# AdeeshKolluru/AdsorbDiff

Measured on AMD Instinct MI355X. Metric: sampled adsorbate sites/sec (50 denoise steps, ~200-atom slabs), higher is better.
Workload: dtype f32 (f16x3-split MFMA, fp32 accumulate; ADF_GEMM=f32 selects exact f32)

## Files before the change

### adsorbdiff_amd/csrc/api.hip

```cpp
#include <stdarg.h>
#include <stdlib.h>
#include <string.h>

#include <new>

#include "common.h"

static thread_local char g_err[512] = "";

void adf_set_error(const char* fmt, ...) {
    va_list ap;
    va_start(ap, fmt);
    vsnprintf(g_err, sizeof(g_err), fmt, ap);
    va_end(ap);
}

extern "C" const char* adf_last_error(void) { return g_err; }
extern "C" const char* adf_version(void) { return "adsorbdiff_hip 0.5.0 (gfx950)"; }

adf_tune adf_tune_from_env() {
    auto off_is_0 = [](const char* name) { const char* e = getenv(name); return (e && atoi(e) == 0) ? 0 : 1; };
    auto is_f32 = [](const char* name) { const char* e = getenv(name); return e && strcmp(e, "f32") == 0; };
    adf_tune t = {};
    const char* mi = getenv("ADF_GEMM16_MI");
    t.gemm16_mi = (mi && atoi(mi) == 4) ? 4 : 2;
    t.gemm_w8_plain = off_is_0("ADF_GEMM_W8_PLAIN");
    t.gemm_w8 = off_is_0("ADF_GEMM_W8");
    t.gemm_wreg = off_is_0("ADF_GEMM_WREG");
    const char* wf = getenv("ADF_GEMM_WR_FUSED");
    t.gemm_wr_fused = wf ? atoi(wf) : 2;
    if (t.gemm_wr_fused != 0 && t.gemm_wr_fused != 4) t.gemm_wr_fused = 2;
    t.head_gate_fused = off_is_0("ADF_HEAD_GATE_FUSED");
    t.lift_emit = off_is_0("ADF_LIFT_EMIT");
    t.graph_sys_csr = off_is_0("ADF_GRAPH_SYS_CSR");
    t.train_gemm16 = is_f32("ADF_TRAIN_GEMM") ? 0 : 1;
    t.wgrad_f32 = is_f32("ADF_WGRAD") ? 1 : 0;
    const char* pw = getenv("ADF_EQV2_PW_MI");
    t.eqv2_pw_mi = (pw && atoi(pw) == 3) ? 3 : 4;
    const char* gt = getenv("ADF_EQV2_GEMM_TILE");
    t.eqv2_gemm_tile256 = (gt && atoi(gt) == 128) ? 0 : 1;
    t.eqv2_rotin_generic = getenv("ADF_EQV2_ROTIN_GENERIC") != nullptr;
    t.eqv2_rotout_generic = getenv("ADF_EQV2_ROTOUT_GENERIC") != nullptr;
    const char* r4 = getenv("ADF_GEMM_ROWS4");
    t.gemm_rows4 = r4 ? (atoi(r4) & 3) : 3;
    return t;
}
const adf_tune& adf_tune_process() {
    static const adf_tune t = adf_tune_from_env();
    return t;
}
int adf_current_num_cus() {
    int dev = 0, n = 0;
    if (hipGetDevice(&dev) != hipSuccess || hipDeviceGetAttribute(&n, hipDeviceAttributeMultiprocessorCount, dev) != hipSuccess) return 0;
    return n;
}

extern "C" int32_t adf_profile_enable(adf_painn_t h, int32_t on) {
    if (!h) { adf_set_error("null handle"); return ADF_EINVAL; }
    h->prof.enable(on != 0);
    ADF_HIP_CHECK(hipMemset(h->kcount, 0, 8 * sizeof(unsigned long long)));
    return ADF_OK;
}

extern "C" int32_t adf_profile_read(adf_painn_t h, float* ms, int64_t* count, int64_t* message_ksteps, void* stream) {
    if (!h || !ms || !count) { adf_set_error("null argument"); return ADF_EINVAL; }
    ADF_HIP_CHECK(hipStreamSynchronize((hipStream_t)stream));
    if (message_ksteps) {
        unsigned long long k[8];
        ADF_HIP_CHECK(hipMemcpy(k, h->kcount, sizeof(k), hipMemcpyDeviceToHost));
        ADF_HIP_CHECK(hipMemset(h->kcount, 0, sizeof(k)));
        *message_ksteps = (int64_t)k[0];
    }
    return h->prof.read(ms, count, ADF_PROF_NCAT);
}

extern "C" int32_t adf_painn_create(const adf_painn_hparams* hp, adf_painn_t* out) {
    if (!hp || !out) { adf_set_error("null argument"); return ADF_EINVAL; }
    if (hp->hidden_channels % ADF_SLICE_CH != 0 || hp->hidden_channels < 128 || hp->hidden_channels > 1024) {
        adf_set_error("hidden_channels=%d must be a multiple of %d in [128,1024]", hp->hidden_channels, ADF_SLICE_CH);
        return ADF_EINVAL;
    }
    if (hp->num_rbf % 2 != 0 || hp->num_rbf > 128 || hp->num_rbf < 2) {
        adf_set_error("num_rbf=%d must be even and <= 128", hp->num_rbf);
        return ADF_EINVAL;
    }
    if (hp->max_neighbors < 1 || hp->max_neighbors > ADF_MAX_K) {
        adf_set_error("max_neighbors=%d must be in [1,%d]", hp->max_neighbors, ADF_MAX_K);
        return ADF_EINVAL;
    }
    if (hp->num_layers < 1 || hp->num_layers > 16 || hp->num_heads < 0 || hp->num_heads > 2) {
        adf_set_error("num_layers must be in [1,16], num_heads in [0,2]");
        return ADF_EINVAL;
    }
    adf_painn* h = new (std::nothrow) adf_painn();
    if (!h) { adf_set_error("host allocation failed"); return ADF_EOOM; }
    h->hp = *hp;
    hipDeviceProp_t prop;
    if (hipGetDevice(&h->device) != hipSuccess || hipGetDeviceProperties(&prop, h->device) != hipSuccess) {
        adf_set_error("no usable HIP device: %s", hipGetErrorString(hipGetLastError()));
        adf_painn_destroy(h);
        return ADF_EHIP;
    }
    h->num_cus = prop.multiProcessorCount;
    h->dist_floor = 1.0e-3f;
    {
        const char* e = getenv("ADF_INCREMENTAL");
        h->inc_on = !(e && e[0] == '0');
        const char* e2 = getenv("ADF_INC_SYNC");
        h->inc_sync = e2 && e2[0] == '1';
    }
    const int H = hp->hidden_channels, R = hp->num_rbf, L = hp->num_layers;
    adf_pool& m = h->m_life;
    int32_t st = m.alloc(&h->rbf_pack, (size_t)L * (H / ADF_SLICE_CH) * R * 192);
    if (st == ADF_OK) st = m.alloc(&h->rbf_bias_pack, (size_t)L * (H / ADF_SLICE_CH) * 192);
    if (st == ADF_OK) st = m.alloc(&h->rbf_pack16, (size_t)L * (H / ADF_SLICE_CH) * R * 192 * 2 * sizeof(uint16_t));
    if (st == ADF_OK) st = m.alloc(&h->rbf_bias_pack16, (size_t)L * (H / ADF_SLICE_CH) * 192);
    if (st == ADF_OK) st = m.alloc(&h->rbf_scales, 16);
    if (st == ADF_OK) st = m.alloc(&h->flags, ADF_NFLAGS);
    if (st == ADF_OK && hipMemset(h->flags, 0, sizeof(int32_t) * ADF_NFLAGS) != hipSuccess) st = ADF_EHIP;
    {
        const size_t HH = (size_t)H * H;
        const size_t per_layer = HH + 3 * HH + 2 * HH + 2 * HH + 3 * HH;
        const size_t per_head = HH + HH / 2 + 2 * HH + HH + HH / 4 + HH / 2;
        const size_t elems = (size_t)L * per_layer + (size_t)hp->num_heads * per_head;
        h->w16_bytes = elems * 2 * sizeof(uint16_t) + 4096;
        if (st == ADF_OK) st = m.alloc(&h->w16_arena, h->w16_bytes);
        if (st == ADF_OK) st = m.alloc(&h->w16_scales, 256);
        if (st == ADF_OK) st = m.alloc(&h->w16_bias_perm, (size_t)L * 2 * 3 * H);
        if (st == ADF_OK) st = m.alloc(&h->w16_scratch, 1);
        if (st == ADF_OK) st = m.alloc(&h->wfrag_arena, h->w16_bytes);
        const char* e = getenv("ADF_GEMM");
        h->gemm_f32 = e && strcmp(e, "f32") == 0;
        const char* el = getenv("ADF_LIFT");
        h->lift_on = !(el && strcmp(el, "0") == 0);
        const char* e2 = getenv("ADF_MSG");
        h->msg_f32 = e2 ? strcmp(e2, "f32") == 0 : h->gemm_f32;
        const char* er = getenv("ADF_ROW_MAXIMA");
        h->rmx = (er && atoi(er) == 0) ? 0 : 1;
        h->tune = adf_tune_from_env();
    }
    if (st == ADF_OK) st = m.alloc(&h->kcount, 8);
    if (st == ADF_OK && hipMemset(h->kcount, 0, 8 * sizeof(unsigned long long)) != hipSuccess) st = ADF_EHIP;
    if (st != ADF_OK) { adf_painn_destroy(h); return st; }
    *out = h;
    return ADF_OK;
}

static void inc_free(adf_painn* h) {
    h->m_inc.release();
    h->inc_tmp_bytes = 0;
    h->inc_capN = 0; h->inc_valid = false;
}

static void free_workspaces(adf_painn* h) {
    h->m_ws.release();
    h->inc_valid = false;
    h->scan_tmp_bytes = 0;
    h->lift.cap = 0; h->mag_v3_valid = false;
    h->xpart = h->catpart = h->vpart = nullptr; h->part_stride = 0;
    h->part_x = h->part_vec = nullptr; h->dbg_msg_rows = h->dbg_cat_rows = h->dbg_comb_rows = 0; h->dbg_mag = nullptr;
    h->cache_valid = false;
    h->capN = h->capB = h->capE = 0;
}

extern "C" int32_t adf_painn_destroy(adf_painn_t h) {
    if (!h) return ADF_OK;
    if (h->inc_cnt_host) (void)hipHostFree(h->inc_cnt_host);
    for (int i = 0; i < 2; ++i)
        if (h->inc_ev[i]) (void)hipEventDestroy((hipEvent_t)h->inc_ev[i]);
    adf_grad_free(h);
    delete h;
    return ADF_OK;
}

extern "C" int32_t adf_painn_set_weights(adf_painn_t h, int32_t n_weights, const void* const* w,
                                         const float* scale_factors, void* stream) {
    if (!h || !w || !scale_factors) { adf_set_error("null argument"); return ADF_EINVAL; }
    const int L = h->hp.num_layers;
    const int expect = 2 + ADF_WEIGHTS_PER_LAYER * L + ADF_WEIGHTS_PER_HEAD * h->hp.num_heads;
    if (n_weights != expect) {
        adf_set_error("expected %d weight tensors, got %d", expect, n_weights);
        return ADF_EINVAL;
    }
    for (int i = 0; i < n_weights; ++i)
        if (!w[i]) { adf_set_error("weight %d is null", i); return ADF_EINVAL; }
    auto f = [&](int i) { return reinterpret_cast<const float*>(w[i]); };
    h->emb = f(0);
    h->rbf_offset = f(1);
    int k = 2;
    for (int l = 0; l < L; ++l) {
        adf_layer_weights& lw = h->layer[l];
        lw.ln_w = f(k++); lw.ln_b = f(k++); lw.xp0_w = f(k++); lw.xp0_b = f(k++); lw.xp2_w = f(k++); lw.xp2_b = f(k++);
        lw.rbf_w = f(k++); lw.rbf_b = f(k++); lw.vp_w = f(k++); lw.xv0_w = f(k++); lw.xv0_b = f(k++);
        lw.xv2_w = f(k++); lw.xv2_b = f(k++);
        h->scale[l] = scale_factors[l];
    }
    for (int hd = 0; hd < h->hp.num_heads; ++hd)
        for (int b = 0; b < 2; ++b) {
            adf_block_weights& bw = h->head[hd][b];
            bw.vec1_w = f(k++); bw.vec2_w = f(k++); bw.un0_w = f(k++); bw.un0_b = f(k++); bw.un2_w = f(k++);
            bw.un2_b = f(k++);
        }
    ADF_TRY(adf_pack_rbf(h, (hipStream_t)stream));
    {
        hipStream_t s = (hipStream_t)stream;
        const long long H = h->hp.hidden_channels, HH = H * H;
        unsigned char* cur = h->w16_arena;
        unsigned char* fcur = h->wfrag_arena;
        int nscale = 0;
        float* bperm = h->w16_bias_perm;
        auto split = [&](const float* w, long long rows, long long K, adf_w16* out, const float* fused_bias = nullptr,
                         bool pair_perm = false) -> int32_t {
            const long long n = rows * K;
            out->hi = cur; cur += n * 2;
            out->lo = cur; cur += n * 2;
            out->inv_scale = h->w16_scales + nscale++;
            out->bias_perm = nullptr;
            out->frag = nullptr;
            if (fused_bias) {
                out->bias_perm = bperm; bperm += 3 * H;
                ADF_TRY(adf_split_weight(w, n, out, h->w16_scratch, s, (int)H, (int)H, fused_bias));
            } else if (pair_perm) {
                ADF_TRY(adf_split_weight(w, n, out, h->w16_scratch, s, (int)H, (int)H, nullptr, 2));
            } else {
                ADF_TRY(adf_split_weight(w, n, out, h->w16_scratch, s));
            }
            if (rows % 32 == 0 && K % 16 == 0) {
                out->frag = fcur; fcur += n * 4;
                ADF_TRY(adf_pack_frag(out, (int)rows, (int)K, out->frag, s));
            }
            return ADF_OK;
        };
        for (int l = 0; l < L; ++l) {
            adf_layer_weights& lw = h->layer[l];
            ADF_TRY(split(lw.xp0_w, H, H, &lw.xp0_16));
            ADF_TRY(split(lw.xp2_w, 3 * H, H, &lw.xp2_16, lw.xp2_b));
            ADF_TRY(split(lw.vp_w, 2 * H, H, &lw.vp_16, nullptr, true));
            ADF_TRY(split(lw.xv0_w, H, 2 * H, &lw.xv0_16));
            ADF_TRY(split(lw.xv2_w, 3 * H, H, &lw.xv2_16, lw.xv2_b));
        }
        for (int hd = 0; hd < h->hp.num_heads; ++hd) {
            adf_block_weights& b0 = h->head[hd][0];
            adf_block_weights& b1 = h->head[hd][1];
            ADF_TRY(split(b0.vec1_w, H, H, &b0.vec1_16));
            ADF_TRY(split(b0.vec2_w, H / 2, H, &b0.vec2_16));
            ADF_TRY(split(b0.un0_w, H, 2 * H, &b0.un0_16));
            ADF_TRY(split(b0.un2_w, H, H, &b0.un2_16));
            ADF_TRY(split(b1.vec1_w, H / 2, H / 2, &b1.vec1_16));
            ADF_TRY(split(b1.un0_w, H / 2, H, &b1.un0_16));
        }
        if ((size_t)(cur - h->w16_arena) > h->w16_bytes || (size_t)(fcur - h->wfrag_arena) > h->w16_bytes || nscale > 256) {
            adf_set_error("internal: fp16 weight arena overflow");
            return ADF_EINVAL;
        }
    }
    h->weights_set = true;
    h->rec0_valid = false;
    h->inc_valid = false;
    adf_grad_invalidate(h);
    return ADF_OK;
}

static int32_t ensure_capacity(adf_painn* h, int64_t N, int64_t B) {
    if (N <= h->capN && B <= h->capB) return ADF_OK;
    const int64_t capN = N > h->capN ? N : h->capN;
    const int64_t capB = B > h->capB ? B : h->capB;
    ADF_HIP_CHECK(hipDeviceSynchronize());
    free_workspaces(h);
    const int64_t H = h->hp.hidden_channels, K = h->hp.max_neighbors;
    const int64_t capE = 2 * capN * K;
    int32_t st = ADF_OK;
#define ALLOC(field, count) if (st == ADF_OK) st = h->m_ws.alloc(&h->field, (size_t)(count))
    ALLOC(nbr_cnt, capN);
    ALLOC(nbr_src, capN * K);
    ALLOC(nbr_shift, capN * K);
    ALLOC(cache_d2, capN * K);
    ALLOC(cache_cid, capN * K);
    ALLOC(cache_cnt, capN);
    ALLOC(deg, capN + 1);
    ALLOC(nptr, capN + 1);
    ALLOC(cursor, capN);
    ALLOC(img_cnt, capB);
    ALLOC(sys_slow, capB);
    ALLOC(e_src, capE);
    ALLOC(e_geom, capE);
    if (h->inc_on) {
        ALLOC(prev_nptr, capN + 1);
        ALLOC(prev_src, capE);
        ALLOC(prev_geom, capE);
    }
    if (st == ADF_OK) {
        h->scan_tmp_bytes = adf_scan_temp_bytes(capN + 1);
        st = h->m_ws.alloc(&h->scan_tmp, h->scan_tmp_bytes + 16);
    }
    ALLOC(x, capN * H);
    ALLOC(vecA, capN * 3 * H);
    ALLOC(vecB, capN * 3 * H);
    ALLOC(rec, (capN + 1) * 5 * H);
    ALLOC(y, capN * H);
    ALLOC(xh, capN * 3 * H);
    ALLOC(vv, capN * 6 * H);
    ALLOC(cat, capN * 2 * H);
    ALLOC(dot, capN * H);
    ALLOC(sys, capB * 16);
    ALLOC(lift.buf, capN * 3);
    ALLOC(mag_a, capN);
    ALLOC(mag_b, capN);
    ALLOC(mag_v3, capN * 3);
    const int64_t ps = (capN + 31) / 32 * 32, ns = H / ADF_SLICE_CH;
    if (h->rmx) ALLOC(rmx_part, (4 * ns + H / 32 + 4) * ps);
#undef ALLOC
    h->lift.cap = st == ADF_OK ? capN * 3 : 0;
    if (st != ADF_OK) { free_workspaces(h); return st; }
    if (h->rmx) {
        h->part_stride = ps;
        h->xpart = h->rmx_part; h->catpart = h->xpart + ns * ps; h->vpart = h->catpart + (H / 32) * ps;
        h->dbg_mag = h->vpart + 3 * ns * ps;
    }
    h->capN = capN; h->capB = capB; h->capE = capE;
    return ADF_OK;
}

static int32_t check_batch(const adf_painn* h, const adf_batch* b) {
    if (!h || !b) { adf_set_error("null argument"); return ADF_EINVAL; }
    if (b->num_atoms <= 0 || b->num_systems <= 0) { adf_set_error("empty batch"); return ADF_EINVAL; }
    if (!b->pos || !b->cell || !b->batch || !b->atom_offset) { adf_set_error("null batch array"); return ADF_EINVAL; }
    for (int k = 0; k < 3; ++k)
        if (b->reps[k] < 0 || b->reps[k] > 16) { adf_set_error("reps[%d]=%d out of range", k, b->reps[k]); return ADF_EINVAL; }
    return ADF_OK;
}

static int32_t read_flags(adf_painn* h, hipStream_t s) {
    int32_t f[ADF_NFLAGS];
    ADF_HIP_CHECK(hipMemcpyAsync(f, h->flags, sizeof(f), hipMemcpyDeviceToHost, s));
    ADF_HIP_CHECK(hipMemsetAsync(h->flags, 0, sizeof(f), s));
    ADF_HIP_CHECK(hipStreamSynchronize(s));
    if (f[4]) { adf_set_error("atomic number outside [1, %d] (rows of the embedding table)", h->hp.num_elements); return ADF_EINVAL; }
    if (f[0]) { adf_set_error("a centre atom has more than %d in-cutoff candidates", ADF_MAX_CAND); return ADF_EOVERFLOW; }
    if (f[2]) { adf_set_error("edge buffer overflow"); return ADF_EOVERFLOW; }
    if (f[3]) { adf_set_error("an atom has more than %d incoming edges", ADF_MAX_INDEG); return ADF_EOVERFLOW; }
    if (f[1]) { adf_set_error("An image has no neighbors"); return ADF_ENONEIGHBOR; }
    if (f[6]) { adf_set_error("energy gradient: an edge row has no reverse row in its partner's segment (asymmetric graph)"); return ADF_EINVAL; }
    if (f[5]) {
        adf_set_error("non-finite model output%s", h->gemm_f32 ? " (exact-f32 arithmetic: the inputs or weights are not finite)"
                      : " in f16x3 arithmetic: an activation left the fp16 range or the inputs are not finite; "
                        "adf_painn_set_arithmetic(h, 1) selects exact f32");
        return ADF_ENUMERIC;
    }
    return ADF_OK;
}

extern "C" int32_t adf_graph_set_moving(adf_painn_t h, const int32_t* moving, const int32_t* mov_idx,
                                        const int32_t* mov_off) {
    if (!h) { adf_set_error("null handle"); return ADF_EINVAL; }
    if (moving && (!mov_idx || !mov_off)) { adf_set_error("moving mask needs mov_idx and mov_off"); return ADF_EINVAL; }
    h->moving = moving; h->mov_idx = mov_idx; h->mov_off = mov_off;
    ADF_HIP_CHECK(hipMemset(h->flags, 0, sizeof(int32_t) * ADF_NFLAGS));
    h->cache_valid = false;
    h->rec0_valid = false;
    h->inc_valid = false;
    return ADF_OK;
}

extern "C" int32_t adf_graph_build(adf_painn_t h, const adf_batch* b, void* stream, int64_t* num_edges) {
    ADF_TRY(check_batch(h, b));
    ADF_TRY(ensure_capacity(h, b->num_atoms, b->num_systems));
    hipStream_t s = (hipStream_t)stream;
    ADF_TRY(adf_graph_build_impl(h, b, s));
    if (num_edges) {
        int32_t e = 0;
        ADF_HIP_CHECK(hipMemcpyAsync(&e, h->nptr + b->num_atoms, sizeof(int32_t), hipMemcpyDeviceToHost, s));
        ADF_TRY(read_flags(h, s));
        *num_edges = e;
    }
    return ADF_OK;
}

__global__ void adf_export_edges_kernel(const int32_t* nptr, const int32_t* e_src, const float4* eg, int N,
                                        int32_t* src, int32_t* dst, float* dist, float* vec, long long cap) {
    const int n = blockIdx.x * 4 + (threadIdx.x >> 6);
    if (n >= N) return;
    for (int e = nptr[n] + (threadIdx.x & 63); e < nptr[n + 1]; e += 64) {
        if (e >= cap) continue;
        if (src) src[e] = e_src[e];
        if (dst) dst[e] = n;
        const float4 q = eg[e];
        if (dist) dist[e] = q.w;
        if (vec) { vec[3 * (size_t)e] = q.x; vec[3 * (size_t)e + 1] = q.y; vec[3 * (size_t)e + 2] = q.z; }
    }
}

__global__ void adf_export_shift_kernel(const int32_t* nbr_shift, int32_t* out, long long n, int r0, int r1, int r2) {
    const long long i = (long long)blockIdx.x * blockDim.x + threadIdx.x;
    if (i >= n) return;
    const int c = nbr_shift[i];
    const int n2 = 2 * r2 + 1, n1 = 2 * r1 + 1;
    const int ia = c / (n1 * n2), rem = c - ia * (n1 * n2);
    out[3 * i] = ia - r0;
    out[3 * i + 1] = rem / n2 - r1;
    out[3 * i + 2] = rem % n2 - r2;
}

extern "C" int32_t adf_graph_export(adf_painn_t h, int32_t* nbr_count, int32_t* nbr_src, int32_t* nbr_shift,
                                    int64_t edge_capacity, int32_t* edge_src, int32_t* edge_dst, float* edge_dist,
                                    float* edge_vec, int64_t* num_edges, void* stream) {
    if (!h || h->lastN <= 0) { adf_set_error("no graph built"); return ADF_EINVAL; }
    hipStream_t s = (hipStream_t)stream;
    const int64_t N = h->lastN, K = h->hp.max_neighbors;
    if (nbr_count) ADF_HIP_CHECK(hipMemcpyAsync(nbr_count, h->nbr_cnt, sizeof(int32_t) * N, hipMemcpyDeviceToDevice, s));
    if (nbr_src) ADF_HIP_CHECK(hipMemcpyAsync(nbr_src, h->nbr_src, sizeof(int32_t) * N * K, hipMemcpyDeviceToDevice, s));
    if (nbr_shift)
        hipLaunchKernelGGL(adf_export_shift_kernel, dim3((unsigned)((N * K + 255) / 256)), dim3(256), 0, s, h->nbr_shift,
                           nbr_shift, (long long)(N * K), h->last_reps[0], h->last_reps[1], h->last_reps[2]);
    if (edge_src || edge_dst || edge_dist || edge_vec)
        hipLaunchKernelGGL(adf_export_edges_kernel, dim3((unsigned)((N + 3) / 4)), dim3(256), 0, s, h->nptr, h->e_src,
                           h->e_geom, (int)N, edge_src, edge_dst, edge_dist, edge_vec, (long long)edge_capacity);
    ADF_HIP_CHECK(hipGetLastError());
    int32_t e = 0;
    ADF_HIP_CHECK(hipMemcpyAsync(&e, h->nptr + N, sizeof(int32_t), hipMemcpyDeviceToHost, s));
    ADF_HIP_CHECK(hipStreamSynchronize(s));
    if (num_edges) *num_edges = e;
    return ADF_OK;
}

static int32_t zero_pad_rows(adf_painn* h, int N, hipStream_t s) {
    const size_t row = (size_t)5 * h->hp.hidden_channels;
    ADF_HIP_CHECK(hipMemsetAsync(h->rec + (size_t)N * row, 0, sizeof(float) * row, s));
    return ADF_OK;
}

static int32_t make_records(adf_painn* h, int l, int n, const float* x, const float* vec, bool vec_is_zero, float* rec,
                            const int32_t* row_map, hipStream_t s) {
    const int H = h->hp.hidden_channels;
    const adf_layer_weights& w = h->layer[l];
    if (n <= 0) return ADF_OK;
    adf_prof_begin(h, ADF_PROF_NODE, s);
    const bool lift = h->lift_on && !h->gemm_f32;
    const bool em = lift && h->tune.lift_emit;
    ADF_TRY(adf_nodewise_layernorm(x, w.ln_w, w.ln_b, h->y, n, H, s, em ? h->mag_a : nullptr, h->rows_dev));
    ADF_TRY(adf_linear(h, h->y, H, w.xp0_w, &w.xp0_16, w.xp0_b, h->cat, H, n, H, H, 1, s, em ? h->mag_a : nullptr,
                       em ? h->mag_b : nullptr));
    if (h->gemm_f32) {
        if (row_map) { adf_set_error("internal: mapped records need the f16x3 path"); return ADF_EINVAL; }
        ADF_TRY(adf_launch_gemm(h->cat, H, w.xp2_w, H, w.xp2_b, h->xh, 3 * H, n, 3 * H, H, 0, s));
        ADF_TRY(adf_pack_records(h, n, h->xh, vec, vec_is_zero, s, rec));
    } else {
        adf_epi ep = {};
        ep.vec_in = vec; ep.rec = rec ? rec : h->rec; ep.H = H; ep.vec_is_zero = vec_is_zero ? 1 : 0;
        ep.row_map = row_map;
        ep.rmag = em ? h->mag_b : nullptr;
        ep.m_dev = h->rows_dev;
        ADF_TRY(adf_launch_gemm16_fused(h->cat, H, &w.xp2_16, n, H, H, 1, &ep, s, h->tune, lift ? &h->lift : nullptr));
    }
    adf_prof_end(h, s);
    return ADF_OK;
}

static int32_t message_layer(adf_painn* h, int l, int N, const float* x, const float* vec, float* x_out,
                             float* vec_out, bool vec_is_zero, hipStream_t s, const int32_t* tlist = nullptr,
                             int n_targets = 0, float* rec = nullptr, bool records_ready = false) {
    if (!records_ready) ADF_TRY(make_records(h, l, N, x, vec, vec_is_zero, rec, nullptr, s));
    adf_prof_begin(h, ADF_PROF_MESSAGE, s);
    const int items = tlist ? n_targets : N;
    const bool emit = h->rmx && h->lift_on && !h->gemm_f32 && !h->msg_f32 && items > 0 && items <= h->part_stride;
    h->part_x = h->part_vec = nullptr;
    const int32_t st = adf_message_impl(h, l, N, x, h->xh, vec, x_out, vec_out, vec_is_zero, s, tlist, n_targets, rec,
                                        tlist ? h->rows_dev : nullptr, emit ? h->xpart : nullptr, h->vpart, h->part_stride);
    if (st == ADF_OK && emit) {
        h->part_x = x_out; h->part_vec = vec_out; h->part_n = items; h->part_dev = tlist ? h->rows_dev : nullptr;
        h->dbg_msg_rows = items;
    }
    adf_prof_end(h, s);
    return st;
}

static int32_t update_layer(adf_painn* h, int l, int N, float* x, float* vec, hipStream_t s, bool from_message = true) {
    const int H = h->hp.hidden_channels;
    const adf_layer_weights& w = h->layer[l];
    adf_prof_begin(h, ADF_PROF_NODE, s);
    const bool parts = from_message && h->rmx && h->lift_on && !h->gemm_f32 && N > 0 && h->part_x == x && h->part_vec == vec &&
                       h->part_n == N && h->part_dev == h->rows_dev;
    h->part_x = h->part_vec = nullptr;
    if (h->gemm_f32) {
        ADF_TRY(adf_launch_gemm(vec, H, w.vp_w, H, nullptr, h->vv, 2 * H, 3 * N, 2 * H, H, 0, s));
        ADF_TRY(adf_nodewise_update_prep(h->vv, x, h->cat, h->dot, N, H, s));
        ADF_TRY(adf_linear(h, h->cat, 2 * H, w.xv0_w, &w.xv0_16, w.xv0_b, h->y, H, N, H, 2 * H, 1, s));
    } else {
        adf_epi ep = {};
        ep.v1 = h->vv; ep.dotw = h->dot; ep.cat = h->cat; ep.H = H; ep.m_dev = h->rows_dev;
        const adf_lift* lf = h->lift_on ? &h->lift : nullptr;
        if (parts) {
            ADF_TRY(adf_launch_rowmax_combine(h->vpart, 3 * h->part_stride, H / ADF_SLICE_CH, 3ll * N, h->lift.buf, s, h->rows_dev, 3));
            ep.rmag = h->lift.buf;
            if (h->dbg_capture) ADF_HIP_CHECK(hipMemcpyAsync(h->dbg_mag, h->lift.buf, sizeof(float) * 3 * (size_t)N, hipMemcpyDeviceToDevice, s));
        }
        if (parts || (h->dbg_capture && h->rmx && lf && N <= h->part_stride)) {
            ep.catpart = h->catpart; ep.part_stride = h->part_stride; h->dbg_cat_rows = N;
        }
        ADF_TRY(adf_launch_gemm16_fused(vec, H, &w.vp_16, N, H, H, 3, &ep, s, h->tune, lf));
        if (parts) {
            ADF_TRY(adf_launch_rowmax_combine(h->xpart, h->part_stride, H / ADF_SLICE_CH + H / 32, N, h->lift.buf, s, h->rows_dev, 1));
            if (h->dbg_capture) {
                ADF_HIP_CHECK(hipMemcpyAsync(h->dbg_mag + 3 * h->part_stride, h->lift.buf, sizeof(float) * (size_t)N, hipMemcpyDeviceToDevice, s));
                h->dbg_comb_rows = N;
            }
        }
        adf_epi e0 = {};
        e0.A2 = h->cat; e0.K1 = H; e0.m_dev = h->rows_dev;
        e0.rmag = parts ? h->lift.buf : nullptr;
        e0.out_mag = h->lift_on ? reinterpret_cast<unsigned int*>(h->mag_b) : nullptr;
        ADF_TRY(adf_launch_gemm16(x, H, &w.xv0_16, w.xv0_b, h->y, H, N, H, 2 * H, 1, &e0, s, lf, h->tune, h->num_cus));
    }
    int32_t st;
    if (h->gemm_f32) {
        ADF_TRY(adf_launch_gemm(h->y, H, w.xv2_w, H, w.xv2_b, h->xh, 3 * H, N, 3 * H, H, 0, s));
        st = adf_nodewise_update_apply(h->xh, h->dot, h->vv, x, vec, h->scale[l], N, H, s);
    } else {
        adf_epi ep = {};
        ep.x = x; ep.vec = vec; ep.dot = h->dot; ep.vv = h->vv; ep.scale = h->scale[l]; ep.H = H;
        ep.rmag = h->lift_on ? h->mag_b : nullptr;
        ep.m_dev = h->rows_dev;
        st = adf_launch_gemm16_fused(h->y, H, &w.xv2_16, N, H, H, 2, &ep, s, h->tune);
    }
    adf_prof_end(h, s);
    return st;
}

extern "C" int32_t adf_painn_message_layer(adf_painn_t h, int32_t layer, int32_t N, const float* x, const float* vec,
                                           float* x_out, float* vec_out, void* stream) {
    if (!h || !h->weights_set || layer < 0 || layer >= h->hp.num_layers || N != h->lastN) {
        adf_set_error("message_layer: bad handle/layer, or N differs from the built graph");
        return ADF_EINVAL;
    }
    hipStream_t s = (hipStream_t)stream;
    ADF_TRY(zero_pad_rows(h, N, s));
    ADF_TRY(message_layer(h, layer, N, x, vec, x_out, vec_out, false, s));
    return ADF_OK;
}

extern "C" int32_t adf_painn_update_layer(adf_painn_t h, int32_t layer, int32_t N, float* x, float* vec, void* stream) {
    if (!h || !h->weights_set || layer < 0 || layer >= h->hp.num_layers) {
        adf_set_error("update_layer: bad handle/layer");
        return ADF_EINVAL;
    }
    ADF_TRY(ensure_capacity(h, N, 1));
    return update_layer(h, layer, N, x, vec, (hipStream_t)stream, false);
}

extern "C" int32_t adf_painn_get_tune(adf_painn_t h, adf_tune* out) {
    if (!h || !out) { adf_set_error("get_tune: null handle or output"); return ADF_EINVAL; }
    *out = h->tune;
    return ADF_OK;
}

extern "C" int32_t adf_painn_debug_row_maxima(adf_painn_t h, int32_t which, float* out, int64_t capacity, int32_t* rows,
                                              void* stream) {
    if (!h || which < 0 || which > 6) { adf_set_error("debug_row_maxima: null handle or which outside 0..6"); return ADF_EINVAL; }
    if (which == 4) { h->dbg_capture = capacity != 0; h->dbg_comb_rows = 0; return ADF_OK; }
    const int H = h->hp.hidden_channels, ns = H / ADF_SLICE_CH;
    const int n = which <= 1 ? h->dbg_msg_rows : which <= 3 ? h->dbg_cat_rows : h->dbg_comb_rows;
    if (!h->rmx_part || n <= 0) { adf_set_error("debug_row_maxima: no launch has emitted row maxima (ADF_ROW_MAXIMA=0?)"); return ADF_EINVAL; }
    if (rows) *rows = n;
    if (!out) return ADF_OK;
    const int64_t need = (which == 1 || which == 5) ? 3ll * n : which == 3 ? (int64_t)n * H : n;
    if (capacity < need) { adf_set_error("debug_row_maxima: out holds %lld floats, need %lld", (long long)capacity, (long long)need); return ADF_EINVAL; }
    hipStream_t s = (hipStream_t)stream;
    if (which == 0) return adf_launch_rowmax_combine(h->xpart, h->part_stride, ns, n, out, s);
    if (which == 1) return adf_launch_rowmax_combine(h->vpart, 3 * h->part_stride, ns, 3ll * n, out, s);
    if (which == 2) return adf_launch_rowmax_combine(h->catpart, h->part_stride, H / 32, n, out, s);
    if (which >= 5) {
        ADF_HIP_CHECK(hipMemcpyAsync(out, h->dbg_mag + (which == 5 ? 0 : 3 * h->part_stride), sizeof(float) * (size_t)need, hipMemcpyDeviceToDevice, s));
        return ADF_OK;
    }
    ADF_HIP_CHECK(hipMemcpyAsync(out, h->cat, sizeof(float) * (size_t)n * H, hipMemcpyDeviceToDevice, s));
    return ADF_OK;
}

__global__ void adf_scatter_rows3_kernel(const float* __restrict__ src, const int32_t* __restrict__ idx, int n,
                                         float* __restrict__ dst) {
    const int i = blockIdx.x * blockDim.x + threadIdx.x;
    if (i < 3 * n) dst[(size_t)idx[i / 3] * 3 + i % 3] = src[i];
}

static int32_t ensure_subset(adf_painn* h, int32_t n_out) {
    if (n_out <= h->capS) return ADF_OK;
    const int64_t cap = (int64_t)n_out + n_out / 4 + 64;
    const size_t H = h->hp.hidden_channels;
    h->m_sub.release();
    h->capS = 0;
    ADF_TRY(h->m_sub.alloc(&h->sub_x, (size_t)cap * H));
    ADF_TRY(h->m_sub.alloc(&h->sub_vec, (size_t)cap * 3 * H));
    ADF_TRY(h->m_sub.alloc(&h->sub_f, (size_t)cap * 3));
    h->capS = cap;
    return ADF_OK;
}

static int inc_prepare(adf_painn* h, int N) {
    const int L = h->hp.num_layers, H = h->hp.hidden_channels;
    if (!h->inc_on || !h->moving || h->gemm_f32 || h->msg_f32 || L > ADF_MAX_LAYERS || !h->prev_nptr)
        return 0;
    if (N > h->inc_capN) {
        (void)hipDeviceSynchronize();
        inc_free(h);
        const size_t cap = (size_t)N;
        int32_t st = ADF_OK;
        for (int l = 0; l <= L && st == ADF_OK; ++l) {
            st = h->m_inc.alloc(&h->incX[l], cap * H);
            if (st == ADF_OK && l >= 1) st = h->m_inc.alloc(&h->incV[l], cap * 3 * H);
            if (st == ADF_OK && l < L) st = h->m_inc.alloc(&h->incR[l], (cap + 1) * 5 * H);
        }
        if (st == ADF_OK) st = h->m_inc.alloc(&h->inc_c0, cap);
        if (st == ADF_OK) st = h->m_inc.alloc(&h->inc_chg, 2 * cap);
        if (st == ADF_OK) st = h->m_inc.alloc(&h->inc_pend, cap * L);
        if (st == ADF_OK) st = h->m_inc.alloc(&h->inc_need, cap * L);
        if (st == ADF_OK) st = h->m_inc.alloc(&h->inc_tf, cap * L);
        if (st == ADF_OK) st = h->m_inc.alloc(&h->inc_list, cap * L);
        if (st == ADF_OK) st = h->m_inc.alloc(&h->inc_cnt, (size_t)2 * ADF_MAX_LAYERS + 1);
        if (st == ADF_OK) {
            h->inc_tmp_bytes = adf_inc_temp_bytes((int64_t)cap);
            st = h->m_inc.alloc(&h->inc_tmp, h->inc_tmp_bytes + 16);
        }
        if (st == ADF_OK && !h->inc_cnt_host &&
            hipHostMalloc(reinterpret_cast<void**>(&h->inc_cnt_host), sizeof(int32_t) * 2 * (2 * ADF_MAX_LAYERS + 1)) != hipSuccess)
            st = ADF_EOOM;
        for (int i = 0; i < 2 && st == ADF_OK; ++i)
            if (!h->inc_ev[i] && hipEventCreateWithFlags(reinterpret_cast<hipEvent_t*>(&h->inc_ev[i]), hipEventDisableTiming) != hipSuccess)
                st = ADF_EHIP;
        if (st != ADF_OK) {
            (void)hipGetLastError();
            inc_free(h);
            h->inc_on = false;
            fprintf(stderr, "adsorbdiff_hip: no memory for incremental layers (%d atoms), continuing without\n", N);
            return 0;
        }
        h->inc_capN = (int64_t)cap;
    }
    if (h->inc_N != N || h->inc_layers != L || h->build_serial != h->inc_serial) h->inc_valid = false;
    h->inc_N = N; h->inc_layers = L;
    int32_t* tn = h->nptr; h->nptr = h->prev_nptr; h->prev_nptr = tn;
    int32_t* ts = h->e_src; h->e_src = h->prev_src; h->prev_src = ts;
    float4* tg = h->e_geom; h->e_geom = h->prev_geom; h->prev_geom = tg;
    const int state = h->inc_valid ? 1 : 2;
    h->inc_valid = false;
    return state;
}

static int32_t inc_harvest(adf_painn* h, int slot, bool wait, bool peek = false) {
    if (!h->inc_ev_live[slot]) return ADF_OK;
    hipEvent_t ev = (hipEvent_t)h->inc_ev[slot];
    if (wait) {
        ADF_HIP_CHECK(hipEventSynchronize(ev));
    } else {
        const hipError_t q = hipEventQuery(ev);
        if (q == hipErrorNotReady) { (void)hipGetLastError(); return ADF_OK; }
        ADF_HIP_CHECK(q);
    }
    const int L = h->inc_layers, N = h->inc_pend_N[slot];
    const int32_t* c = h->inc_cnt_host + (size_t)slot * (2 * ADF_MAX_LAYERS + 1);
    for (int i = 0; i < 2 * L + 1; ++i) h->inc_seen[i] = c[i];
    h->inc_seen_valid = true;
    h->inc_pend_Nseen = N;
    if (peek) return ADF_OK;
    h->inc_ev_live[slot] = false;
    for (int l = 0; l < L; ++l) {
        const bool whole = h->inc_pend_whole[slot][l] != 0;
        h->inc_rows += (unsigned long long)(whole ? N : c[l]);
        h->inc_rows_full += (unsigned long long)N;
        h->inc_edges += (unsigned long long)(whole ? c[2 * L] : c[L + l]);
        if (whole || c[l] > 0) ++h->inc_launches;
    }
    return ADF_OK;
}

static int32_t forward_incremental(adf_painn* h, int N, const int32_t* Z, const int32_t* out_idx, int32_t n_out,
                                   float* f1, float* f2, bool first, int heads, hipStream_t s) {
    const int L = h->hp.num_layers, H = h->hp.hidden_channels;
    const size_t cap = (size_t)h->inc_capN, row = (size_t)5 * H;
    if (out_idx && n_out == 0) return ADF_OK;
    adf_prof_begin(h, ADF_PROF_GRAPH, s);
    if (first) {
        ADF_TRY(adf_nodewise_embed(h, Z, N, h->incX[0], s));
        for (int l = 0; l < L; ++l) ADF_HIP_CHECK(hipMemsetAsync(h->incR[l] + (size_t)N * row, 0, sizeof(float) * row, s));
        ADF_HIP_CHECK(hipMemsetAsync(h->inc_pend, 0, cap * L, s));
    } else {
        ADF_TRY(adf_inc_compare(h, N, s));
    }
    ADF_HIP_CHECK(hipMemsetAsync(h->inc_cnt, 0, sizeof(int32_t) * (2 * ADF_MAX_LAYERS + 1), s));
    if (out_idx) ADF_TRY(adf_inc_need_from_list(h, N, L, out_idx, n_out, s));
    for (int l = 0; l < L; ++l) ADF_TRY(adf_inc_plan_layer(h, l, N, first, out_idx != nullptr, s));
    ADF_HIP_CHECK(hipMemcpyAsync(h->inc_cnt + 2 * L, h->nptr + N, sizeof(int32_t), hipMemcpyDeviceToDevice, s));
    const int slot = h->inc_slot;
    h->inc_slot ^= 1;
    if (h->inc_ev_live[slot]) ADF_TRY(inc_harvest(h, slot, true));
    int32_t* host = h->inc_cnt_host + (size_t)slot * (2 * ADF_MAX_LAYERS + 1);
    ADF_HIP_CHECK(hipMemcpyAsync(host, h->inc_cnt, sizeof(int32_t) * (2 * L + 1), hipMemcpyDeviceToHost, s));
    ADF_HIP_CHECK(hipEventRecord((hipEvent_t)h->inc_ev[slot], s));
    h->inc_ev_live[slot] = true;
    h->inc_pend_N[slot] = N;
    ADF_TRY(inc_harvest(h, slot ^ 1, false));
    if (h->inc_sync) ADF_TRY(inc_harvest(h, slot, true, true));
    adf_prof_end(h, s);
    if (first) ADF_TRY(make_records(h, 0, N, h->incX[0], nullptr, true, h->incR[0], nullptr, s));
    for (int l = 0; l < L; ++l) {
        const int n_seen = h->inc_seen_valid ? h->inc_seen[l] : N;
        const bool whole = first || !h->inc_seen_valid || h->inc_pend_Nseen != N || (long long)n_seen * 10 >= (long long)N * 9;
        h->inc_pend_whole[slot][l] = whole ? 1 : 0;
        if (h->inc_sync && !whole && n_seen == 0) continue;
        const float* vin = l == 0 ? h->vecA : h->incV[l];
        if (whole) {
            ADF_TRY(message_layer(h, l, N, h->incX[l], vin, h->incX[l + 1], h->incV[l + 1], l == 0, s, nullptr, 0,
                                  h->incR[l], true));
            ADF_TRY(update_layer(h, l, N, h->incX[l + 1], h->incV[l + 1], s));
            if (l + 1 < L)
                ADF_TRY(make_records(h, l + 1, N, h->incX[l + 1], h->incV[l + 1], false, h->incR[l + 1], nullptr, s));
            continue;
        }
        const int32_t* list = h->inc_list + cap * l;
        const int ncap = h->inc_sync ? n_seen : N;
        h->rows_dev = h->inc_cnt + l;
        int32_t st = message_layer(h, l, N, h->incX[l], vin, h->x, h->vecB, l == 0, s, list, ncap, h->incR[l], true);
        if (st == ADF_OK) st = update_layer(h, l, ncap, h->x, h->vecB, s);
        if (st == ADF_OK) {
            adf_prof_begin(h, ADF_PROF_NODE, s);
            st = adf_inc_scatter_rows(h->x, list, ncap, H, h->incX[l + 1], s, h->rows_dev);
            if (st == ADF_OK) st = adf_inc_scatter_rows(h->vecB, list, ncap, 3 * H, h->incV[l + 1], s, h->rows_dev);
            adf_prof_end(h, s);
        }
        if (st == ADF_OK && l + 1 < L) st = make_records(h, l + 1, ncap, h->x, h->vecB, false, h->incR[l + 1], list, s);
        h->rows_dev = nullptr;
        ADF_TRY(st);
    }
    adf_prof_begin(h, ADF_PROF_HEADS, s);
    if (!out_idx) {
        if (heads >= 1) ADF_TRY(adf_head_forward(h, 0, N, h->incX[L], h->incV[L], f1, s));
        if (heads == 2) ADF_TRY(adf_head_forward(h, 1, N, h->incX[L], h->incV[L], f2, s));
        h->x_last = h->incX[L];
    } else {
        ADF_TRY(ensure_subset(h, n_out));
        ADF_TRY(adf_inc_gather_rows(h->incX[L], out_idx, n_out, H, h->sub_x, s));
        ADF_TRY(adf_inc_gather_rows(h->incV[L], out_idx, n_out, 3 * H, h->sub_vec, s));
        for (int hd = 0; hd < heads; ++hd) {
            ADF_TRY(adf_head_forward(h, hd, n_out, h->sub_x, h->sub_vec, h->sub_f, s));
            hipLaunchKernelGGL(adf_scatter_rows3_kernel, dim3((3 * n_out + 255) / 256), dim3(256), 0, s, h->sub_f, out_idx,
                               n_out, hd == 0 ? f1 : f2);
        }
        ADF_HIP_CHECK(hipGetLastError());
    }
    adf_prof_end(h, s);
    h->inc_valid = true;
    return ADF_OK;
}

static int32_t forward_impl(adf_painn_t h, const adf_batch* b, const int32_t* out_idx, int32_t n_out, float* f1,
                            float* f2, void* stream, bool head1_only = false) {
    ADF_TRY(check_batch(h, b));
    if (!h->weights_set) { adf_set_error("weights not set"); return ADF_EINVAL; }
    const int heads = head1_only ? 1 : h->hp.num_heads;
    if (heads > h->hp.num_heads) { adf_set_error("the model has no force head"); return ADF_EINVAL; }
    if (!b->atomic_numbers || (heads >= 1 && !f1) || (heads == 2 && !f2)) { adf_set_error("null argument"); return ADF_EINVAL; }
    h->x_last = nullptr;
    hipStream_t s = (hipStream_t)stream;
    const int N = b->num_atoms;
    ADF_TRY(ensure_capacity(h, N, b->num_systems));
    const int inc = inc_prepare(h, N);
    adf_prof_begin(h, ADF_PROF_GRAPH, s);
    ADF_TRY(adf_graph_build_impl(h, b, s));
    adf_prof_end(h, s);
    if (inc) {
        h->inc_serial = h->build_serial;
        return forward_incremental(h, N, b->atomic_numbers, out_idx, n_out, f1, f2, inc == 2, heads, s);
    }
    ADF_TRY(zero_pad_rows(h, N, s));
    ADF_TRY(adf_nodewise_embed(h, b->atomic_numbers, N, h->x, s));
    float* vin = h->vecA;
    float* vout = h->vecB;
    const int L = h->hp.num_layers, H = h->hp.hidden_channels;
    float* rec0 = nullptr;
    bool rec0_ready = false;
    if (h->moving) {
        const size_t row = (size_t)5 * H;
        if ((int64_t)N + 1 > h->rec0_cap) {
            h->rec0_cap = 0; h->rec0_valid = false;
            ADF_TRY(h->m_rec0.alloc(&h->rec0, ((size_t)N + 1) * row));
            h->rec0_cap = (int64_t)N + 1;
        }
        rec0 = h->rec0;
        rec0_ready = h->rec0_valid && h->rec0_N == N;
        if (!rec0_ready) ADF_HIP_CHECK(hipMemsetAsync(rec0 + (size_t)N * row, 0, sizeof(float) * row, s));
        h->rec0_valid = true; h->rec0_N = N;
    }
    if (!out_idx) {
        for (int l = 0; l < L; ++l) {
            if (l == 0) ADF_TRY(message_layer(h, 0, N, h->x, vin, h->x, vout, true, s, nullptr, 0, rec0, rec0_ready));
            else
            ADF_TRY(message_layer(h, l, N, h->x, vin, h->x, vout, l == 0, s));
            ADF_TRY(update_layer(h, l, N, h->x, vout, s));
            float* t = vin; vin = vout; vout = t;
        }
        adf_prof_begin(h, ADF_PROF_HEADS, s);
        if (heads >= 1) ADF_TRY(adf_head_forward(h, 0, N, h->x, vin, f1, s));
        if (heads == 2) ADF_TRY(adf_head_forward(h, 1, N, h->x, vin, f2, s));
        adf_prof_end(h, s);
        h->x_last = h->x;
        return ADF_OK;
    }
    if (n_out == 0) return ADF_OK;
    ADF_TRY(ensure_subset(h, n_out));
    for (int l = 0; l + 1 < L; ++l) {
        if (l == 0) ADF_TRY(message_layer(h, 0, N, h->x, vin, h->x, vout, true, s, nullptr, 0, rec0, rec0_ready));
        else
        ADF_TRY(message_layer(h, l, N, h->x, vin, h->x, vout, l == 0, s));
        ADF_TRY(update_layer(h, l, N, h->x, vout, s));
        float* t = vin; vin = vout; vout = t;
    }
    ADF_TRY(message_layer(h, L - 1, N, h->x, vin, h->sub_x, h->sub_vec, L == 1, s, out_idx, n_out,
                          L == 1 ? rec0 : nullptr, L == 1 && rec0_ready));
    ADF_TRY(update_layer(h, L - 1, n_out, h->sub_x, h->sub_vec, s));
    adf_prof_begin(h, ADF_PROF_HEADS, s);
    for (int hd = 0; hd < heads; ++hd) {
        ADF_TRY(adf_head_forward(h, hd, n_out, h->sub_x, h->sub_vec, h->sub_f, s));
        hipLaunchKernelGGL(adf_scatter_rows3_kernel, dim3((3 * n_out + 255) / 256), dim3(256), 0, s, h->sub_f, out_idx,
                           n_out, hd == 0 ? f1 : f2);
    }
    ADF_HIP_CHECK(hipGetLastError());
    adf_prof_end(h, s);
    return ADF_OK;
}

extern "C" int32_t adf_painn_forward(adf_painn_t h, const adf_batch* b, float* f1, float* f2, void* stream) {
    return forward_impl(h, b, nullptr, 0, f1, f2, stream);
}

extern "C" int32_t adf_painn_forward_subset(adf_painn_t h, const adf_batch* b, const int32_t* out_idx, int32_t n_out,
                                            float* f1, float* f2, void* stream) {
    if (!out_idx || n_out < 0) { adf_set_error("forward_subset: null index list"); return ADF_EINVAL; }
    return forward_impl(h, b, out_idx, n_out, f1, f2, stream);
}

extern "C" int32_t adf_painn_set_energy_head(adf_painn_t h, int32_t n_weights, const void* const* w, void* stream) {
    if (!h || !w) { adf_set_error("null argument"); return ADF_EINVAL; }
    if (n_weights != 4) { adf_set_error("set_energy_head: expected 4 tensors (out_energy.0.weight/bias, out_energy.2.weight/bias), got %d", n_weights); return ADF_EINVAL; }
    for (int i = 0; i < 4; ++i)
        if (!w[i]) { adf_set_error("energy-head tensor %d is null", i); return ADF_EINVAL; }
    const int H = h->hp.hidden_channels, H2 = H / 2;
    const size_t n = (size_t)H2 * H;
    if (!h->oe0_buf) ADF_TRY(h->m_life.alloc(&h->oe0_buf, n * 4 + 64));
    h->oe0_w = reinterpret_cast<const float*>(w[0]);
    h->oe0_b = reinterpret_cast<const float*>(w[1]);
    h->oe2_w = reinterpret_cast<const float*>(w[2]);
    h->oe2_b = reinterpret_cast<const float*>(w[3]);
    adf_w16& e = h->oe0_16;
    e = adf_w16{};
    e.hi = h->oe0_buf; e.lo = h->oe0_buf + n * 2; e.inv_scale = reinterpret_cast<float*>(h->oe0_buf + n * 4);
    ADF_TRY(adf_split_weight(h->oe0_w, (long long)n, &e, reinterpret_cast<unsigned int*>(h->oe0_buf + n * 4 + 16),
                             (hipStream_t)stream));
    h->energy_set = true;
    adf_grad_invalidate(h);
    return ADF_OK;
}

extern "C" int32_t adf_painn_set_distance_floor(adf_painn_t h, float floor) {
    if (!h || !(floor > 0.f)) { adf_set_error("set_distance_floor: null handle or non-positive floor"); return ADF_EINVAL; }
    if (floor != h->dist_floor) {
        h->dist_floor = floor;
        h->cache_valid = false;
        h->rec0_valid = false;
        h->inc_valid = false;
    }
    return ADF_OK;
}

__global__ __launch_bounds__(256) void adf_energy_sum_kernel(const float* __restrict__ y, int H2, const float* __restrict__ w,
                                                             const float* __restrict__ bias, const int32_t* __restrict__ atom_offset,
                                                             float* __restrict__ energy) {
    __shared__ float part[4];
    const int b = blockIdx.x, lane = threadIdx.x & 63, wave = threadIdx.x >> 6;
    const int a0 = atom_offset[b], a1 = atom_offset[b + 1];
    const float b0 = bias[0];
    float acc = 0.f;
    for (int a = a0 + wave; a < a1; a += 4) {
        const float* row = y + (size_t)a * H2;
        float d = 0.f;
        for (int c = lane; c < H2; c += 64) d = fmaf(row[c], w[c], d);
        for (int o = 32; o > 0; o >>= 1) d = __fadd_rn(d, __shfl_xor(d, o, 64));
        acc = __fadd_rn(acc, __fadd_rn(d, b0));
    }
    if (lane == 0) part[wave] = acc;
    __syncthreads();
    if (threadIdx.x == 0) energy[b] = __fadd_rn(__fadd_rn(part[0], part[1]), __fadd_rn(part[2], part[3]));
}

int32_t adf_energy_sum(const float* y, int H2, const float* w, const float* bias, const int32_t* atom_offset, float* energy,
                       int num_systems, hipStream_t s) {
    hipLaunchKernelGGL(adf_energy_sum_kernel, dim3(num_systems), dim3(256), 0, s, y, H2, w, bias, atom_offset, energy);
    ADF_HIP_CHECK(hipGetLastError());
    return ADF_OK;
}

extern "C" int32_t adf_painn_forward_energy(adf_painn_t h, const adf_batch* b, float* energy, float* forces, void* stream) {
    ADF_TRY(check_batch(h, b));
    if (!h->energy_set) { adf_set_error("forward_energy: energy head not set (adf_painn_set_energy_head)"); return ADF_EINVAL; }
    if (!energy || (h->hp.num_heads >= 1 && !forces)) { adf_set_error("forward_energy: null output"); return ADF_EINVAL; }
    if (h->hp.num_heads > 1) { adf_set_error("forward_energy: the S2EF model has one force head"); return ADF_EINVAL; }
    hipStream_t s = (hipStream_t)stream;
    ADF_TRY(forward_impl(h, b, nullptr, 0, forces, nullptr, stream));
    if (!h->x_last) { adf_set_error("internal: no node features after the forward"); return ADF_EINVAL; }
    const int N = b->num_atoms, H = h->hp.hidden_channels, H2 = H / 2;
    adf_prof_begin(h, ADF_PROF_HEADS, s);
    ADF_TRY(adf_linear(h, h->x_last, H, h->oe0_w, &h->oe0_16, h->oe0_b, h->y, H2, N, H2, H, 1, s));
    ADF_TRY(adf_energy_sum(h->y, H2, h->oe2_w, h->oe2_b, b->atom_offset, energy, b->num_systems, s));
    adf_prof_end(h, s);
    return ADF_OK;
}

extern "C" int32_t adf_linear_forward(const float* A, const float* W, const float* bias, float* C, int32_t M,
                                      int32_t N, int32_t K, int32_t act_ssilu, int32_t mode, void* stream) {
    hipStream_t s = (hipStream_t)stream;
    if (!A || !W || !C || M <= 0 || N <= 0 || K <= 0) { adf_set_error("bad argument"); return ADF_EINVAL; }
    if (mode == 0) return adf_launch_gemm(A, K, W, K, bias, C, N, M, N, K, act_ssilu, s);
    adf_pool tmp;
    unsigned char* buf = nullptr;
    const size_t n = (size_t)N * K;
    ADF_TRY(tmp.alloc(&buf, n * 4 + 64));
    adf_w16 w16 = {};
    w16.hi = buf; w16.lo = buf + n * 2; w16.inv_scale = reinterpret_cast<float*>(buf + n * 4);
    unsigned int* scratch = reinterpret_cast<unsigned int*>(buf + n * 4 + 16);
    int32_t st = adf_split_weight(W, (long long)n, &w16, scratch, s);
    float* mags = nullptr;
    const char* el = getenv("ADF_LIFT");
    const bool lift = !(el && strcmp(el, "0") == 0);
    if (st == ADF_OK && lift) st = tmp.alloc(&mags, (size_t)M);
    adf_lift lf = {mags, M};
    if (st == ADF_OK) st = adf_launch_gemm16(A, K, &w16, bias, C, N, M, N, K, act_ssilu, nullptr, s, lift ? &lf : nullptr,
                                             adf_tune_process(), adf_current_num_cus());
    (void)hipStreamSynchronize(s);
    return st;
}

extern "C" int32_t adf_painn_set_arithmetic(adf_painn_t h, int32_t exact_f32) {
    if (!h) { adf_set_error("null handle"); return ADF_EINVAL; }
    h->gemm_f32 = exact_f32 != 0;
    h->msg_f32 = exact_f32 != 0;
    h->rec0_valid = false;
    h->inc_valid = false;
    return ADF_OK;
}

extern "C" int32_t adf_painn_set_incremental(adf_painn_t h, int32_t on) {
    if (!h) { adf_set_error("null handle"); return ADF_EINVAL; }
// ... 126 lines not shown
```

### adsorbdiff_amd/csrc/common.h

```cpp
#pragma once
#include <hip/hip_runtime.h>
#include <stdint.h>
#include <stdio.h>
#include <string>
#include <vector>

#include "../../include/adsorbdiff_hip.h"

#define ADF_GROUP_NODES 32
#define ADF_SLICE_CH 64
#define ADF_MAX_CAND 1024
#define ADF_MAX_K 128
#define ADF_NFLAGS 8
#define ADF_MAX_INDEG 1024
#define ADF_MAX_LAYERS 16

void adf_set_error(const char* fmt, ...);

#define ADF_HIP_CHECK(expr)                                                             \
    do {                                                                                \
        hipError_t _e = (expr);                                                         \
        if (_e != hipSuccess) {                                                         \
            adf_set_error("%s failed: %s (%s:%d)", #expr, hipGetErrorString(_e),        \
                          __FILE__, __LINE__);                                          \
            return (_e == hipErrorOutOfMemory) ? ADF_EOOM : ADF_EHIP;                   \
        }                                                                               \
    } while (0)

#define ADF_TRY(expr)                     \
    do {                                  \
        int32_t _s = (expr);              \
        if (_s != ADF_OK) return _s;      \
    } while (0)

struct adf_pool {
    std::vector<void**> slots;
    adf_pool() = default;
    adf_pool(const adf_pool&) = delete;
    adf_pool& operator=(const adf_pool&) = delete;
    ~adf_pool() { release(); }
    int32_t alloc(void** field, size_t bytes) {
        bool known = false;
        for (void** s : slots) known = known || s == field;
        if (known) { if (*field) (void)hipFree(*field); } else slots.push_back(field);
        *field = nullptr;
        if (bytes == 0) bytes = 16;
        const hipError_t e = hipMalloc(field, bytes);
        if (e == hipSuccess) return ADF_OK;
        *field = nullptr;
        (void)hipGetLastError();
        adf_set_error("device allocation of %zu bytes failed: %s", bytes, hipGetErrorString(e));
        return ADF_EOOM;
    }
    template <typename T>
    int32_t alloc(T** field, size_t count) { return alloc(reinterpret_cast<void**>(field), count * sizeof(T)); }
    void release() {
        for (void** s : slots) {
            if (*s) (void)hipFree(*s);
            *s = nullptr;
        }
        slots.clear();
    }
};

struct adf_prof {
    bool on = false;
    bool open = false;
    std::vector<hipEvent_t> ev;
    std::vector<int> cat;
    size_t used = 0;
    adf_prof() = default;
    adf_prof(const adf_prof&) = delete;
    adf_prof& operator=(const adf_prof&) = delete;
    ~adf_prof() { for (hipEvent_t e : ev) (void)hipEventDestroy(e); }
    void begin(int c, hipStream_t s) {
        open = false;
        if (!on) return;
        if (used + 2 > ev.size())
            for (int i = 0; i < 512; ++i) {
                hipEvent_t e;
                if (hipEventCreate(&e) != hipSuccess) { (void)hipGetLastError(); break; }
                ev.push_back(e);
            }
        if (used + 2 > ev.size()) return;
        cat.resize(used / 2);
        cat.push_back(c);
        (void)hipEventRecord(ev[used], s);
        open = true;
    }
    void end(hipStream_t s) {
        if (!on || !open) return;
        (void)hipEventRecord(ev[used + 1], s);
        used += 2;
        open = false;
    }
    void enable(bool o) { on = o; open = false; used = 0; cat.clear(); }
    int32_t read(float* ms, int64_t* count, int ncat) {
        for (int c = 0; c < ncat; ++c) { ms[c] = 0.f; count[c] = 0; }
        for (size_t i = 0; i < used; i += 2) {
            float t = 0.f;
            ADF_HIP_CHECK(hipEventElapsedTime(&t, ev[i], ev[i + 1]));
            ms[cat[i / 2]] += t;
            count[cat[i / 2]] += 1;
        }
        enable(on);
        return ADF_OK;
    }
    struct scope {
        adf_prof& p; hipStream_t s;
        scope(adf_prof& p_, int c, hipStream_t s_) : p(p_), s(s_) { p.begin(c, s); }
        ~scope() { p.end(s); }
    };
};

struct adf_w16 {
    void* hi;
    void* lo;
    float* inv_scale;
    float* bias_perm;
    void* frag;
};
struct adf_epi {
    const float* vec_in;
    float* rec;
    float* x;
    float* vec;
    const float* dot;
    const float* vv;
    float* v1;
    float* dotw;
    float* cat;
    float scale;
    int H;
    int vec_is_zero;
    const float* A2;
    int K1;
    const int32_t* row_map;
    const float* rmag;
    unsigned int* out_mag;
    const int32_t* m_dev;
    int accumulate;
    const float* gate;
    int gate_ld;
    float* catpart;
    long long part_stride;
};
struct adf_lift {
    float* buf;
    long long cap;
};
struct adf_layer_weights {
    const float *ln_w, *ln_b, *xp0_w, *xp0_b, *xp2_w, *xp2_b, *rbf_w, *rbf_b;
    const float *vp_w, *xv0_w, *xv0_b, *xv2_w, *xv2_b;
    adf_w16 xp0_16, xp2_16, vp_16, xv0_16, xv2_16;
};
struct adf_block_weights {
    const float *vec1_w, *vec2_w, *un0_w, *un0_b, *un2_w, *un2_b;
    adf_w16 vec1_16, vec2_16, un0_16, un2_16;
};

struct adf_painn {
    adf_painn_hparams hp;
    int device;
    bool weights_set;
    const float* emb;
    const float* rbf_offset;
    adf_layer_weights layer[16];
    adf_block_weights head[2][2];
    float scale[16];
    float* rbf_pack;
    float* rbf_bias_pack;
    void* rbf_pack16;
    float* rbf_bias_pack16;
    float* rbf_scales;
    unsigned char* w16_arena;
    size_t w16_bytes;
    float* w16_scales;
    float* w16_bias_perm;
    unsigned int* w16_scratch;
    unsigned char* wfrag_arena;
    bool gemm_f32;
    bool msg_f32;
    adf_tune tune;
    bool lift_on;
    adf_lift lift;
    float *mag_a, *mag_b;
    float* mag_v3;
    bool mag_v3_valid;
    int rmx;
    float* rmx_part;
    float *xpart, *catpart, *vpart;
    int64_t part_stride;
    const float *part_x, *part_vec;
    int part_n;
    const int32_t* part_dev;
    int dbg_msg_rows, dbg_cat_rows;
    bool dbg_capture;
    float* dbg_mag;
    int dbg_comb_rows;

    int64_t capN, capB, capE;
    int32_t* nbr_cnt;
    int32_t* nbr_src;
    int32_t* nbr_shift;
    int32_t* deg;
    int32_t* nptr;
    int32_t* cursor;
    int32_t* img_cnt;
    int32_t* sys_slow;
    void* scan_tmp;
    size_t scan_tmp_bytes;
    const int32_t* moving;
    const int32_t* mov_idx;
    const int32_t* mov_off;
    float* cache_d2;
    int32_t* cache_cid;
    int32_t* cache_cnt;
    bool cache_valid;
    int32_t* e_src;
    float4* e_geom;
    int32_t* flags;
    float *x, *vecA, *vecB, *y, *xh, *vv, *cat, *dot;
    float* rec;
    bool rbf_uniform;
    float* rec0;
    int64_t rec0_cap, rec0_N;
    bool rec0_valid;
    bool inc_on;
    bool inc_valid;
    int64_t inc_capN, inc_N;
    int inc_layers;
    float* incX[ADF_MAX_LAYERS + 1];
    float* incV[ADF_MAX_LAYERS + 1];
    float* incR[ADF_MAX_LAYERS];
    int32_t *prev_nptr, *prev_src;
    float4* prev_geom;
    unsigned char *inc_c0, *inc_chg;
    unsigned char *inc_pend, *inc_need, *inc_tf;
    int32_t* inc_list;
    int32_t* inc_cnt;
    int32_t* inc_cnt_host;
    void* inc_ev[2];
    bool inc_ev_live[2];
    int inc_slot;
    bool inc_sync;
    int32_t inc_seen[2 * ADF_MAX_LAYERS + 1];
    bool inc_seen_valid;
    unsigned char inc_pend_whole[2][ADF_MAX_LAYERS];
    int32_t inc_pend_N[2];
    int32_t inc_pend_Nseen;
    const int32_t* rows_dev;
    void* inc_tmp; size_t inc_tmp_bytes;
    unsigned long long inc_rows, inc_rows_full, inc_edges, inc_launches;
    unsigned long long build_serial, inc_serial;
    float *sub_x, *sub_vec, *sub_f;
    int64_t capS;
    float* sys;
    const float *oe0_w, *oe0_b, *oe2_w, *oe2_b;
    adf_w16 oe0_16;
    unsigned char* oe0_buf;
    bool energy_set;
    const float* x_last;
    float dist_floor;
    void* grad;
    int64_t lastN, lastB;
    int32_t last_reps[3];
    int num_cus;
    adf_prof prof;
    unsigned long long* kcount;
    adf_pool m_life;
    adf_pool m_ws;
    adf_pool m_inc;
    adf_pool m_sub;
    adf_pool m_rec0;
};

enum { ADF_PROF_GRAPH = 0, ADF_PROF_MESSAGE = 1, ADF_PROF_NODE = 2, ADF_PROF_HEADS = 3, ADF_PROF_STEPPER = 4 };
static inline void adf_prof_begin(adf_painn* h, int cat, hipStream_t s) { h->prof.begin(cat, s); }
static inline void adf_prof_end(adf_painn* h, hipStream_t s) { h->prof.end(s); }

int32_t adf_launch_gemm(const float* A, int lda, const float* W, int ldw, const float* bias, float* C, int ldc,
                        int M, int N, int K, int act_ssilu, hipStream_t s);
adf_tune adf_tune_from_env();
const adf_tune& adf_tune_process();
int adf_current_num_cus();
int32_t adf_launch_gemm16(const float* A, int lda, const adf_w16* W, const float* bias, float* C, int ldc, int M,
                          int N, int K, int act_ssilu, const adf_epi* ep, hipStream_t s, const adf_lift* lf,
                          const adf_tune& tune, int num_cus);
int32_t adf_launch_rowmag(const float* A, int lda, int K1, const float* A2, int K2, long long M, float* mag, hipStream_t s,
                          const int32_t* m_dev = nullptr, int m_mul = 1);
int32_t adf_launch_rowmax_combine(const float* part, long long stride, int nparts, long long M, float* mag, hipStream_t s,
                                  const int32_t* m_dev = nullptr, int m_mul = 1);
int32_t adf_split_weight(const float* w, long long n, adf_w16* out, unsigned int* scratch_bits, hipStream_t s,
                         int perm_H = 0, int K = 0, const float* bias = nullptr, int parts = 3);
int32_t adf_launch_gemm16_vecnorm(const float* A, int lda, const adf_w16* W, float* nrm, int M, int N, int K,
                                  hipStream_t s, const adf_tune& tune, const adf_lift* lf = nullptr,
                                  const float* premag = nullptr);
int32_t adf_launch_gemm16_fused(const float* A, int lda, const adf_w16* W, int M, int H, int K, int epi,
                                const adf_epi* ep, hipStream_t s, const adf_tune& tune, const adf_lift* lf = nullptr);
static inline int32_t adf_linear(const adf_painn* h, const float* A, int lda, const float* W, const adf_w16* W16,
                                 const float* bias, float* C, int ldc, int M, int N, int K, int act, hipStream_t s,
                                 const float* premag = nullptr, float* out_mag = nullptr) {
    if (h->gemm_f32) return adf_launch_gemm(A, lda, W, K, bias, C, ldc, M, N, K, act, s);
    adf_epi ep = {};
    ep.m_dev = h->rows_dev;
    if (h->lift_on) { ep.rmag = premag; ep.out_mag = reinterpret_cast<unsigned int*>(out_mag); }
    return adf_launch_gemm16(A, lda, W16, bias, C, ldc, M, N, K, act, &ep, s, h->lift_on ? &h->lift : nullptr, h->tune,
                             h->num_cus);
}
int32_t adf_pack_frag(const adf_w16* w, int N, int K, void* out, hipStream_t s);
int32_t adf_graph_build_impl(adf_painn* h, const adf_batch* b, hipStream_t s);
int32_t adf_energy_sum(const float* y, int H2, const float* w, const float* bias, const int32_t* atom_offset, float* energy,
                       int num_systems, hipStream_t s);
__device__ __forceinline__ float adf_row16_max(float v) {
#define ADF_ROR(n_) __int_as_float(__builtin_amdgcn_update_dpp(0, __float_as_int(v), 0x120 + (n_), 0xf, 0xf, false))
    v = fmaxf(v, ADF_ROR(8));
    v = fmaxf(v, ADF_ROR(4));
    v = fmaxf(v, ADF_ROR(2));
    v = fmaxf(v, ADF_ROR(1));
#undef ADF_ROR
    return v;
}
__device__ __forceinline__ float adf_half32_max_hi(float v) {
    v = adf_row16_max(v);
    return fmaxf(v, __int_as_float(__builtin_amdgcn_update_dpp(0, __float_as_int(v), 0x142, 0xa, 0xf, false)));
}
__device__ __forceinline__ float adf_lane8_max(float v) {
#define ADF_DPP(c_) __int_as_float(__builtin_amdgcn_update_dpp(0, __float_as_int(v), (c_), 0xf, 0xf, false))
    v = fmaxf(v, ADF_DPP(0xb1));
    v = fmaxf(v, ADF_DPP(0x4e));
    v = fmaxf(v, ADF_DPP(0x141));
#undef ADF_DPP
    return v;
}
__device__ __forceinline__ float adf_ssilu(float x) { return x / (1.0f + expf(-x)) * 1.6666666666666667f; }
__device__ __forceinline__ float adf_dssilu_times(float x, float w) {
    const float sg = 1.0f / (1.0f + expf(-x));
    return sg * (1.0f + x * (1.0f - sg)) * 1.6666666666666667f * w;
}
void adf_grad_invalidate(adf_painn* h);
void adf_grad_free(adf_painn* h);
bool adf_message_geo_supported(const adf_painn* h);
int32_t adf_message_geo(adf_painn* h, int layer, const float* xh, const float* vec, bool vec_is_zero, float4* part,
                        long long ecap, bool accumulate, hipStream_t s);
size_t adf_inc_temp_bytes(int64_t n);
int32_t adf_inc_compare(adf_painn* h, int N, hipStream_t s);
int32_t adf_inc_need_from_list(adf_painn* h, int N, int L, const int32_t* out_idx, int n_out, hipStream_t s);
int32_t adf_inc_plan_layer(adf_painn* h, int l, int N, bool first, bool have_need, hipStream_t s);
int32_t adf_inc_scatter_rows(const float* src, const int32_t* idx, int n, int width, float* dst, hipStream_t s,
                             const int32_t* n_dev = nullptr);
int32_t adf_inc_gather_rows(const float* src, const int32_t* idx, int n, int width, float* dst, hipStream_t s);
size_t adf_scan_temp_bytes(int64_t n);
int32_t adf_message_impl(adf_painn* h, int layer, int N, const float* x, const float* xh, const float* vec,
                         float* x_out, float* vec_out, bool vec_is_zero, hipStream_t s,
                         const int32_t* tlist = nullptr, int n_targets = 0, const float* rec = nullptr,
                         const int32_t* n_targets_dev = nullptr,
                         float* xpart = nullptr, float* vpart = nullptr, long long part_stride = 0);
int32_t adf_pack_rbf(adf_painn* h, hipStream_t s);
int32_t adf_pack_rbf_layer(adf_painn* h, int l, hipStream_t s);
int32_t adf_pack_records(adf_painn* h, int N, const float* xh, const float* vec, bool vec_is_zero, hipStream_t s,
                         float* rec = nullptr);
int32_t adf_nodewise_embed(adf_painn* h, const int32_t* Z, int N, float* x, hipStream_t s);
int32_t adf_nodewise_layernorm(const float* x, const float* w, const float* b, float* y, int N, int H, hipStream_t s,
                               float* out_mag = nullptr, const int32_t* n_dev = nullptr);
int32_t adf_nodewise_update_prep(const float* vv, const float* x, float* cat, float* dot, int N, int H, hipStream_t s);
int32_t adf_nodewise_update_apply(const float* h3, const float* dot, const float* vv, float* x, float* vec,
                                  float scale, int N, int H, hipStream_t s);
int32_t adf_head_forward(adf_painn* h, int head, int N, const float* x, const float* vec, float* out, hipStream_t s);
int32_t adf_stepper_init(const adf_batch* b, float* pos, const int32_t* tags, const float* noise,
                         hipStream_t s);
int32_t adf_stepper_step(float* sys, const adf_batch* b, float* pos, const int32_t* tags, const int32_t* fixed,
                         const float* f1, const float* f2, const adf_step_coef* coef, const adf_step_coef* coefs_dev,
                         int num_steps, const float* z_tr, const float* z_rot, int32_t early_stop_count,
                         int32_t* state, float* dcom, float* drot, hipStream_t s);
int32_t adf_stepper_tr_step(float* sys, const adf_batch* b, float* pos, const int32_t* tags, const float* f1,
                            const adf_tr_coef* coef, const adf_tr_coef* coefs_dev, int num_steps, const float* z,
                            int32_t early_stop_count, int32_t* state, float* dcom, hipStream_t s);

struct adf_model {
    void* h;
    int32_t (*check)(void* h, const adf_batch* b);
    int32_t (*grow)(void* h, const adf_batch* b, float** sys);
    int32_t (*forward)(void* h, const adf_batch* b, const int32_t* out_idx, int32_t n_out, float* f1, float* f2,
                       hipStream_t s);
    void (*prof)(void* h, bool begin, hipStream_t s);
};
int32_t adf_frames_push_impl(adf_frames* f, const float* src, hipStream_t s);
int32_t adf_model_init_placement(const adf_model& m, const adf_batch* b, float* pos, const int32_t* tags,
                                 const float* noise, hipStream_t s);
int32_t adf_model_sde_step(const adf_model& m, const adf_batch* b, float* pos, const int32_t* tags, const int32_t* fixed,
                           const float* f1, const float* f2, const adf_step_coef* coef, const adf_step_coef* coefs_dev,
                           int32_t num_steps, const float* z_tr, const float* z_rot, int32_t early_stop_count,
                           int32_t* state, float* dcom, float* drot, hipStream_t s);
int32_t adf_model_tr_step(const adf_model& m, const adf_batch* b, float* pos, const int32_t* tags, const float* f1,
                          const adf_tr_coef* coef, const adf_tr_coef* coefs_dev, int32_t num_steps, const float* z,
                          int32_t early_stop_count, int32_t* state, float* dcom, hipStream_t s);
int32_t adf_model_sample(const adf_model& m, const adf_batch* b, float* pos, const int32_t* tags, const int32_t* fixed,
                         const adf_step_coef* coefs_dev, int32_t num_steps, const float* z_tr_all, const float* z_rot_all,
                         int32_t early_stop_count, int32_t poll_every, int32_t* state, const int32_t* out_idx,
                         int32_t n_out, float* f1, float* f2, adf_frames* sink, int32_t frame_every, hipStream_t s);
int32_t adf_model_tr_sample(const adf_model& m, const adf_batch* b, float* pos, const int32_t* tags,
                            const adf_tr_coef* coefs_dev, int32_t num_steps, const float* z_all, int32_t early_stop_count,
                            int32_t poll_every, int32_t* state, const int32_t* out_idx, int32_t n_out, float* f1,
                            adf_frames* sink, int32_t frame_every, hipStream_t s);
```

### adsorbdiff_amd/csrc/gemm16.hip

```cpp
#include <stdlib.h>

#include "common.h"

typedef float f32x16 __attribute__((ext_vector_type(16)));
typedef _Float16 half8 __attribute__((ext_vector_type(8)));
typedef _Float16 half4 __attribute__((ext_vector_type(4)));

#ifndef EPI_ABL
#define EPI_ABL 0
#endif
#ifndef EPI2_POLICY
#define EPI2_POLICY 0
#endif
#ifndef G16_ABL
#define G16_ABL 0
#endif
#ifndef G16_WDEEP
#define G16_WDEEP 1
#endif
#ifndef G16_START_DELAY
#define G16_START_DELAY 0
#endif
#define HK 32
#define TLD3 96
#define TLD2 64
#define HLD 40

__device__ __forceinline__ float adf_pow2_lift(float mx) {
    if (!(mx > 0.f) || !(mx < 3.0e38f)) return 1.0f;
    int e;
    (void)frexpf(mx, &e);
    e = 15 - e;
    e = e > 120 ? 120 : (e < -120 ? -120 : e);
    return ldexpf(1.0f, e);
}

__device__ __forceinline__ float ssilu16(float x) {
    float s = x / (1.0f + expf(-x));
    return s * 1.6666666666666667f;
}

template <int ACT, int MI, int NJ, int EPI, bool WR = false, int NWN = 2, int NWM = 2>
__global__ __launch_bounds__(64 * NWM * NWN, (MI == 4 || NWM * NWN == 8 ? 1 : 2)) void adf_gemm_f16x3_kernel(
    const float* __restrict__ A, int lda, const _Float16* __restrict__ Whi, const _Float16* __restrict__ Wlo,
    const float* __restrict__ inv_scale, const float* __restrict__ bias, float* __restrict__ C, int ldc, int Mh, int N,
    int K, int tiles_n, adf_epi ep) {
    const int M = ep.m_dev ? min(Mh, (int)*ep.m_dev) : Mh;
    static_assert(NWN == 2 || WR, "eight waves only with the register-streamed weights");
    static_assert(NWM == 2 || (NWM == 1 && WR), "one wave along M only with the register-streamed weights");
    constexpr int NT = 64 * NWM * NWN;
    constexpr int TM = 32 * MI * NWM;
    constexpr int TN = 32 * NJ * NWN;
    constexpr int NA = TM * 8 / NT;
    static_assert(TM * 8 % NT == 0, "A staging: whole float4s per thread");
    constexpr int LDS_WR = 4 * TM * HLD > NT / 64 * 6400 ? 4 * TM * HLD : NT / 64 * 6400;
    constexpr int LDS_MAIN = WR ? LDS_WR : (2 * TM + 2 * TN) * HLD;
    constexpr int LDS_REC = EPI == 1 ? NT / 64 * 2048 : 0;
    __shared__ __attribute__((aligned(16))) _Float16 lds[LDS_MAIN + LDS_REC];
    __shared__ float rinv[TM];
    _Float16* Ahi = lds;
    _Float16* Alo = Ahi + TM * HLD;
    _Float16* Bhi = Alo + TM * HLD;
    _Float16* Blo = Bhi + TN * HLD;
    const int tid = threadIdx.x;
    const int lane = tid & 63;
    const int wave = tid >> 6;
    const int wm = (wave / NWN) * (32 * MI);
    const int wn = (wave % NWN) * (32 * NJ);

    const int id = blockIdx.x;
    const int xcd = id & 7;
    const int qd = id >> 3;
    const int tile_m = (qd / tiles_n) * 8 + xcd;
    const int tile_n = qd % tiles_n;
    const int m0 = tile_m * (EPI >= 3 ? TM / 3 : TM);
    const int n0 = tile_n * TN;
    if (m0 >= M) return;
#if G16_START_DELAY
    if constexpr (NWM == 1) {
        if (qd >= 32 && qd < 64)
            for (int i = 0; i < G16_START_DELAY; ++i) __builtin_amdgcn_s_sleep(127);
    }
#endif

    unsigned int a_goff[NA];
    int a_off[NA];
    float a_rs[NA];
    auto global_row = [&](int row) -> unsigned int {
        if constexpr (EPI >= 3) {
            const int atom = m0 + (row / 96) * 32 + (row & 31), ax = (row % 96) >> 5;
            return (unsigned int)min(atom, M - 1) * 3u + ax;
        } else {
            return (unsigned int)min(m0 + row, M - 1);
        }
    };
#pragma unroll
    for (int i = 0; i < NA; ++i) {
        const int f = tid + NT * i;
        const int row = f >> 3, kq = f & 7;
        const unsigned int grow = global_row(row);
        a_goff[i] = (grow * (unsigned int)lda + kq * 4) * 4u;
        a_off[i] = row * HLD + kq * 4;
        a_rs[i] = ep.rmag ? adf_pow2_lift(ep.rmag[grow]) : 1.0f;
    }
    if (tid < TM) rinv[tid] = ep.rmag ? 1.0f / adf_pow2_lift(ep.rmag[global_row(tid)]) : 1.0f;
    const char* const A1b = reinterpret_cast<const char*>(A);
    const char* const A2b = reinterpret_cast<const char*>(ep.A2) - (size_t)ep.K1 * 4;
    int w_src[NJ];
    int w_off[NJ];
#pragma unroll
    for (int i = 0; i < NJ; ++i) {
        const int f = tid + 256 * i;
        const int row = f >> 2, part = f & 3;
        w_src[i] = min(n0 + row, N - 1) * K + part * 8;
        w_off[i] = row * HLD + part * 8;
    }

    float4 ra[NA];
    half8 rwh[NJ], rwl[NJ];
#pragma unroll
    for (int i = 0; i < NA; ++i) ra[i] = *reinterpret_cast<const float4*>(A1b + a_goff[i]);
    if constexpr (!WR) {
#pragma unroll
        for (int i = 0; i < NJ; ++i) {
            rwh[i] = *reinterpret_cast<const half8*>(Whi + w_src[i]);
            rwl[i] = *reinterpret_cast<const half8*>(Wlo + w_src[i]);
        }
    }
    half8 wfa[NJ][2], wfb[NJ][2];
    const half8* const wfr = reinterpret_cast<const half8*>(Whi) + (size_t)((n0 + wn) / 32) * (K / 16) * 128 + lane;
    auto load_wf = [&](int s_, half8 (&wf)[NJ][2]) {
#pragma unroll
        for (int j = 0; j < NJ; ++j) {
            const size_t base = ((size_t)j * (K / 16) + s_) * 128;
            wf[j][0] = wfr[base];
            wf[j][1] = wfr[base + 64];
        }
    };
    if constexpr (WR) load_wf(0, wfa);

    f32x16 acc[MI][NJ];
#pragma unroll
    for (int i = 0; i < MI; ++i)
#pragma unroll
        for (int j = 0; j < NJ; ++j)
#pragma unroll
            for (int r = 0; r < 16; ++r) acc[i][j][r] = 0.f;

    const int nk = K / HK;
    const int fa = (wm + (lane & 31)) * HLD + (lane >> 5) * 8;
    const int fb = (wn + (lane & 31)) * HLD + (lane >> 5) * 8;
    auto stage_a = [&](int boff = 0) {
#pragma unroll
        for (int i = 0; i < NA; ++i) {
            if (G16_ABL & 2) {
                *reinterpret_cast<float2*>(Ahi + boff + a_off[i]) = make_float2(ra[i].x, ra[i].y);
                *reinterpret_cast<float2*>(Alo + boff + a_off[i]) = make_float2(ra[i].z, ra[i].w);
                continue;
            }
            const float sx = ra[i].x * a_rs[i], sy = ra[i].y * a_rs[i], sz = ra[i].z * a_rs[i], sw = ra[i].w * a_rs[i];
            half4 h, l;
            h[0] = (_Float16)sx; h[1] = (_Float16)sy; h[2] = (_Float16)sz; h[3] = (_Float16)sw;
            l[0] = (_Float16)(sx - (float)h[0]); l[1] = (_Float16)(sy - (float)h[1]);
            l[2] = (_Float16)(sz - (float)h[2]); l[3] = (_Float16)(sw - (float)h[3]);
            *reinterpret_cast<half4*>(Ahi + boff + a_off[i]) = h;
            *reinterpret_cast<half4*>(Alo + boff + a_off[i]) = l;
        }
    };
    auto request_a = [&](int kt1) {
        const int k1 = kt1 * HK;
        const char* ab = ((ep.K1 > 0 && k1 >= ep.K1) ? A2b : A1b) + (size_t)k1 * 4;
#pragma unroll
        for (int i = 0; i < NA; ++i) ra[i] = *reinterpret_cast<const float4*>(ab + ((G16_ABL & 4) ? (a_goff[i] & 127u) : a_goff[i]));
    };
    if constexpr (WR) {
        auto kstep = [&](int boff, int ks, const half8 (&cur)[NJ][2]) {
            if (G16_ABL & 8) { asm volatile("" :: "v"(cur[0][0]), "v"(cur[0][1]), "v"(cur[NJ - 1][0]), "v"(cur[NJ - 1][1])); return; }
#pragma unroll
            for (int i = 0; i < MI; ++i) {
                const half8 ah = *reinterpret_cast<const half8*>(Ahi + boff + fa + i * 32 * HLD + ks * 16);
                const half8 al = *reinterpret_cast<const half8*>(Alo + boff + fa + i * 32 * HLD + ks * 16);
#pragma unroll
                for (int j = 0; j < NJ; ++j) {
                    acc[i][j] = __builtin_amdgcn_mfma_f32_32x32x16_f16(al, cur[j][0], acc[i][j], 0, 0, 0);
                    acc[i][j] = __builtin_amdgcn_mfma_f32_32x32x16_f16(ah, cur[j][1], acc[i][j], 0, 0, 0);
                    acc[i][j] = __builtin_amdgcn_mfma_f32_32x32x16_f16(ah, cur[j][0], acc[i][j], 0, 0, 0);
                }
            }
        };
        {
            constexpr int BUF = 2 * TM * HLD;
            float4 rb[NA];
            auto request_b = [&](int kt1) {
                const int k1 = kt1 * HK;
                const char* ab = ((ep.K1 > 0 && k1 >= ep.K1) ? A2b : A1b) + (size_t)k1 * 4;
#pragma unroll
                for (int i = 0; i < NA; ++i) rb[i] = *reinterpret_cast<const float4*>(ab + ((G16_ABL & 4) ? (a_goff[i] & 127u) : a_goff[i]));
            };
            auto stage_from = [&](const float4 (&src)[NA], int boff) {
#pragma unroll
                for (int i = 0; i < NA; ++i) {
                    if (G16_ABL & 2) {
                        *reinterpret_cast<float2*>(Ahi + boff + a_off[i]) = make_float2(src[i].x, src[i].y);
                        *reinterpret_cast<float2*>(Alo + boff + a_off[i]) = make_float2(src[i].z, src[i].w);
                        continue;
                    }
                    const float sx = src[i].x * a_rs[i], sy = src[i].y * a_rs[i], sz = src[i].z * a_rs[i], sw = src[i].w * a_rs[i];
                    half4 h, l;
                    h[0] = (_Float16)sx; h[1] = (_Float16)sy; h[2] = (_Float16)sz; h[3] = (_Float16)sw;
                    l[0] = (_Float16)(sx - (float)h[0]); l[1] = (_Float16)(sy - (float)h[1]);
                    l[2] = (_Float16)(sz - (float)h[2]); l[3] = (_Float16)(sw - (float)h[3]);
                    *reinterpret_cast<half4*>(Ahi + boff + a_off[i]) = h;
                    *reinterpret_cast<half4*>(Alo + boff + a_off[i]) = l;
                }
            };
#if G16_WDEEP
            half8 wfc[NJ][2], wfd[NJ][2];
            load_wf(1, wfb);
            auto tile = [&](int kt, int cur, const float4 (&nxt_regs)[NA], const half8 (&w0)[NJ][2], const half8 (&w1)[NJ][2],
                            half8 (&w2)[NJ][2], half8 (&w3)[NJ][2]) {
                load_wf(min(2 * kt + 2, 2 * nk - 1), w2);
                __builtin_amdgcn_sched_barrier(0);
                kstep(cur, 0, w0);
                __builtin_amdgcn_sched_barrier(0);
                load_wf(min(2 * kt + 3, 2 * nk - 1), w3);
                __builtin_amdgcn_sched_barrier(0);
                kstep(cur, 1, w1);
                stage_from(nxt_regs, BUF - cur);
#else
            auto tile = [&](int kt, int cur, const float4 (&nxt_regs)[NA]) {
                load_wf(2 * kt + 1, wfb);
                __builtin_amdgcn_sched_barrier(0);
                kstep(cur, 0, wfa);
                __builtin_amdgcn_sched_barrier(0);
                load_wf(min(2 * kt + 2, 2 * nk - 1), wfa);
                __builtin_amdgcn_sched_barrier(0);
                kstep(cur, 1, wfb);
                stage_from(nxt_regs, BUF - cur);
#endif
                __builtin_amdgcn_sched_group_barrier(0x100, 2 * MI, 0);
#pragma unroll
                for (int u = 0; u < 3 * MI * NJ; ++u) {
                    __builtin_amdgcn_sched_group_barrier(0x8, 1, 0);
                    __builtin_amdgcn_sched_group_barrier(0x2, 4, 0);
                    if (u % 3 == 2) __builtin_amdgcn_sched_group_barrier(0x200, 1, 0);
                }
                __builtin_amdgcn_sched_barrier(0);
            };
            __syncthreads();
            stage_a(0);
            request_a(min(1, nk - 1));
            request_b(min(2, nk - 1));
            __syncthreads();
            for (int kt = 0; kt < nk; kt += 2) {
#if G16_WDEEP
                tile(kt, 0, ra, wfa, wfb, wfc, wfd);
                request_a(min(kt + 3, nk - 1));
                __syncthreads();
                tile(kt + 1, BUF, rb, wfc, wfd, wfa, wfb);
#else
                tile(kt, 0, ra);
                request_a(min(kt + 3, nk - 1));
                __syncthreads();
                tile(kt + 1, BUF, rb);
#endif
                request_b(min(kt + 4, nk - 1));
                __syncthreads();
            }
        }
    } else {
    for (int kt = 0; kt < nk; ++kt) {
        __syncthreads();
        stage_a();
#pragma unroll
        for (int i = 0; i < NJ; ++i) {
            *reinterpret_cast<half8*>(Bhi + w_off[i]) = rwh[i];
            *reinterpret_cast<half8*>(Blo + w_off[i]) = rwl[i];
        }
        __syncthreads();
        if (kt + 1 < nk) {
            const int k1 = (kt + 1) * HK;
            request_a(kt + 1);
#pragma unroll
            for (int i = 0; i < NJ; ++i) {
                rwh[i] = *reinterpret_cast<const half8*>(Whi + w_src[i] + k1);
                rwl[i] = *reinterpret_cast<const half8*>(Wlo + w_src[i] + k1);
            }
        }
#pragma unroll
        for (int ks = 0; ks < 2; ++ks) {
            half8 bh[NJ], bl[NJ];
#pragma unroll
            for (int j = 0; j < NJ; ++j) {
                bh[j] = *reinterpret_cast<const half8*>(Bhi + fb + j * 32 * HLD + ks * 16);
                bl[j] = *reinterpret_cast<const half8*>(Blo + fb + j * 32 * HLD + ks * 16);
            }
#pragma unroll
            for (int i = 0; i < MI; ++i) {
                const half8 ah = *reinterpret_cast<const half8*>(Ahi + fa + i * 32 * HLD + ks * 16);
                const half8 al = *reinterpret_cast<const half8*>(Alo + fa + i * 32 * HLD + ks * 16);
#pragma unroll
                for (int j = 0; j < NJ; ++j) {
                    acc[i][j] = __builtin_amdgcn_mfma_f32_32x32x16_f16(al, bh[j], acc[i][j], 0, 0, 0);
                    acc[i][j] = __builtin_amdgcn_mfma_f32_32x32x16_f16(ah, bl[j], acc[i][j], 0, 0, 0);
                    acc[i][j] = __builtin_amdgcn_mfma_f32_32x32x16_f16(ah, bh[j], acc[i][j], 0, 0, 0);
                }
            }
        }
    }
    }

    const float isc = *inv_scale;
    if constexpr (EPI == 0) {
        if (((N | ldc) & 3) == 0 && (reinterpret_cast<uintptr_t>(C) & 15) == 0 && NJ % 2 == 0) {
            const int q = lane & 31;
            __syncthreads();
            float* T = reinterpret_cast<float*>(lds) + wave * (32 * TLD2);
#pragma unroll
            for (int jj = 0; jj < NJ / 2; ++jj) {
                const int cb = n0 + wn + 64 * jj;
                const float bv0 = (bias && cb + q < N) ? bias[cb + q] : 0.f;
                const float bv1 = (bias && cb + 32 + q < N) ? bias[cb + 32 + q] : 0.f;
#pragma unroll
                for (int i = 0; i < MI; ++i) {
#pragma unroll
                    for (int r = 0; r < 16; ++r) {
                        const int lr = (r & 3) + 8 * (r >> 2) + 4 * (lane >> 5);
                        const float sc = isc * rinv[wm + 32 * i + lr];
                        float v0 = acc[i][2 * jj][r] * sc + bv0, v1 = acc[i][2 * jj + 1][r] * sc + bv1;
                        if (ACT) { v0 = ssilu16(v0); v1 = ssilu16(v1); }
                        T[lr * TLD2 + q] = v0;
                        T[lr * TLD2 + 32 + q] = v1;
                    }
                    __builtin_amdgcn_fence(__ATOMIC_RELEASE, "wavefront");
                    __builtin_amdgcn_wave_barrier();
#pragma unroll
                    for (int it = 0; it < 8; ++it) {
                        const int item = lane + 64 * it;
                        const int lr = item >> 4, c4 = item & 15;
                        const int row = m0 + wm + 32 * i + lr, col = cb + 4 * c4;
                        float4 v = *reinterpret_cast<const float4*>(T + lr * TLD2 + 4 * c4);
                        if (row < M && col < N) {
                            if (ep.gate) {
                                const float4 g4 = *reinterpret_cast<const float4*>(ep.gate + (size_t)(row / 3) * ep.gate_ld + col);
                                v.x = g4.x * v.x; v.y = g4.y * v.y; v.z = g4.z * v.z; v.w = g4.w * v.w;
                            }
                            if (ep.accumulate) {
                                const float4 o = *reinterpret_cast<const float4*>(C + (size_t)row * ldc + col);
                                v.x += o.x; v.y += o.y; v.z += o.z; v.w += o.w;
                            }
                            *reinterpret_cast<float4*>(C + (size_t)row * ldc + col) = v;
                        }
                        if (ep.out_mag) {
                            float mg = col < N ? fmaxf(fmaxf(fabsf(v.x), fabsf(v.y)), fmaxf(fabsf(v.z), fabsf(v.w))) : 0.f;
                            mg = adf_row16_max(mg);
                            if (c4 == 0 && row < M) atomicMax(ep.out_mag + row, __float_as_uint(mg));
                        }
                    }
                    __builtin_amdgcn_wave_barrier();
                }
            }
            return;
        }
#pragma unroll
        for (int j = 0; j < NJ; ++j) {
            const int col = n0 + wn + 32 * j + (lane & 31);
            if (col >= N) continue;
            const float bv = bias ? bias[col] : 0.f;
#pragma unroll
            for (int i = 0; i < MI; ++i) {
#pragma unroll
                for (int r = 0; r < 16; ++r) {
                    const int row = m0 + wm + 32 * i + (r & 3) + 8 * (r >> 2) + 4 * (lane >> 5);
                    if (row < M) {
                        float v = acc[i][j][r] * (isc * rinv[row - m0]) + bv;
                        if (ACT) v = ssilu16(v);
                        if (ep.accumulate) v += C[(size_t)row * ldc + col];
                        C[(size_t)row * ldc + col] = v;
                        if (ep.out_mag) atomicMax(ep.out_mag + row, __float_as_uint(fabsf(v)));
                    }
                }
            }
        }
    } else if constexpr (EPI == 3) {
        static_assert(EPI != 3 || (NJ == 2 && MI == 3), "vec_proj epilogue: 3 components x (v1, v2)");
        const int q = lane & 31;
        const int g = (n0 + wn) / 64;
        const int H = ep.H;
        const float inv_sqrt_h = 1.0f / sqrtf((float)H);
        __syncthreads();
        float* T = reinterpret_cast<float*>(lds) + wave * 3200;
        const int a0 = m0 + (wave / NWN) * 32;
        float dv[16], nv[16];
#pragma unroll
        for (int r = 0; r < 16; ++r) {
            const int lr = (r & 3) + 8 * (r >> 2) + 4 * (lane >> 5);
            float d = 0.f, qq = 0.f;
#pragma unroll
            for (int i = 0; i < 3; ++i) {
                const float sc = isc * rinv[wm + 32 * i + lr];
                const float v1 = acc[i][0][r] * sc, v2 = acc[i][1][r] * sc;
                d += v1 * v2;
                qq += v2 * v2;
                T[lr * TLD3 + i * 32 + q] = v1;
            }
            dv[r] = d * inv_sqrt_h;
            nv[r] = sqrtf(qq + 1e-8f);
        }
        __builtin_amdgcn_fence(__ATOMIC_RELEASE, "wavefront");
        __builtin_amdgcn_wave_barrier();
#pragma unroll
        for (int it = 0; it < 4; ++it) {
            const int item = lane + 64 * it;
            const int lr = item >> 3, c4 = item & 7;
            const int n = a0 + lr;
            if (n < M) {
                float* vo = ep.v1 + (size_t)n * 3 * H + 32 * g + 4 * c4;
#pragma unroll
                for (int ax = 0; ax < 3; ++ax) {
                    const float4 tv_ = *reinterpret_cast<const float4*>(T + lr * TLD3 + ax * 32 + 4 * c4);
                    if (G16_ABL & 1) asm volatile("" :: "v"(tv_.x), "v"(tv_.w)); else
                    *reinterpret_cast<float4*>(vo + ax * H) = tv_;
                }
            }
        }
        __builtin_amdgcn_wave_barrier();
#pragma unroll
        for (int r = 0; r < 16; ++r) {
            const int lr = (r & 3) + 8 * (r >> 2) + 4 * (lane >> 5);
            T[lr * TLD3 + q] = dv[r];
            T[lr * TLD3 + 32 + q] = nv[r];
        }
        __builtin_amdgcn_fence(__ATOMIC_RELEASE, "wavefront");
        __builtin_amdgcn_wave_barrier();
#pragma unroll
        for (int it = 0; it < 4; ++it) {
            const int lr = it * 8 + (lane >> 3), c4 = lane & 7;
            const int n = a0 + lr, c = 32 * g + 4 * c4;
            const float4 dv_ = *reinterpret_cast<const float4*>(T + lr * TLD3 + 4 * c4);
            const float4 nv_ = *reinterpret_cast<const float4*>(T + lr * TLD3 + 32 + 4 * c4);
            if (n < M) {
                if (G16_ABL & 1) { asm volatile("" :: "v"(dv_.x), "v"(nv_.w)); } else {
                *reinterpret_cast<float4*>(ep.dotw + (size_t)n * H + c) = dv_;
                *reinterpret_cast<float4*>(ep.cat + (size_t)n * H + c) = nv_;
                }
            }
            if (ep.catpart) {
                const float mg = adf_lane8_max(fmaxf(fmaxf(fmaxf(0.f, fabsf(nv_.x)), fabsf(nv_.y)), fmaxf(fabsf(nv_.z), fabsf(nv_.w))));
                if (c4 == 0 && n < M) ep.catpart[(size_t)g * ep.part_stride + n] = mg;
            }
        }
    } else if constexpr (EPI == 4) {
        static_assert(EPI != 4 || (NJ == 2 && MI == 3), "norm epilogue: 3 components x 64 columns per wave");
        const int q = lane & 31;
        const int cb = n0 + wn;
        __syncthreads();
        float* T = reinterpret_cast<float*>(lds) + wave * 3200;
        const int a0 = m0 + (wave / NWN) * 32;
#pragma unroll
        for (int r = 0; r < 16; ++r) {
            const int lr = (r & 3) + 8 * (r >> 2) + 4 * (lane >> 5);
#pragma unroll
            for (int j = 0; j < 2; ++j) {
                const float a = acc[0][j][r] * (isc * rinv[wm + lr]), b = acc[1][j][r] * (isc * rinv[wm + 32 + lr]),
                            d = acc[2][j][r] * (isc * rinv[wm + 64 + lr]);
                T[lr * TLD2 + j * 32 + q] = sqrtf(a * a + b * b + d * d);
            }
        }
        __builtin_amdgcn_fence(__ATOMIC_RELEASE, "wavefront");
        __builtin_amdgcn_wave_barrier();
#pragma unroll
        for (int it = 0; it < 8; ++it) {
            const int lr = it * 4 + (lane >> 4), c4 = lane & 15;
            const int n = a0 + lr, c = cb + 4 * c4;
            if (n < M && c < N)
                *reinterpret_cast<float4*>(ep.cat + (size_t)n * N + c) = *reinterpret_cast<const float4*>(T + lr * TLD2 + 4 * c4);
        }
    } else {
        static_assert(EPI >= 3 || (NJ == 3 && MI == 2), "fused epilogues are written for the 64 x 96 wave tile");
        if (((EPI_ABL & 1) && EPI == 1) || ((EPI_ABL & 2) && EPI == 2)) {
            float sacc = 0.f;
            for (int i = 0; i < MI; ++i) for (int j = 0; j < NJ; ++j) for (int r = 0; r < 16; ++r) sacc += acc[i][j][r];
            if (ep.H < 0) ep.x[0] = sacc;
            return;
        }
        const int q = lane & 31;
        const int g = (n0 + wn) / 96;
        const int H = ep.H;
        const float b0 = bias[n0 + wn + q], b1 = bias[n0 + wn + 32 + q], b2 = bias[n0 + wn + 64 + q];
        __syncthreads();
        float* T = reinterpret_cast<float*>(lds) + wave * 3200;
#pragma unroll
        for (int i = 0; i < MI; ++i) {
#pragma unroll
            for (int r = 0; r < 16; ++r) {
                const int lr = (r & 3) + 8 * (r >> 2) + 4 * (lane >> 5);
                const float sc = isc * rinv[wm + 32 * i + lr];
                T[lr * TLD3 + q] = acc[i][0][r] * sc + b0;
                T[lr * TLD3 + 32 + q] = acc[i][1][r] * sc + b1;
                T[lr * TLD3 + 64 + q] = acc[i][2][r] * sc + b2;
            }
            __builtin_amdgcn_fence(__ATOMIC_RELEASE, "wavefront");
            __builtin_amdgcn_wave_barrier();
            const int c4 = lane & 7;
            const int c = 32 * g + 4 * c4;
            if constexpr (EPI == 1) {
                float4 v0[4], v1[4], v2[4];
                if (EPI_ABL & 4) { for (int it = 0; it < 4; ++it) { v0[it] = make_float4(1.f, 2.f, 3.f, 4.f); v1[it] = v0[it]; v2[it] = v0[it]; } }
                else if (!ep.vec_is_zero) {
#pragma unroll
                    for (int it = 0; it < 4; ++it) {
                        const int n = min(m0 + wm + 32 * i + it * 8 + (lane >> 3), M - 1);
                        const float* vr = ep.vec_in + (size_t)n * 3 * H + c;
                        v0[it] = *reinterpret_cast<const float4*>(vr);
                        v1[it] = *reinterpret_cast<const float4*>(vr + H);
                        v2[it] = *reinterpret_cast<const float4*>(vr + 2 * H);
                    }
                }
#pragma unroll
                for (int it = 0; it < 4; ++it) {
                    const int lr = it * 8 + (lane >> 3);
                    const int n = m0 + wm + 32 * i + lr;
                    const float4 p0 = *reinterpret_cast<const float4*>(T + lr * TLD3 + 4 * c4);
                    const float4 p1 = *reinterpret_cast<const float4*>(T + lr * TLD3 + 32 + 4 * c4);
                    const float4 p2 = *reinterpret_cast<const float4*>(T + lr * TLD3 + 64 + 4 * c4);
                    float4 o[4];
                    if (!ep.vec_is_zero) {
                        o[0] = make_float4(v0[it].x * p1.x, v1[it].x * p1.x, v2[it].x * p1.x, p0.x);
                        o[1] = make_float4(v0[it].y * p1.y, v1[it].y * p1.y, v2[it].y * p1.y, p0.y);
                        o[2] = make_float4(v0[it].z * p1.z, v1[it].z * p1.z, v2[it].z * p1.z, p0.z);
                        o[3] = make_float4(v0[it].w * p1.w, v1[it].w * p1.w, v2[it].w * p1.w, p0.w);
                    } else {
                        o[0] = make_float4(0.f, 0.f, 0.f, p0.x);
                        o[1] = make_float4(0.f, 0.f, 0.f, p0.y);
                        o[2] = make_float4(0.f, 0.f, 0.f, p0.z);
                        o[3] = make_float4(0.f, 0.f, 0.f, p0.w);
                    }
                    float4* X = reinterpret_cast<float4*>(lds + LDS_MAIN) + wave * 256;
#pragma unroll
                    for (int k = 0; k < 4; ++k) X[lane * 4 + k] = o[k];
                    __builtin_amdgcn_fence(__ATOMIC_RELEASE, "wavefront");
                    __builtin_amdgcn_wave_barrier();
#pragma unroll
                    for (int k = 0; k < 4; ++k) o[k] = X[(lane >> 3) * 32 + 8 * k + c4];
                    __builtin_amdgcn_wave_barrier();
                    if ((EPI_ABL & 8) && n >= 0) { if (ep.H < 0) ep.rec[0] = p2.x + o[0].x + o[1].y + o[2].z + o[3].w; }
                    else if (n < M) {
                        float* rec = ep.rec + ((size_t)(ep.row_map ? ep.row_map[n] : n) * (H / 32) + g) * 160;
#pragma unroll
                        for (int k = 0; k < 4; ++k) *reinterpret_cast<float4*>(rec + 32 * k + 4 * c4) = o[k];
                        *reinterpret_cast<float4*>(rec + 128 + 4 * c4) = p2;
                    }
                }
            } else {
                float4 d[4], xv[4], w1[4][3], tv[4][3];
#pragma unroll
                for (int it = 0; it < 4; ++it) {
                    const int n = min(m0 + wm + 32 * i + it * 8 + (lane >> 3), M - 1);
                    const size_t xo = (size_t)n * H + c;
#if EPI2_POLICY & 2
                    typedef float f32x4_t __attribute__((ext_vector_type(4)));
                    auto ntld = [](const float* p_) { const f32x4_t v = __builtin_nontemporal_load(reinterpret_cast<const f32x4_t*>(p_));
                                                      return make_float4(v.x, v.y, v.z, v.w); };
#define EPI2_LD(p_) ntld(p_)
#else
#define EPI2_LD(p_) (*reinterpret_cast<const float4*>(p_))
#endif
                    d[it] = EPI2_LD(ep.dot + xo);
                    xv[it] = EPI2_LD(ep.x + xo);
                    const float* vr = ep.vec + (size_t)n * 3 * H + c;
                    const float* v1p = ep.vv + (size_t)n * 3 * H + c;
#pragma unroll
                    for (int ax = 0; ax < 3; ++ax) {
                        w1[it][ax] = EPI2_LD(v1p + ax * H);
                        tv[it][ax] = EPI2_LD(vr + ax * H);
                    }
                }
#pragma unroll
                for (int it = 0; it < 4; ++it) {
                    const int lr = it * 8 + (lane >> 3);
                    const int n = m0 + wm + 32 * i + lr;
                    const float4 p0 = *reinterpret_cast<const float4*>(T + lr * TLD3 + 4 * c4);
                    const float4 p1 = *reinterpret_cast<const float4*>(T + lr * TLD3 + 32 + 4 * c4);
                    const float4 p2 = *reinterpret_cast<const float4*>(T + lr * TLD3 + 64 + 4 * c4);
                    const float k2 = 0.70710678118654752f, sc = ep.scale;
                    float4 xo4 = xv[it];
                    xo4.x = (xo4.x + (p0.x + p1.x * d[it].x) * k2) * sc;
                    xo4.y = (xo4.y + (p0.y + p1.y * d[it].y) * k2) * sc;
                    xo4.z = (xo4.z + (p0.z + p1.z * d[it].z) * k2) * sc;
                    xo4.w = (xo4.w + (p0.w + p1.w * d[it].w) * k2) * sc;
#undef EPI2_LD
#if EPI2_POLICY & 1
                    typedef unsigned int u32x4 __attribute__((ext_vector_type(4)));
                    const auto rx = __builtin_amdgcn_make_buffer_rsrc(ep.x, 0, (int)((unsigned int)M * (unsigned int)H * 4u), 0x00020000);
                    const auto rv = __builtin_amdgcn_make_buffer_rsrc(ep.vec, 0, (int)((unsigned int)M * 3u * (unsigned int)H * 4u), 0x00020000);
#define EPI2_ST(r_, p_, base_, v_) __builtin_amdgcn_raw_buffer_store_b128(__builtin_bit_cast(u32x4, v_), r_, (int)(((p_) - (base_)) * 4), 0, 16)
#else
#define EPI2_ST(r_, p_, base_, v_) (*reinterpret_cast<float4*>(p_) = (v_))
#endif
                    if (n < M) {
                        EPI2_ST(rx, ep.x + (size_t)n * H + c, ep.x, xo4);
                        float* vr = ep.vec + (size_t)n * 3 * H + c;
#pragma unroll
                        for (int ax = 0; ax < 3; ++ax) {
                            float4 t = tv[it][ax];
                            const float4 v1 = w1[it][ax];
                            t.x += p2.x * v1.x; t.y += p2.y * v1.y; t.z += p2.z * v1.z; t.w += p2.w * v1.w;
                            EPI2_ST(rv, vr + ax * H, ep.vec, t);
                        }
                    }
#undef EPI2_ST
                }
            }
            __builtin_amdgcn_wave_barrier();
        }
    }
}

__global__ __launch_bounds__(256) void adf_rowmag_kernel(const float* __restrict__ A, int lda, int K1,
                                                         const float* __restrict__ A2, int K2, long long M,
                                                         float* __restrict__ mag, const int32_t* __restrict__ m_dev,
                                                         int m_mul) {
    const long long r = (long long)blockIdx.x * 4 + (threadIdx.x >> 6);
    const int lane = threadIdx.x & 63;
    if (r >= M || (m_dev && r >= (long long)*m_dev * m_mul)) return;
    float mx = 0.f;
    const float* a = A + (size_t)r * lda;
    for (int k = lane * 4; k < K1; k += 256) {
        const float4 v = *reinterpret_cast<const float4*>(a + k);
        mx = fmaxf(fmaxf(fmaxf(mx, fabsf(v.x)), fabsf(v.y)), fmaxf(fabsf(v.z), fabsf(v.w)));
    }
    if (A2) {
        const float* b = A2 + (size_t)r * lda;
        for (int k = lane * 4; k < K2; k += 256) {
            const float4 v = *reinterpret_cast<const float4*>(b + k);
            mx = fmaxf(fmaxf(fmaxf(mx, fabsf(v.x)), fabsf(v.y)), fmaxf(fabsf(v.z), fabsf(v.w)));
        }
    }
#pragma unroll
    for (int o = 32; o > 0; o >>= 1) mx = fmaxf(mx, __shfl_xor(mx, o));
    if (lane == 0) mag[r] = mx;
}

__global__ __launch_bounds__(256) void adf_rowmax_combine_kernel(const float* __restrict__ part, long long stride, int nparts,
                                                                 long long M, float* __restrict__ mag,
                                                                 const int32_t* __restrict__ m_dev, int m_mul) {
    const long long r = (long long)blockIdx.x * 256 + threadIdx.x;
    if (r >= M || (m_dev && r >= (long long)*m_dev * m_mul)) return;
    float mx = 0.f;
    for (int p = 0; p < nparts; ++p) mx = fmaxf(mx, part[(size_t)p * stride + r]);
    mag[r] = mx;
}

int32_t adf_launch_rowmax_combine(const float* part, long long stride, int nparts, long long M, float* mag, hipStream_t s,
                                  const int32_t* m_dev, int m_mul) {
    if (M <= 0) return ADF_OK;
    hipLaunchKernelGGL(adf_rowmax_combine_kernel, dim3((unsigned)((M + 255) / 256)), dim3(256), 0, s, part, stride, nparts, M,
                       mag, m_dev, m_mul);
    ADF_HIP_CHECK(hipGetLastError());
    return ADF_OK;
}

int32_t adf_launch_rowmag(const float* A, int lda, int K1, const float* A2, int K2, long long M, float* mag, hipStream_t s,
                          const int32_t* m_dev, int m_mul) {
    if (M <= 0) return ADF_OK;
    hipLaunchKernelGGL(adf_rowmag_kernel, dim3((unsigned)((M + 3) / 4)), dim3(256), 0, s, A, lda, K1, A2, K2, M, mag, m_dev,
                       m_mul);
    ADF_HIP_CHECK(hipGetLastError());
    return ADF_OK;
}

static int32_t lift_mags(const float* A, int lda, int K1, const float* A2, int K2, long long rows, const adf_lift* lf,
                         const float* premag, const float** out, hipStream_t s, const int32_t* m_dev = nullptr, int m_mul = 1) {
    *out = premag;
    if (!premag && lf && lf->buf) {
        if (rows > lf->cap) { adf_set_error("gemm16: lift scratch holds %lld rows, need %lld", lf->cap, rows); return ADF_EINVAL; }
        ADF_TRY(adf_launch_rowmag(A, lda, K1, A2, K2, rows, lf->buf, s, m_dev, m_mul));
        *out = lf->buf;
    }
    return ADF_OK;
}

__global__ void adf_absmax_kernel(const float* __restrict__ w, long long n, unsigned int* out_bits) {
    float m = 0.f;
    for (long long i = (long long)blockIdx.x * blockDim.x + threadIdx.x; i < n; i += (long long)gridDim.x * blockDim.x)
        m = fmaxf(m, fabsf(w[i]));
#pragma unroll
    for (int o = 32; o > 0; o >>= 1) m = fmaxf(m, __shfl_xor(m, o));
    if ((threadIdx.x & 63) == 0) atomicMax(out_bits, __float_as_uint(m));
}

__global__ void adf_split_kernel(const float* __restrict__ w, long long n, const unsigned int* absmax_bits,
                                 _Float16* __restrict__ hi, _Float16* __restrict__ lo, float* inv_scale, int perm_H,
                                 int K, const float* __restrict__ bias, float* __restrict__ bias_perm, int parts) {
    const float amax = __uint_as_float(*absmax_bits);
    int e = 0;
    if (amax > 0.f) (void)frexpf(amax, &e);
    const float scale = ldexpf(1.0f, 10 - e);
    if (blockIdx.x == 0 && threadIdx.x == 0) *inv_scale = 1.0f / scale;
    for (long long i = (long long)blockIdx.x * blockDim.x + threadIdx.x; i < n; i += (long long)gridDim.x * blockDim.x) {
        long long src = i;
        if (perm_H > 0) {
            const long long prow = i / K;
            const int k = (int)(i - prow * K);
            const int gw = 32 * parts;
            const int g = (int)(prow / gw), part = (int)((prow % gw) / 32), qq = (int)(prow % 32);
            const long long orow = (long long)part * perm_H + 32 * g + qq;
            src = orow * K + k;
            if (k == 0 && bias_perm) bias_perm[prow] = bias ? bias[orow] : 0.f;
        }
        const float v = w[src] * scale;
        const _Float16 h = (_Float16)v;
        hi[i] = h;
        lo[i] = (_Float16)(v - (float)h);
    }
}

int32_t adf_split_weight(const float* w, long long n, adf_w16* out, unsigned int* scratch_bits, hipStream_t s,
                         int perm_H, int K, const float* bias, int parts) {
    ADF_HIP_CHECK(hipMemsetAsync(scratch_bits, 0, sizeof(unsigned int), s));
    hipLaunchKernelGGL(adf_absmax_kernel, dim3(64), dim3(256), 0, s, w, n, scratch_bits);
    hipLaunchKernelGGL(adf_split_kernel, dim3(64), dim3(256), 0, s, w, n, scratch_bits, (_Float16*)out->hi,
                       (_Float16*)out->lo, out->inv_scale, perm_H, K, bias, out->bias_perm, parts);
    ADF_HIP_CHECK(hipGetLastError());
    return ADF_OK;
}

__global__ void adf_pack_frag_kernel(const _Float16* __restrict__ hi, const _Float16* __restrict__ lo, half8* __restrict__ out,
                                     int N, int K) {
    const int nks = K / 16;
    const long long total = (long long)(N / 32) * nks * 2 * 64;
    for (long long i = (long long)blockIdx.x * blockDim.x + threadIdx.x; i < total; i += (long long)gridDim.x * blockDim.x) {
        const int lane = (int)(i & 63), plane = (int)((i >> 6) & 1);
        const long long cs = i >> 7;
        const int s = (int)(cs % nks), cb = (int)(cs / nks);
        const _Float16* src = (plane ? lo : hi) + (size_t)(32 * cb + (lane & 31)) * K + 16 * s + 8 * (lane >> 5);
        out[i] = *reinterpret_cast<const half8*>(src);
    }
}

int32_t adf_pack_frag(const adf_w16* w, int N, int K, void* out, hipStream_t s) {
    if (N % 32 || K % 16) { adf_set_error("pack_frag: N %% 32 or K %% 16"); return ADF_EINVAL; }
    hipLaunchKernelGGL(adf_pack_frag_kernel, dim3(256), dim3(256), 0, s, (const _Float16*)w->hi, (const _Float16*)w->lo,
                       (half8*)out, N, K);
    ADF_HIP_CHECK(hipGetLastError());
    return ADF_OK;
}

static int32_t check_a_span(long long rows, int lda) {
    if (rows * (long long)lda * 4 >= (1ll << 32)) {
        adf_set_error("gemm16: A operand of %lld rows x %d exceeds the 32-bit offset range, split the batch", rows, lda);
        return ADF_EOOM;
    }
    return ADF_OK;
}

int32_t adf_launch_gemm16(const float* A, int lda, const adf_w16* W, const float* bias, float* C, int ldc, int M,
                          int N, int K, int act_ssilu, const adf_epi* ep_in, hipStream_t s, const adf_lift* lf,
                          const adf_tune& tune, int num_cus) {
    if (M <= 0) return ADF_OK;
    adf_epi ep = {};
    if (ep_in) ep = *ep_in;
    if (!ep.A2) ep.K1 = 0;
    if (K % HK != 0 || (lda & 3) || (ep.A2 && (ep.K1 <= 0 || ep.K1 % HK != 0 || ep.K1 >= K))) {
        adf_set_error("gemm16: K=%d (K1=%d) must be multiples of %d and lda a multiple of 4", K, ep.K1, HK);
        return ADF_EINVAL;
    }
    ADF_TRY(check_a_span(M, lda));
    const int mi = tune.gemm16_mi;
    const int TM = 64 * mi, TN = 256;
    const int tiles_n = (N + TN - 1) / TN;
    const int tiles_m = (M + TM - 1) / TM;
    const int tiles_m8 = (tiles_m + 7) / 8 * 8;
    dim3 grid((unsigned)(tiles_m8 * tiles_n));
    if (ep.gate && (((N | ldc | ep.gate_ld) & 3) || (((uintptr_t)C | (uintptr_t)ep.gate) & 15))) {
        adf_set_error("gemm16: the gate epilogue needs N, ldc and gate_ld multiples of 4 and 16-byte aligned C and gate");
        return ADF_EINVAL;
    }
    ADF_TRY(lift_mags(A, lda, ep.A2 ? ep.K1 : K, ep.A2, ep.A2 ? K - ep.K1 : 0, M, lf, ep.rmag, &ep.rmag, s, ep.m_dev, 1));
    if (ep.out_mag) ADF_HIP_CHECK(hipMemsetAsync(ep.out_mag, 0, sizeof(float) * (size_t)M, s));
    const int ncu = num_cus > 0 ? num_cus : 256;
    const long long wg8 = (long long)((M + 191) / 192) * (N / 256 > 0 ? N / 256 : 1);
    const bool ragged = wg8 < 4ll * ncu && wg8 % ncu != 0 && wg8 % ncu < (3 * ncu) / 10 && wg8 > ncu;
    const long long wg4 = (long long)((M + 95) / 96) * (N / 256 > 0 ? N / 256 : 1), slots4 = 2ll * ncu;
    const bool ragged4 = wg4 < 4 * slots4 && wg4 % slots4 != 0 && wg4 % slots4 < (3 * slots4) / 10 && wg4 > slots4;
    if ((tune.gemm_rows4 & 1) && tune.gemm_w8_plain && W->frag && N % 256 == 0 && (K / HK) % 2 == 0 && mi == 2 && !ragged4) {
        const int tn4 = N / 256, tmw4 = ((M + 95) / 96 + 7) / 8 * 8;
        dim3 g4((unsigned)(tmw4 * tn4));
        if (act_ssilu)
            hipLaunchKernelGGL((adf_gemm_f16x3_kernel<1, 3, 2, 0, true, 4, 1>), g4, dim3(256), 0, s, A, lda, (const _Float16*)W->frag,
                               (const _Float16*)nullptr, W->inv_scale, bias, C, ldc, M, N, K, tn4, ep);
        else
            hipLaunchKernelGGL((adf_gemm_f16x3_kernel<0, 3, 2, 0, true, 4, 1>), g4, dim3(256), 0, s, A, lda, (const _Float16*)W->frag,
                               (const _Float16*)nullptr, W->inv_scale, bias, C, ldc, M, N, K, tn4, ep);
        ADF_HIP_CHECK(hipGetLastError());
        return ADF_OK;
    }
    if (!(tune.gemm_rows4 & 1) && tune.gemm_w8_plain && W->frag && N % 256 == 0 && (K / HK) % 2 == 0 && mi == 2 && !ragged) {
        const int tn8 = N / 256, tmw8 = ((M + 191) / 192 + 7) / 8 * 8;
        dim3 g8((unsigned)(tmw8 * tn8));
        if (act_ssilu)
            hipLaunchKernelGGL((adf_gemm_f16x3_kernel<1, 3, 2, 0, true, 4>), g8, dim3(512), 0, s, A, lda, (const _Float16*)W->frag,
                               (const _Float16*)nullptr, W->inv_scale, bias, C, ldc, M, N, K, tn8, ep);
        else
            hipLaunchKernelGGL((adf_gemm_f16x3_kernel<0, 3, 2, 0, true, 4>), g8, dim3(512), 0, s, A, lda, (const _Float16*)W->frag,
                               (const _Float16*)nullptr, W->inv_scale, bias, C, ldc, M, N, K, tn8, ep);
        ADF_HIP_CHECK(hipGetLastError());
        return ADF_OK;
    }
#define LAUNCH16(ACT_, MI_)                                                                                  \
    hipLaunchKernelGGL((adf_gemm_f16x3_kernel<ACT_, MI_, 4, 0>), grid, dim3(256), 0, s, A, lda,              \
                       (const _Float16*)W->hi, (const _Float16*)W->lo, W->inv_scale, bias, C, ldc, M, N, K, \
                       tiles_n, ep)
    if (mi == 4) { if (act_ssilu) LAUNCH16(1, 4); else LAUNCH16(0, 4); }
    else { if (act_ssilu) LAUNCH16(1, 2); else LAUNCH16(0, 2); }
#undef LAUNCH16
    ADF_HIP_CHECK(hipGetLastError());
    return ADF_OK;
}

int32_t adf_launch_gemm16_vecnorm(const float* A, int lda, const adf_w16* W, float* nrm, int M, int N, int K,
                                  hipStream_t s, const adf_tune& tune, const adf_lift* lf, const float* premag) {
    if (M <= 0) return ADF_OK;
    if (K % HK != 0 || (lda & 3) || (N & 3)) { adf_set_error("gemm16_vecnorm: bad shape"); return ADF_EINVAL; }
    ADF_TRY(check_a_span(3ll * M, lda));
    adf_epi ep = {};
    ep.cat = nrm;
    ADF_TRY(lift_mags(A, lda, K, nullptr, 0, 3ll * M, lf, premag, &ep.rmag, s));
    const int tn = (N + 127) / 128, tm8 = ((M + 63) / 64 + 7) / 8 * 8;
    if ((tune.gemm_rows4 & 1) && tune.gemm_w8 && W->frag && N % 256 == 0 && (K / HK) % 2 == 0) {
        const int tm4 = ((M + 31) / 32 + 7) / 8 * 8;
        hipLaunchKernelGGL((adf_gemm_f16x3_kernel<0, 3, 2, 4, true, 4, 1>), dim3((unsigned)(tm4 * (N / 256))), dim3(256), 0, s, A, lda,
                           (const _Float16*)W->frag, (const _Float16*)nullptr, W->inv_scale, (const float*)nullptr,
                           (float*)nullptr, 0, M, N, K, N / 256, ep);
        ADF_HIP_CHECK(hipGetLastError());
        return ADF_OK;
    }
    if (tune.gemm_w8 && W->frag && N % 256 == 0 && (K / HK) % 2 == 0) {
        hipLaunchKernelGGL((adf_gemm_f16x3_kernel<0, 3, 2, 4, true, 4>), dim3((unsigned)(tm8 * (N / 256))), dim3(512), 0, s, A, lda,
                           (const _Float16*)W->frag, (const _Float16*)nullptr, W->inv_scale, (const float*)nullptr,
                           (float*)nullptr, 0, M, N, K, N / 256, ep);
        ADF_HIP_CHECK(hipGetLastError());
        return ADF_OK;
    }
    hipLaunchKernelGGL((adf_gemm_f16x3_kernel<0, 3, 2, 4>), dim3((unsigned)(tm8 * tn)), dim3(256), 0, s, A, lda,
                       (const _Float16*)W->hi, (const _Float16*)W->lo, W->inv_scale, (const float*)nullptr,
                       (float*)nullptr, 0, M, N, K, tn, ep);
    ADF_HIP_CHECK(hipGetLastError());
    return ADF_OK;
}

int32_t adf_launch_gemm16_fused(const float* A, int lda, const adf_w16* W, int M, int H, int K, int epi,
                                const adf_epi* ep_in, hipStream_t s, const adf_tune& tune, const adf_lift* lf) {
    adf_epi epv = *ep_in;
    const adf_epi* ep = &epv;
    if (M <= 0) return ADF_OK;
    if (K % HK != 0 || (lda & 3) || H % 64 != 0 || (epi != 3 && !W->bias_perm)) {
        adf_set_error("gemm16_fused: bad shape");
        return ADF_EINVAL;
    }
    ADF_TRY(check_a_span(epi == 3 ? 3ll * M : (long long)M, lda));
    ADF_TRY(lift_mags(A, lda, K, nullptr, 0, epi == 3 ? 3ll * M : (long long)M, lf, ep_in->rmag, &epv.rmag, s, ep_in->m_dev,
                      epi == 3 ? 3 : 1));
    const int N = 3 * H, TM = 128, TN = 192;
    const int tiles_n = N / TN;
    const int tiles_m = (M + TM - 1) / TM;
    const int tiles_m8 = (tiles_m + 7) / 8 * 8;
    dim3 grid((unsigned)(tiles_m8 * tiles_n));
    if (epi == 3) {
        const int tn = 2 * H / 128, tm8 = ((M + 63) / 64 + 7) / 8 * 8;
        if ((tune.gemm_rows4 & 1) && tune.gemm_wreg && W->frag && tune.gemm_w8 && (2 * H) % 256 == 0 && (K / HK) % 2 == 0)
            hipLaunchKernelGGL((adf_gemm_f16x3_kernel<0, 3, 2, 3, true, 4, 1>), dim3((unsigned)(((M + 31) / 32 + 7) / 8 * 8 * (2 * H / 256))),
                               dim3(256), 0, s, A, lda, (const _Float16*)W->frag, (const _Float16*)nullptr, W->inv_scale,
                               (const float*)nullptr, (float*)nullptr, 0, M, 2 * H, K, 2 * H / 256, *ep);
        else if (tune.gemm_wreg && W->frag && tune.gemm_w8 && (2 * H) % 256 == 0 && (K / HK) % 2 == 0)
            hipLaunchKernelGGL((adf_gemm_f16x3_kernel<0, 3, 2, 3, true, 4>), dim3((unsigned)(tm8 * (2 * H / 256))), dim3(512), 0, s,
                               A, lda, (const _Float16*)W->frag, (const _Float16*)nullptr, W->inv_scale, (const float*)nullptr,
                               (float*)nullptr, 0, M, 2 * H, K, 2 * H / 256, *ep);
        else
        hipLaunchKernelGGL((adf_gemm_f16x3_kernel<0, 3, 2, 3>), dim3((unsigned)(tm8 * tn)), dim3(256), 0, s, A, lda,
                           (const _Float16*)W->hi, (const _Float16*)W->lo, W->inv_scale, (const float*)nullptr,
                           (float*)nullptr, 0, M, 2 * H, K, tn, *ep);
        ADF_HIP_CHECK(hipGetLastError());
        return ADF_OK;
    }
    const int wf = tune.gemm_wr_fused;
    if ((tune.gemm_rows4 & 2) && wf == 2 && W->frag && (K / HK) % 2 == 0 && N % 384 == 0) {
        dim3 g4((unsigned)(((M + 63) / 64 + 7) / 8 * 8 * (N / 384)));
        if (epi == 1)
            hipLaunchKernelGGL((adf_gemm_f16x3_kernel<0, 2, 3, 1, true, 4, 1>), g4, dim3(256), 0, s, A, lda, (const _Float16*)W->frag,
                               (const _Float16*)nullptr, W->inv_scale, W->bias_perm, (float*)nullptr, 0, M, N, K, N / 384, *ep);
        else
            hipLaunchKernelGGL((adf_gemm_f16x3_kernel<0, 2, 3, 2, true, 4, 1>), g4, dim3(256), 0, s, A, lda, (const _Float16*)W->frag,
                               (const _Float16*)nullptr, W->inv_scale, W->bias_perm, (float*)nullptr, 0, M, N, K, N / 384, *ep);
        ADF_HIP_CHECK(hipGetLastError());
        return ADF_OK;
    }
    if (wf && W->frag && (K / HK) % 2 == 0 && (wf == 2 || N % 384 == 0)) {
        const int tnw = wf == 4 ? N / 384 : tiles_n;
        dim3 gw((unsigned)(tiles_m8 * tnw));
#define LAUNCHWF(EPI_, NWN_)                                                                                                  \
        hipLaunchKernelGGL((adf_gemm_f16x3_kernel<0, 2, 3, EPI_, true, NWN_>), gw, dim3(128 * NWN_), 0, s, A, lda,            \
                           (const _Float16*)W->frag, (const _Float16*)nullptr, W->inv_scale, W->bias_perm, (float*)nullptr, 0, \
                           M, N, K, tnw, *ep)
        if (epi == 1) { if (wf == 4) LAUNCHWF(1, 4); else LAUNCHWF(1, 2); }
        else { if (wf == 4) LAUNCHWF(2, 4); else LAUNCHWF(2, 2); }
#undef LAUNCHWF
        ADF_HIP_CHECK(hipGetLastError());
        return ADF_OK;
    }
    if (epi == 1)
        hipLaunchKernelGGL((adf_gemm_f16x3_kernel<0, 2, 3, 1>), grid, dim3(256), 0, s, A, lda, (const _Float16*)W->hi,
                           (const _Float16*)W->lo, W->inv_scale, W->bias_perm, (float*)nullptr, 0, M, N, K, tiles_n, *ep);
    else
        hipLaunchKernelGGL((adf_gemm_f16x3_kernel<0, 2, 3, 2>), grid, dim3(256), 0, s, A, lda, (const _Float16*)W->hi,
                           (const _Float16*)W->lo, W->inv_scale, W->bias_perm, (float*)nullptr, 0, M, N, K, tiles_n, *ep);
    ADF_HIP_CHECK(hipGetLastError());
    return ADF_OK;
}
```

### adsorbdiff_amd/csrc/nodewise.hip

```cpp
#include "common.h"

__device__ __forceinline__ float ssilu_d(float x) {
    float s = x / (1.0f + expf(-x));
    return s * 1.6666666666666667f;
}

__global__ void adf_embed_kernel(const float* __restrict__ emb, const int32_t* __restrict__ Z, float* __restrict__ x,
                                 int N, int H, int num_elements, int32_t* flags) {
    const int h4 = H / 4;
    const long long total = (long long)N * h4;
    for (long long i = (long long)blockIdx.x * blockDim.x + threadIdx.x; i < total;
         i += (long long)gridDim.x * blockDim.x) {
        const int n = (int)(i / h4), c = (int)(i - (long long)n * h4);
        int z = Z[n] - 1;
        if (z < 0 || z >= num_elements) { if (c == 0) atomicExch(&flags[4], 1); z = min(max(z, 0), num_elements - 1); }
        const float4 v = reinterpret_cast<const float4*>(emb + (size_t)z * H)[c];
        reinterpret_cast<float4*>(x + (size_t)n * H)[c] = v;
    }
}

__global__ __launch_bounds__(256) void adf_layernorm_kernel(const float* __restrict__ x, const float* __restrict__ w,
                                                             const float* __restrict__ b, float* __restrict__ y,
                                                             int N, int H, float* __restrict__ out_mag,
                                                             const int32_t* __restrict__ n_dev) {
// ... 80 lines not shown
         i += (long long)gridDim.x * blockDim.x) {
        const int n = (int)(i / h4), c = (int)(i - (long long)n * h4);
        const float4* hr = reinterpret_cast<const float4*>(h3 + (size_t)n * 3 * H);
        const float4 a = hr[c], b = hr[h4 + c], g = hr[2 * h4 + c];
        const float4 d = reinterpret_cast<const float4*>(dot + (size_t)n * H)[c];
        float4* xr = reinterpret_cast<float4*>(x + (size_t)n * H) + c;
        float4 xv = *xr;
        xv.x = (xv.x + (a.x + b.x * d.x) * inv_sqrt2) * scale;
        xv.y = (xv.y + (a.y + b.y * d.y) * inv_sqrt2) * scale;
        xv.z = (xv.z + (a.z + b.z * d.z) * inv_sqrt2) * scale;
        xv.w = (xv.w + (a.w + b.w * d.w) * inv_sqrt2) * scale;
        *xr = xv;
        const float4* vb = reinterpret_cast<const float4*>(vv + (size_t)n * 6 * H);
        float4* vr = reinterpret_cast<float4*>(vec + (size_t)n * 3 * H);
#pragma unroll
        for (int ax = 0; ax < 3; ++ax) {
            const float4 v1 = vb[ax * 2 * h4 + c];
            float4 t = vr[ax * h4 + c];
            t.x += g.x * v1.x; t.y += g.y * v1.y; t.z += g.z * v1.z; t.w += g.w * v1.w;
            vr[ax * h4 + c] = t;
        }
    }
}

__global__ void adf_head_norm_cat_kernel(const float* __restrict__ xin, const float* __restrict__ t1,
                                         float* __restrict__ cat, int N, int C) {
    const int c4 = C / 4;
    const long long total = (long long)N * c4;
    for (long long i = (long long)blockIdx.x * blockDim.x + threadIdx.x; i < total;
         i += (long long)gridDim.x * blockDim.x) {
        const int n = (int)(i / c4), c = (int)(i - (long long)n * c4);
        const float4* tb = reinterpret_cast<const float4*>(t1 + (size_t)n * 3 * C);
        const float4 a = tb[c], b = tb[c4 + c], d = tb[2 * c4 + c];
        float4* cr = reinterpret_cast<float4*>(cat + (size_t)n * 2 * C);
        cr[c] = reinterpret_cast<const float4*>(xin + (size_t)n * C)[c];
        cr[c4 + c] = make_float4(sqrtf(a.x * a.x + b.x * b.x + d.x * d.x), sqrtf(a.y * a.y + b.y * b.y + d.y * d.y),
                                 sqrtf(a.z * a.z + b.z * b.z + d.z * d.z), sqrtf(a.w * a.w + b.w * b.w + d.w * d.w));
    }
}

__global__ void adf_head_gate_kernel(const float* __restrict__ o, const float* __restrict__ t2,
                                     float* __restrict__ xout, float* __restrict__ vout, int N, int Cout) {
    const int c4 = Cout / 4;
    const long long total = (long long)N * c4;
    for (long long i = (long long)blockIdx.x * blockDim.x + threadIdx.x; i < total;
         i += (long long)gridDim.x * blockDim.x) {
        const int n = (int)(i / c4), c = (int)(i - (long long)n * c4);
        const float4* orow = reinterpret_cast<const float4*>(o + (size_t)n * 2 * Cout);
        const float4 xs = orow[c], g = orow[c4 + c];
        reinterpret_cast<float4*>(xout + (size_t)n * Cout)[c] =
            make_float4(ssilu_d(xs.x), ssilu_d(xs.y), ssilu_d(xs.z), ssilu_d(xs.w));
        const float4* tb = reinterpret_cast<const float4*>(t2 + (size_t)n * 3 * Cout);
        float4* vb = reinterpret_cast<float4*>(vout + (size_t)n * 3 * Cout);
#pragma unroll
        for (int ax = 0; ax < 3; ++ax) {
            const float4 t = tb[ax * c4 + c];
            vb[ax * c4 + c] = make_float4(g.x * t.x, g.y * t.y, g.z * t.z, g.w * t.w);
        }
    }
}

__global__ void adf_head_xact_kernel(const float* __restrict__ o, float* __restrict__ xout, int N, int Cout) {
    const int c4 = Cout / 4;
    const long long total = (long long)N * c4;
    for (long long i = (long long)blockIdx.x * blockDim.x + threadIdx.x; i < total;
         i += (long long)gridDim.x * blockDim.x) {
        const int n = (int)(i / c4), c = (int)(i - (long long)n * c4);
        const float4 xs = reinterpret_cast<const float4*>(o + (size_t)n * 2 * Cout)[c];
        reinterpret_cast<float4*>(xout + (size_t)n * Cout)[c] =
            make_float4(ssilu_d(xs.x), ssilu_d(xs.y), ssilu_d(xs.z), ssilu_d(xs.w));
    }
}

__global__ __launch_bounds__(256) void adf_head_final_kernel(const float* __restrict__ u, const float* __restrict__ v,
                                                              const float* __restrict__ w_vec2,
                                                              const float* __restrict__ un2_w,
                                                              const float* __restrict__ un2_b, float* __restrict__ out,
                                                              int N, int C, int32_t* flags) {
    const int lane = threadIdx.x & 63;
    const int n = blockIdx.x * 4 + (threadIdx.x >> 6);
    if (n >= N) return;
    float g = 0.f, t0 = 0.f, t1 = 0.f, t2 = 0.f;
    for (int c = lane; c < C; c += 64) {
        const float w2 = w_vec2[c];
        g += u[(size_t)n * C + c] * un2_w[C + c];
        t0 += v[((size_t)n * 3 + 0) * C + c] * w2;
        t1 += v[((size_t)n * 3 + 1) * C + c] * w2;
        t2 += v[((size_t)n * 3 + 2) * C + c] * w2;
    }
#pragma unroll
    for (int o = 32; o > 0; o >>= 1) {
        g += __shfl_xor(g, o); t0 += __shfl_xor(t0, o); t1 += __shfl_xor(t1, o); t2 += __shfl_xor(t2, o);
    }
    if (lane == 0) {
        g += un2_b[1];
        out[(size_t)n * 3 + 0] = g * t0;
        out[(size_t)n * 3 + 1] = g * t1;
        out[(size_t)n * 3 + 2] = g * t2;
        const float s3 = g * t0 + g * t1 + g * t2;
        if (!(fabsf(s3) <= 3.0e38f)) atomicExch(&flags[5], 1);
    }
}

static inline unsigned ew_grid(long long total) {
    long long b = (total + 255) / 256;
    if (b > 256 * 8) b = 256 * 8;
    if (b < 1) b = 1;
    return (unsigned)b;
}

int32_t adf_nodewise_embed(adf_painn* h, const int32_t* Z, int N, float* x, hipStream_t s) {
    const int H = h->hp.hidden_channels;
    hipLaunchKernelGGL(adf_embed_kernel, dim3(ew_grid((long long)N * H / 4)), dim3(256), 0, s, h->emb, Z, x, N, H,
                       h->hp.num_elements, h->flags);
    ADF_HIP_CHECK(hipGetLastError());
    return ADF_OK;
}

int32_t adf_nodewise_layernorm(const float* x, const float* w, const float* b, float* y, int N, int H, hipStream_t s,
                               float* out_mag, const int32_t* n_dev) {
    hipLaunchKernelGGL(adf_layernorm_kernel, dim3((N + 3) / 4), dim3(256), 0, s, x, w, b, y, N, H, out_mag, n_dev);
    ADF_HIP_CHECK(hipGetLastError());
    return ADF_OK;
}

int32_t adf_nodewise_update_prep(const float* vv, const float* x, float* cat, float* dot, int N, int H, hipStream_t s) {
    hipLaunchKernelGGL(adf_update_prep_kernel, dim3(ew_grid((long long)N * H / 4)), dim3(256), 0, s, vv, x, cat, dot, N, H);
    ADF_HIP_CHECK(hipGetLastError());
    return ADF_OK;
}

int32_t adf_nodewise_update_apply(const float* h3, const float* dot, const float* vv, float* x, float* vec,
                                  float scale, int N, int H, hipStream_t s) {
    hipLaunchKernelGGL(adf_update_apply_kernel, dim3(ew_grid((long long)N * H / 4)), dim3(256), 0, s, h3, dot, vv, x,
                       vec, scale, N, H);
    ADF_HIP_CHECK(hipGetLastError());
    return ADF_OK;
}

int32_t adf_head_forward(adf_painn* h, int head, int N, const float* x, const float* vec, float* out, hipStream_t s) {
    const int H = h->hp.hidden_channels, H2 = H / 2;
    const adf_block_weights& b0 = h->head[head][0];
    const adf_block_weights& b1 = h->head[head][1];
    float* t1 = h->vv;
    float* t2 = h->vv + (size_t)3 * N * H;
    float* v1 = t2 + (size_t)3 * N * H2;
    float* o = h->xh;
    float* x1 = h->xh + (size_t)N * H;
    float* t1b = x1 + (size_t)N * H2;
    float* cat1 = h->dot;
    const bool lift = h->lift_on && !h->gemm_f32;
    const adf_lift* lf = lift ? &h->lift : nullptr;
    const float* vmag = nullptr;
    if (lift) {
        if (head == 0 || !h->mag_v3_valid) ADF_TRY(adf_launch_rowmag(vec, H, H, nullptr, 0, 3ll * N, h->mag_v3, s));
        h->mag_v3_valid = head == 0;
        vmag = h->mag_v3;
    }
    if (h->gemm_f32) {
        ADF_TRY(adf_linear(h, vec, H, b0.vec1_w, &b0.vec1_16, nullptr, t1, H, 3 * N, H, H, 0, s));
        hipLaunchKernelGGL(adf_head_norm_cat_kernel, dim3(ew_grid((long long)N * H / 4)), dim3(256), 0, s, x, t1, h->cat, N, H);
    } else {
        ADF_TRY(adf_launch_gemm16_vecnorm(vec, H, &b0.vec1_16, h->cat, N, H, H, s, h->tune, lf, vmag));
    }
    const bool fg = h->tune.head_gate_fused && !h->gemm_f32 && (H2 & 3) == 0;
    if (!fg) ADF_TRY(adf_linear(h, vec, H, b0.vec2_w, &b0.vec2_16, nullptr, t2, H2, 3 * N, H2, H, 0, s, vmag));
    if (h->gemm_f32) ADF_TRY(adf_linear(h, h->cat, 2 * H, b0.un0_w, &b0.un0_16, b0.un0_b, h->y, H, N, H, 2 * H, 1, s));
    else {
        adf_epi e0 = {};
        e0.A2 = h->cat; e0.K1 = H;
        e0.out_mag = h->lift_on ? reinterpret_cast<unsigned int*>(h->mag_b) : nullptr;
        ADF_TRY(adf_launch_gemm16(x, H, &b0.un0_16, b0.un0_b, h->y, H, N, H, 2 * H, 1, &e0, s, h->lift_on ? &h->lift : nullptr,
                                  h->tune, h->num_cus));
    }
    ADF_TRY(adf_linear(h, h->y, H, b0.un2_w, &b0.un2_16, b0.un2_b, o, H, N, H, H, 0, s, (h->lift_on && !h->gemm_f32) ? h->mag_b : nullptr));
    if (fg) {
        adf_epi eg = {};
        eg.rmag = vmag;
        eg.out_mag = lift ? reinterpret_cast<unsigned int*>(h->lift.buf) : nullptr;
        eg.gate = o + H2; eg.gate_ld = H;
        ADF_TRY(adf_launch_gemm16(vec, H, &b0.vec2_16, nullptr, v1, H2, 3 * N, H2, H, 0, &eg, s, lf, h->tune, h->num_cus));
        hipLaunchKernelGGL(adf_head_xact_kernel, dim3(ew_grid((long long)N * H2 / 4)), dim3(256), 0, s, o, x1, N, H2);
    } else
    hipLaunchKernelGGL(adf_head_gate_kernel, dim3(ew_grid((long long)N * H2 / 4)), dim3(256), 0, s, o, t2, x1, v1, N, H2);
    if (h->gemm_f32) {
        ADF_TRY(adf_linear(h, v1, H2, b1.vec1_w, &b1.vec1_16, nullptr, t1b, H2, 3 * N, H2, H2, 0, s));
        hipLaunchKernelGGL(adf_head_norm_cat_kernel, dim3(ew_grid((long long)N * H2 / 4)), dim3(256), 0, s, x1, t1b, cat1, N, H2);
        ADF_TRY(adf_linear(h, cat1, H, b1.un0_w, &b1.un0_16, b1.un0_b, h->y, H2, N, H2, H, 1, s));
    } else {
        ADF_TRY(adf_launch_gemm16_vecnorm(v1, H2, &b1.vec1_16, cat1, N, H2, H2, s, h->tune, h->lift_on ? &h->lift : nullptr,
                                          (fg && lift) ? h->lift.buf : nullptr));
        adf_epi e1 = {};
        e1.A2 = cat1; e1.K1 = H2;
        ADF_TRY(adf_launch_gemm16(x1, H2, &b1.un0_16, b1.un0_b, h->y, H2, N, H2, H, 1, &e1, s, h->lift_on ? &h->lift : nullptr,
                                  h->tune, h->num_cus));
    }
    hipLaunchKernelGGL(adf_head_final_kernel, dim3((N + 3) / 4), dim3(256), 0, s, h->y, v1, b1.vec2_w, b1.un2_w,
                       b1.un2_b, out, N, H2, h->flags);
    ADF_HIP_CHECK(hipGetLastError());
    return ADF_OK;
}
```

### adsorbdiff_amd/lib.py

```python
from __future__ import annotations

import ctypes as C
from pathlib import Path

ADF_OK, ADF_EINVAL, ADF_EOOM, ADF_ENONEIGHBOR, ADF_EHIP, ADF_EOVERFLOW, ADF_ENUMERIC = 0, 1, 2, 3, 4, 5, 6


class NumericRangeError(ArithmeticError):
    """Non-finite model output (ADF_ENUMERIC).  Not a RuntimeError on purpose: ``ml_diffuse`` must not answer it by
    splitting the batch; the engine answers it by re-running in exact f32."""

EXPORTS = (
    "adf_painn_create", "adf_painn_destroy", "adf_painn_set_weights", "adf_graph_build", "adf_graph_set_moving",
    "adf_check_flags", "adf_painn_set_arithmetic", "adf_painn_set_incremental", "adf_painn_get_tune",
    "adf_graph_export", "adf_painn_forward", "adf_painn_forward_subset", "adf_linear_forward", "adf_painn_message_layer", "adf_painn_update_layer",
    "adf_painn_debug_row_maxima",
    "adf_sde_init_placement", "adf_sde_step", "adf_sde_step_scheduled", "adf_sample", "adf_sample_traj",
    "adf_tr_step", "adf_tr_sample", "adf_tr_sample_traj",
    "adf_painn_set_energy_head", "adf_painn_set_distance_floor", "adf_painn_forward_energy",
    "adf_painn_forward_energy_gradient", "adf_painn_energy_gradient_workspace",
    "adf_lbfgs_create", "adf_lbfgs_destroy", "adf_lbfgs_reset", "adf_lbfgs_converge", "adf_lbfgs_step",
    "adf_lbfgs_get_mask", "adf_lbfgs_last_step_max", "adf_lbfgs_set_per_system", "adf_lbfgs_get_step_state",
    "adf_lbfgs_active_build", "adf_active_gather", "adf_active_scatter",
    "adf_frames_create", "adf_frames_destroy", "adf_frames_push", "adf_frames_wait", "adf_frames_release", "adf_frames_pushed", "adf_frames_abort",
    "adf_get_counters", "adf_profile_enable", "adf_profile_read", "adf_measure_peaks",
    "adf_lift_adsorbates", "adf_flag_anomalies", "adf_select_best_sites", "adf_comm_unique_id", "adf_comm_create", "adf_comm_destroy", "adf_allgather_sites",
    "adf_op_linear_fwd", "adf_op_linear_bwd_scratch", "adf_op_linear_bwd", "adf_op_ssilu_fwd", "adf_op_ssilu_bwd", "adf_op_layernorm_fwd", "adf_op_layernorm_bwd", "adf_op_embed_fwd", "adf_op_embed_bwd", "adf_op_rbf", "adf_op_message_fwd", "adf_op_message_fwd_fused", "adf_op_message_bwd", "adf_op_message_bwd_fused", "adf_op_message_bwd_fused_supported", "adf_op_message_bwd_perm", "adf_op_edge_owner", "adf_op_rbf_image_bytes", "adf_op_rbf_image", "adf_op_rbf_wgrad_fused_scratch", "adf_op_rbf_wgrad_fused", "adf_op_vdot_fwd", "adf_op_vdot_bwd", "adf_op_update_out_fwd", "adf_op_update_out_bwd", "adf_op_vnorm_fwd", "adf_op_vnorm_bwd", "adf_op_gate_fwd", "adf_op_gate_bwd", "adf_op_copy_rows", "adf_op_score_loss", "adf_op_score_loss_tr", "adf_op_s2ef_loss", "adf_op_s2ef_loss_scratch", "adf_op_energy_sum", "adf_op_energy_head_bwd", "adf_op_energy_head_bwd_scratch", "adf_op_sqnorm_accumulate", "adf_op_adamw_step",
    "adf_noise_draws", "adf_noise_tr_so3", "adf_noise_com", "adf_igso3_score_norm",
    "adf_eval_scratch", "adf_eval_s2ef", "adf_eval_is2rs", "adf_eval_is2re", "adf_eval_add",
    "adf_eqv2_create", "adf_eqv2_destroy", "adf_eqv2_set_constants", "adf_eqv2_set_weights", "adf_eqv2_set_arithmetic",
    "adf_eqv2_set_energy_embedding", "adf_eqv2_set_system_energy",
    "adf_eqv2_set_weights_s2ef", "adf_eqv2_set_energy_head", "adf_eqv2_forward_energy", "adf_eqv2_radial_first_layer",
    "adf_eqv2_set_edges", "adf_eqv2_set_moving", "adf_eqv2_set_incremental", "adf_eqv2_forward", "adf_eqv2_forward_subset", "adf_eqv2_check_flags", "adf_eqv2_init_placement",
    "adf_eqv2_sde_step", "adf_eqv2_sample", "adf_eqv2_sample_traj", "adf_eqv2_tr_step", "adf_eqv2_tr_sample", "adf_eqv2_tr_sample_traj", "adf_eqv2_linear_forward", "adf_eqv2_get_counters", "adf_eqv2_profile_enable", "adf_eqv2_profile_read",
    "adf_last_error", "adf_version",
)


class Hparams(C.Structure):
    _fields_ = [
        ("hidden_channels", C.c_int32), ("num_layers", C.c_int32), ("num_rbf", C.c_int32),
        ("num_elements", C.c_int32), ("max_neighbors", C.c_int32), ("envelope_exponent", C.c_int32),
        ("num_heads", C.c_int32), ("cutoff", C.c_float),
    ]


class EqV2Hparams(C.Structure):
    _fields_ = [
        ("lmax", C.c_int32), ("mmax", C.c_int32), ("num_layers", C.c_int32), ("sphere_channels", C.c_int32),
        ("attn_hidden_channels", C.c_int32), ("num_heads", C.c_int32), ("attn_alpha_channels", C.c_int32),
        ("attn_value_channels", C.c_int32), ("ffn_hidden_channels", C.c_int32), ("grid_resolution", C.c_int32),
        ("edge_channels", C.c_int32), ("num_distance_basis", C.c_int32), ("max_num_elements", C.c_int32),
        ("max_neighbors", C.c_int32), ("max_radius", C.c_float), ("avg_degree", C.c_float),
    ]


class EqV2Counters(C.Structure):
    _fields_ = [("num_edges", C.c_int64), ("num_atoms", C.c_int64), ("dense_flops", C.c_int64), ("conv_flops", C.c_int64),
                ("inc_rows", C.c_int64), ("inc_rows_full", C.c_int64), ("forwards_total", C.c_int64),
                ("conv_flops_total", C.c_int64)]


class Tune(C.Structure):
    _fields_ = [(name, C.c_int32) for name in (
        "gemm16_mi", "gemm_w8_plain", "gemm_w8", "gemm_wreg", "gemm_wr_fused", "head_gate_fused", "lift_emit",
        "graph_sys_csr", "train_gemm16", "wgrad_f32",
        "eqv2_pw_mi", "eqv2_gemm_tile256", "eqv2_rotin_generic", "eqv2_rotout_generic",
        "gemm_rows4")]


class BatchDesc(C.Structure):
    _fields_ = [
        ("num_systems", C.c_int32), ("num_atoms", C.c_int32), ("pos", C.c_void_p), ("cell", C.c_void_p),
        ("atomic_numbers", C.c_void_p), ("batch", C.c_void_p), ("atom_offset", C.c_void_p), ("reps", C.c_int32 * 3),
    ]


class ActiveField(C.Structure):
    _fields_ = [("src", C.c_void_p), ("dst", C.c_void_p), ("row_bytes", C.c_int32), ("per_system", C.c_int32)]


class StepCoef(C.Structure):
    _fields_ = [
        ("coef_tr", C.c_float), ("rot_pre", C.c_float), ("rot_dt", C.c_float), ("rot_g2", C.c_float),
        ("noise_tr", C.c_float), ("noise_rot", C.c_float),
    ]


class TrCoef(C.Structure):
    _fields_ = [("coef", C.c_float), ("noise", C.c_float)]


class Counters(C.Structure):
    _fields_ = [
        ("num_edges", C.c_int64), ("num_atoms", C.c_int64), ("message_bytes_per_layer", C.c_int64),
        ("dense_flops", C.c_int64),
        ("inc_rows", C.c_int64), ("inc_rows_full", C.c_int64), ("inc_msg_launches", C.c_int64),
        ("inc_msg_edges", C.c_int64),
    ]


_LIB = None


def lib_path() -> Path:
    import os

    override = os.environ.get("ADF_LIB_PATH")
    if override:
        return Path(override)
    return Path(__file__).resolve().parent / "libadsorbdiff_hip.so"


def load():
    global _LIB
    if _LIB is not None:
        return _LIB
    path = lib_path()
    if not path.exists():
        raise RuntimeError(
            f"{path} not found: build it with `python -m adsorbdiff_amd.build` "
            "(the HIP path has no CPU fallback)"
        )
    lib = C.CDLL(str(path))
    vp, i32, i64 = C.c_void_p, C.c_int32, C.c_int64
    lib.adf_last_error.restype = C.c_char_p
    lib.adf_version.restype = C.c_char_p
    sigs = {
        "adf_painn_create": [C.POINTER(Hparams), C.POINTER(vp)],
        "adf_painn_destroy": [vp],
        "adf_painn_set_weights": [vp, i32, C.POINTER(vp), C.POINTER(C.c_float), vp],
        "adf_graph_build": [vp, C.POINTER(BatchDesc), vp, C.POINTER(i64)],
        "adf_graph_set_moving": [vp, vp, vp, vp],
        "adf_check_flags": [vp, vp],
        "adf_painn_set_arithmetic": [vp, i32],
        "adf_painn_set_incremental": [vp, i32],
        "adf_painn_get_tune": [vp, C.POINTER(Tune)],
        "adf_graph_export": [vp, vp, vp, vp, i64, vp, vp, vp, vp, C.POINTER(i64), vp],
        "adf_painn_forward": [vp, C.POINTER(BatchDesc), vp, vp, vp],
        "adf_painn_forward_subset": [vp, C.POINTER(BatchDesc), vp, i32, vp, vp, vp],
        "adf_painn_message_layer": [vp, i32, i32, vp, vp, vp, vp, vp],
        "adf_linear_forward": [vp, vp, vp, vp, i32, i32, i32, i32, i32, vp],
        "adf_painn_update_layer": [vp, i32, i32, vp, vp, vp],
        "adf_painn_debug_row_maxima": [vp, i32, vp, C.c_int64, C.POINTER(i32), vp],
        "adf_sde_init_placement": [vp, C.POINTER(BatchDesc), vp, vp, vp, vp],
        "adf_sde_step": [vp, C.POINTER(BatchDesc), vp, vp, vp, vp, vp, C.POINTER(StepCoef), vp, vp, i32, vp, vp, vp, vp],
        "adf_sde_step_scheduled": [vp, C.POINTER(BatchDesc), vp, vp, vp, vp, vp, vp, i32, vp, vp, i32, vp, vp, vp, vp],
        "adf_tr_step": [vp, C.POINTER(BatchDesc), vp, vp, vp, C.POINTER(TrCoef), vp, i32, vp, i32, vp, vp, vp],
        "adf_tr_sample": [vp, C.POINTER(BatchDesc), vp, vp, vp, i32, vp, i32, i32, vp, vp, i32, vp, vp],
        "adf_tr_sample_traj": [vp, C.POINTER(BatchDesc), vp, vp, vp, i32, vp, i32, i32, vp, vp, i32, vp, vp, i32, vp],
        "adf_eqv2_tr_step": [vp, C.POINTER(BatchDesc), vp, vp, vp, C.POINTER(TrCoef), vp, i32, vp, i32, vp, vp, vp],
        "adf_eqv2_tr_sample": [vp, C.POINTER(BatchDesc), vp, vp, vp, i32, vp, i32, i32, vp, vp, i32, vp, vp],
        "adf_eqv2_tr_sample_traj": [vp, C.POINTER(BatchDesc), vp, vp, vp, i32, vp, i32, i32, vp, vp, i32, vp, vp, i32, vp],
        "adf_painn_set_energy_head": [vp, i32, C.POINTER(vp), vp],
        "adf_painn_set_distance_floor": [vp, C.c_float],
        "adf_painn_forward_energy": [vp, C.POINTER(BatchDesc), vp, vp, vp],
        "adf_painn_forward_energy_gradient": [vp, C.POINTER(BatchDesc), vp, vp, vp],
        "adf_painn_energy_gradient_workspace": [vp, i64, C.POINTER(i64)],
        "adf_lbfgs_create": [i64, i32, i32, C.c_double, C.c_double, C.c_double, i32, C.POINTER(vp)],
        "adf_lbfgs_destroy": [vp],
        "adf_lbfgs_reset": [vp, vp],
        "adf_lbfgs_converge": [vp, vp, vp, C.c_double, vp, vp, vp],
        "adf_lbfgs_step": [vp, vp, vp, vp, i64, vp],
        "adf_lbfgs_get_mask": [vp, vp, vp],
        "adf_lbfgs_last_step_max": [vp, vp, vp],
        "adf_lbfgs_set_per_system": [vp, i32],
        "adf_lbfgs_get_step_state": [vp, vp, vp, vp],
        "adf_lbfgs_active_build": [vp, vp, vp, vp, vp, vp],
        "adf_active_gather": [vp, vp, vp, vp, i32, i64, C.POINTER(ActiveField), i32, vp, vp, vp],
        "adf_active_scatter": [vp, vp, vp, vp, i32, i64, vp, vp, i32, vp, vp, vp, vp, vp],
        "adf_get_counters": [vp, C.POINTER(Counters), vp],
        "adf_profile_enable": [vp, i32],
        "adf_profile_read": [vp, C.POINTER(C.c_float), C.POINTER(i64), C.POINTER(i64), vp],
        "adf_measure_peaks": [C.POINTER(C.c_float), vp],
        "adf_lift_adsorbates": [vp, vp, vp, i32, C.c_float, vp, vp],
        "adf_flag_anomalies": [C.POINTER(BatchDesc), vp, vp, vp, vp, i32, C.c_float, C.c_float, C.c_float, vp, vp],
        "adf_select_best_sites": [vp, vp, vp, i32, vp, vp, vp, vp],
        "adf_comm_unique_id": [vp],
        "adf_comm_create": [vp, i32, i32, C.POINTER(vp)],
        "adf_comm_destroy": [vp],
        "adf_allgather_sites": [vp, vp, i64, vp, vp],
        "adf_op_linear_fwd": [vp, i32, vp, vp, vp, i32, i64, i32, i32, vp],
        "adf_op_linear_bwd": [vp, i32, vp, vp, i32, vp, i32, i32, vp, vp, i32, i64, i32, i32, vp, vp],
        "adf_op_ssilu_fwd": [vp, vp, i64, vp],
        "adf_op_ssilu_bwd": [vp, vp, vp, i64, vp],
        "adf_op_layernorm_fwd": [vp, vp, vp, vp, vp, i32, i32, vp],
        "adf_op_layernorm_bwd": [vp, vp, vp, vp, vp, vp, vp, i32, i32, vp, vp],
        "adf_op_embed_fwd": [vp, vp, i32, vp, vp],
        "adf_op_embed_bwd": [vp, vp, vp, i32, i32, vp],
        "adf_op_rbf": [vp, vp, vp],
        "adf_op_message_fwd": [vp, vp, vp, vp, vp, vp, vp, i32, vp],
        "adf_op_message_fwd_fused": [vp, i32, vp, vp, vp, vp, vp, i32, vp],
        "adf_op_message_bwd": [vp, vp, vp, vp, vp, vp, vp, vp, vp, vp, i32, vp],
        "adf_op_message_bwd_fused": [vp, i32, vp, vp, vp, vp, vp, vp, C.c_int64, vp, vp, i32, vp, vp],
        "adf_op_edge_owner": [vp, vp, C.c_int64, vp],
        "adf_op_rbf_image": [vp, vp, C.c_int64, vp, vp],
        "adf_op_rbf_wgrad_fused": [vp, vp, vp, vp, vp, C.c_int64, vp, vp, i32, vp],
        "adf_op_message_bwd_fused_supported": [vp],
        "adf_op_message_bwd_perm": [vp, vp, i32],
        "adf_op_vdot_fwd": [vp, vp, vp, i32, i64, i32, C.c_float, vp],
        "adf_op_vdot_bwd": [vp, vp, i32, vp, vp, i32, vp, vp, i64, i32, vp],
        "adf_op_update_out_fwd": [vp, vp, vp, vp, vp, C.c_float, vp, vp, i64, i32, vp],
        "adf_op_update_out_bwd": [vp, vp, vp, C.c_float, vp, vp, vp, vp, vp, vp, vp, i64, i32, vp],
        "adf_op_vnorm_fwd": [vp, vp, i32, i64, i32, vp],
        "adf_op_vnorm_bwd": [vp, vp, i32, vp, i32, vp, i64, i32, vp],
        "adf_op_gate_fwd": [vp, vp, vp, i32, vp, i64, i32, vp],
        "adf_op_gate_bwd": [vp, vp, vp, i32, vp, vp, vp, i64, i32, vp],
        "adf_op_copy_rows": [vp, i32, vp, i32, i64, i32, i32, vp],
        "adf_op_score_loss": [vp, vp, vp, vp, vp, vp, vp, vp, vp, vp, vp, vp, i32, vp, vp],
        "adf_op_score_loss_tr": [vp, vp, vp, vp, vp, vp, vp, i32, vp, vp],
        "adf_noise_draws": [i64, i32, vp, i32, vp, vp],
        "adf_noise_tr_so3": [vp, vp, vp, vp, i32, i32, vp, C.c_float, C.c_float, C.c_float, C.c_float, vp, vp, vp, vp, i32, i32,
                             vp, vp, vp, vp, vp, vp, vp, vp],
        "adf_noise_com": [vp, vp, vp, vp, i32, i32, vp, C.c_float, C.c_float, vp, vp, vp, vp, vp],
        "adf_igso3_score_norm": [vp, vp, i32, i32, vp, vp],
        "adf_op_s2ef_loss": [vp, vp, vp, vp, vp, vp, i32, i32, C.c_float, C.c_float, C.c_float, C.c_float, C.c_float, C.c_float,
                             vp, vp, vp, vp, vp, vp, vp],
        "adf_op_energy_sum": [vp, i32, vp, vp, vp, vp, i32, vp],
        "adf_op_energy_head_bwd": [vp, vp, vp, vp, vp, vp, vp, i32, i64, i32, vp, vp],
        "adf_op_sqnorm_accumulate": [vp, i64, vp, vp],
        "adf_op_adamw_step": [vp, vp, vp, vp, vp, i64, vp, C.c_float, C.c_float, C.c_float, C.c_float, C.c_float, C.c_float, i32, C.c_float, vp],
# ... 74 lines not shown
```

### include/adsorbdiff_hip.h

```cpp
#ifndef ADSORBDIFF_HIP_H
#define ADSORBDIFF_HIP_H

#include <stdint.h>

#ifdef __cplusplus
extern "C" {
#endif

#define ADF_OK 0
#define ADF_EINVAL 1
#define ADF_EOOM 2
#define ADF_ENONEIGHBOR 3
#define ADF_EHIP 4
#define ADF_EOVERFLOW 5
#define ADF_ENUMERIC 6

typedef struct adf_painn* adf_painn_t;

typedef struct {
    int32_t hidden_channels;
    int32_t num_layers;
    int32_t num_rbf;
    int32_t num_elements;
    int32_t max_neighbors;
    int32_t envelope_exponent;
    int32_t num_heads;
    float cutoff;
} adf_painn_hparams;

#define ADF_WEIGHTS_PER_LAYER 13
#define ADF_WEIGHTS_PER_HEAD 12

int32_t adf_painn_create(const adf_painn_hparams* hp, adf_painn_t* out);
int32_t adf_painn_destroy(adf_painn_t h);

int32_t adf_painn_set_weights(adf_painn_t h, int32_t n_weights, const void* const* weights,
                              const float* scale_factors, void* stream);

typedef struct {
    int32_t num_systems;
    int32_t num_atoms;
    const float* pos;
    const float* cell;
    const int32_t* atomic_numbers;
    const int32_t* batch;
    const int32_t* atom_offset;
    int32_t reps[3];
} adf_batch;

int32_t adf_graph_build(adf_painn_t h, const adf_batch* b, void* stream, int64_t* num_edges);

int32_t adf_graph_set_moving(adf_painn_t h, const int32_t* moving, const int32_t* mov_idx, const int32_t* mov_off);

int32_t adf_painn_set_arithmetic(adf_painn_t h, int32_t exact_f32);

int32_t adf_painn_set_incremental(adf_painn_t h, int32_t on);

typedef struct adf_tune {
    int32_t gemm16_mi;
    int32_t gemm_w8_plain;
    int32_t gemm_w8;
    int32_t gemm_wreg;
    int32_t gemm_wr_fused;
    int32_t head_gate_fused;
    int32_t lift_emit;
    int32_t graph_sys_csr;
    int32_t train_gemm16;
    int32_t wgrad_f32;
    int32_t eqv2_pw_mi;
    int32_t eqv2_gemm_tile256;
    int32_t eqv2_rotin_generic;
    int32_t eqv2_rotout_generic;
    int32_t gemm_rows4;
} adf_tune;
int32_t adf_painn_get_tune(adf_painn_t h, adf_tune* out);

int32_t adf_check_flags(adf_painn_t h, void* stream);

int32_t adf_graph_export(adf_painn_t h, int32_t* nbr_count, int32_t* nbr_src, int32_t* nbr_shift,
                         int64_t edge_capacity, int32_t* edge_src, int32_t* edge_dst, float* edge_dist,
                         float* edge_vec, int64_t* num_edges, void* stream);

int32_t adf_painn_forward(adf_painn_t h, const adf_batch* b, float* f1, float* f2, void* stream);

int32_t adf_painn_forward_subset(adf_painn_t h, const adf_batch* b, const int32_t* out_idx, int32_t n_out, float* f1,
                                 float* f2, void* stream);

int32_t adf_painn_message_layer(adf_painn_t h, int32_t layer, int32_t num_atoms, const float* x,
                                const float* vec, float* x_out, float* vec_out, void* stream);
int32_t adf_painn_update_layer(adf_painn_t h, int32_t layer, int32_t num_atoms, float* x, float* vec,
                               void* stream);
int32_t adf_painn_debug_row_maxima(adf_painn_t h, int32_t which, float* out, int64_t capacity, int32_t* rows,
                                   void* stream);

int32_t adf_linear_forward(const float* A, const float* W, const float* bias, float* C, int32_t M, int32_t N,
                           int32_t K, int32_t act_ssilu, int32_t mode, void* stream);

typedef struct {
    float coef_tr;
    float rot_pre;
    float rot_dt;
    float rot_g2;
    float noise_tr;
    float noise_rot;
} adf_step_coef;

int32_t adf_sde_init_placement(adf_painn_t h, const adf_batch* b, float* pos, const int32_t* tags,
                               const float* noise, void* stream);

int32_t adf_sde_step(adf_painn_t h, const adf_batch* b, float* pos, const int32_t* tags,
                     const int32_t* fixed, const float* f1, const float* f2, const adf_step_coef* coef,
                     const float* z_tr, const float* z_rot, int32_t early_stop_count, int32_t* state,
                     float* dcom, float* drot, void* stream);

int32_t adf_sde_step_scheduled(adf_painn_t h, const adf_batch* b, float* pos, const int32_t* tags,
                               const int32_t* fixed, const float* f1, const float* f2,
                               const adf_step_coef* coefs_dev, int32_t num_steps, const float* z_tr,
                               const float* z_rot, int32_t early_stop_count, int32_t* state, float* dcom,
                               float* drot, void* stream);

int32_t adf_sample(adf_painn_t h, const adf_batch* b, float* pos, const int32_t* tags, const int32_t* fixed,
                   const adf_step_coef* coefs_dev, int32_t num_steps, const float* z_tr_all, const float* z_rot_all,
                   int32_t early_stop_count, int32_t poll_every, int32_t* state, const int32_t* out_idx,
                   int32_t n_out, float* f1, float* f2, void* stream);

typedef struct {
    float coef;
    float noise;
} adf_tr_coef;

int32_t adf_tr_step(adf_painn_t h, const adf_batch* b, float* pos, const int32_t* tags, const float* f1,
                    const adf_tr_coef* coef, const adf_tr_coef* coefs_dev, int32_t num_steps, const float* z,
                    int32_t early_stop_count, int32_t* state, float* dcom, void* stream);
int32_t adf_tr_sample(adf_painn_t h, const adf_batch* b, float* pos, const int32_t* tags, const adf_tr_coef* coefs_dev,
                      int32_t num_steps, const float* z_all, int32_t early_stop_count, int32_t poll_every,
                      int32_t* state, const int32_t* out_idx, int32_t n_out, float* f1, void* stream);

typedef struct {
    int64_t num_edges;
    int64_t num_atoms;
    int64_t message_bytes_per_layer;
    int64_t dense_flops;
    int64_t inc_rows, inc_rows_full, inc_msg_launches, inc_msg_edges;
} adf_counters;
int32_t adf_get_counters(adf_painn_t h, adf_counters* out, void* stream);

#define ADF_PROF_NCAT 5
int32_t adf_profile_enable(adf_painn_t h, int32_t on);
int32_t adf_profile_read(adf_painn_t h, float* ms, int64_t* count, int64_t* message_ksteps, void* stream);

int32_t adf_measure_peaks(float* out_host3, void* stream);

typedef struct adf_frames* adf_frames_t;
int32_t adf_frames_create(int32_t device, int64_t frame_floats, int32_t slots, adf_frames_t* out);
int32_t adf_frames_destroy(adf_frames_t f);
int32_t adf_frames_push(adf_frames_t f, const float* src, void* stream);
int32_t adf_frames_wait(adf_frames_t f, int64_t index, int32_t timeout_ms, const float** host_ptr);
int32_t adf_frames_release(adf_frames_t f, int64_t index);
int64_t adf_frames_pushed(adf_frames_t f);
int32_t adf_frames_abort(adf_frames_t f);
int32_t adf_sample_traj(adf_painn_t h, const adf_batch* b, float* pos, const int32_t* tags, const int32_t* fixed,
                        const adf_step_coef* coefs_dev, int32_t num_steps, const float* z_tr_all, const float* z_rot_all,
                        int32_t early_stop_count, int32_t poll_every, int32_t* state, const int32_t* out_idx,
                        int32_t n_out, float* f1, float* f2, adf_frames_t sink, int32_t frame_every, void* stream);
int32_t adf_tr_sample_traj(adf_painn_t h, const adf_batch* b, float* pos, const int32_t* tags,
                           const adf_tr_coef* coefs_dev, int32_t num_steps, const float* z_all, int32_t early_stop_count,
                           int32_t poll_every, int32_t* state, const int32_t* out_idx, int32_t n_out, float* f1,
                           adf_frames_t sink, int32_t frame_every, void* stream);

int32_t adf_lift_adsorbates(float* pos, const int32_t* tags, const int32_t* atom_offset, int32_t B, float min_gap,
                            float* lifted, void* stream);

int32_t adf_flag_anomalies(const adf_batch* b, const float* pos_final, const float* pos_slab_ref, const int32_t* tags,
                           const float* radii, int32_t num_radii, float skin, float surface_mult, float desorption_mult,
                           int32_t* flags, void* stream);

int32_t adf_select_best_sites(const float* energy, const int32_t* flags, const int32_t* group_offset, int32_t num_groups,
                              int32_t* best, float* best_energy, int32_t* n_valid, void* stream);

#define ADF_COMM_ID_BYTES 128
typedef struct adf_comm* adf_comm_t;
int32_t adf_comm_unique_id(uint8_t* out128);
int32_t adf_comm_create(const uint8_t* id128, int32_t rank, int32_t world, adf_comm_t* out);
int32_t adf_comm_destroy(adf_comm_t comm);
int32_t adf_allgather_sites(adf_comm_t comm, const void* local, int64_t bytes_per_rank, void* out, void* stream);

int32_t adf_op_linear_fwd(const float* A, int32_t lda, const float* W, const float* bias, float* C, int32_t ldc, int64_t M,
                          int32_t N, int32_t K, void* stream);
int64_t adf_op_linear_bwd_scratch(int64_t M, int32_t N, int32_t K);
int32_t adf_op_linear_bwd(const float* A, int32_t lda, const float* W, const float* dC, int32_t ldc, float* dA, int32_t ldda,
                          int32_t acc_dA, float* dW, float* db, int32_t acc_dW, int64_t M, int32_t N, int32_t K,
                          float* scratch, void* stream);
int32_t adf_op_ssilu_fwd(const float* h, float* y, int64_t n, void* stream);
int32_t adf_op_ssilu_bwd(const float* h, const float* dy, float* dh, int64_t n, void* stream);
int32_t adf_op_layernorm_fwd(const float* x, const float* w, const float* b, float* y, float* stats, int32_t N, int32_t H,
                             void* stream);
int32_t adf_op_layernorm_bwd(const float* x, const float* w, const float* stats, const float* dy, float* dx, float* dw,
                             float* db, int32_t N, int32_t H, float* scratch, void* stream);
int32_t adf_op_embed_fwd(adf_painn_t h, const int32_t* Z, int32_t N, float* x, void* stream);
int32_t adf_op_embed_bwd(const float* dx, const int32_t* Z, float* demb, int32_t N, int32_t H, void* stream);
int32_t adf_op_rbf(adf_painn_t h, float* rbf, void* stream);
int32_t adf_op_message_fwd(adf_painn_t h, const float* xh, const float* vec, const float* rbfh, const float* x, float* x1,
                           float* vec1, int32_t vec_is_zero, void* stream);
int32_t adf_op_message_fwd_fused(adf_painn_t h, int32_t layer, const float* xh, const float* vec, const float* x, float* x1,
                                 float* vec1, int32_t vec_is_zero, void* stream);
int32_t adf_op_message_bwd(adf_painn_t h, const float* xh, const float* vec, const float* rbfh, const float* gx1,
                           const float* gv1, float* dxh, float* drbfh, float* dvec, float* dx, int32_t vec_is_zero,
                           void* stream);
int32_t adf_op_message_bwd_fused_supported(adf_painn_t h);
int32_t adf_op_message_bwd_perm(adf_painn_t h, int32_t* perm_host, int32_t n);
int32_t adf_op_message_bwd_fused(adf_painn_t h, int32_t layer, const float* xh, const float* vec, const float* gx1,
                                 const float* gv1, float* dxh, float* drbfh_lane_order, int64_t num_edges, float* dvec,
                                 float* dx, int32_t vec_is_zero, float* dbias_rows, void* stream);
int32_t adf_op_edge_owner(adf_painn_t h, int32_t* edge_owner, int64_t num_edges, void* stream);
int64_t adf_op_rbf_image_bytes(int64_t num_edges);
int32_t adf_op_rbf_image(adf_painn_t h, const float* rbf, int64_t num_edges, void* image, void* stream);
int64_t adf_op_rbf_wgrad_fused_scratch(adf_painn_t h);
int32_t adf_op_rbf_wgrad_fused(adf_painn_t h, const float* xh, const float* vec, const void* rbf_image, const int32_t* edge_owner,
                               int64_t num_edges, float* dW, float* scratch, int32_t vec_is_zero, void* stream);
int32_t adf_op_vdot_fwd(const float* vv, float* dot, float* nrm, int32_t ldn, int64_t N, int32_t C, float eps, void* stream);
int32_t adf_op_vdot_bwd(const float* vv, const float* nrm, int32_t ldn, const float* ddot, const float* dnrm, int32_t lddn,
                        const float* dv1, float* dvv, int64_t N, int32_t C, void* stream);
int32_t adf_op_update_out_fwd(const float* x1, const float* vec1, const float* a, const float* dot, const float* vv, float s,
                              float* x2, float* vec2, int64_t N, int32_t H, void* stream);
int32_t adf_op_update_out_bwd(const float* a, const float* dot, const float* vv, float s, const float* dx2,
                              const float* dvec2, float* da, float* ddot, float* dv1, float* dx1, float* dvec1, int64_t N,
// ... 214 lines not shown
```

Measured before the change: 259.8.

## Emit row maxima from last update GEMM epilogue to feed output heads

The last layer's gated update GEMM now writes per-row partial absolute maxima for x and vec. Small combine kernels reduce these so the output heads can skip their separate row-magnitude passes over vec and x. The head GEMMs also emit partial maxima for the concatenated inputs, and the un2 GEMM gains a split-activation epilogue that writes the SiLU'd half directly, which removes the separate xact kernel. In exchange there is more workspace, pointer bookkeeping to track whether the maxima are still valid (which in incremental mode can force a whole-layer recompute of the last layer), and extra small combine launches.

```diff
diff --git a/adsorbdiff_amd/csrc/api.hip b/adsorbdiff_amd/csrc/api.hip
--- a/adsorbdiff_amd/csrc/api.hip
+++ b/adsorbdiff_amd/csrc/api.hip
@@ -43,6 +43,7 @@
     t.eqv2_rotout_generic = getenv("ADF_EQV2_ROTOUT_GENERIC") != nullptr;
     const char* r4 = getenv("ADF_GEMM_ROWS4");
     t.gemm_rows4 = r4 ? (atoi(r4) & 3) : 3;
+    t.head_maxima = off_is_0("ADF_HEAD_MAXIMA");
     return t;
 }
 const adf_tune& adf_tune_process() {
@@ -159,6 +160,8 @@
     h->lift.cap = 0; h->mag_v3_valid = false;
     h->xpart = h->catpart = h->vpart = nullptr; h->part_stride = 0;
     h->part_x = h->part_vec = nullptr; h->dbg_msg_rows = h->dbg_cat_rows = h->dbg_comb_rows = 0; h->dbg_mag = nullptr;
+    h->mag_x_last = h->hd_cat = h->mag_x1 = h->hd_cat1 = h->mag_v_last = h->e2x = h->e2v = nullptr;
+    h->hm_x = h->hm_vec = nullptr; h->hm_n = 0;
     h->cache_valid = false;
     h->capN = h->capB = h->capE = 0;
 }
@@ -309,6 +312,8 @@
     ALLOC(mag_v3, capN * 3);
     const int64_t ps = (capN + 31) / 32 * 32, ns = H / ADF_SLICE_CH;
     if (h->rmx) ALLOC(rmx_part, (4 * ns + H / 32 + 4) * ps);
+    const int64_t nc0 = H / 64, nc1 = (H / 2 + 63) / 64;
+    if (h->rmx && h->tune.head_maxima) ALLOC(hd_part, (1 + nc0 + 1 + nc1 + 3 + 4 * (H / 32)) * ps);
 #undef ALLOC
     h->lift.cap = st == ADF_OK ? capN * 3 : 0;
     if (st != ADF_OK) { free_workspaces(h); return st; }
@@ -316,6 +321,12 @@
         h->part_stride = ps;
         h->xpart = h->rmx_part; h->catpart = h->xpart + ns * ps; h->vpart = h->catpart + (H / 32) * ps;
         h->dbg_mag = h->vpart + 3 * ns * ps;
+    }
+    if (h->hd_part) {
+        h->mag_x_last = h->hd_part; h->hd_cat = h->mag_x_last + ps;
+        h->mag_x1 = h->hd_cat + nc0 * ps; h->hd_cat1 = h->mag_x1 + ps;
+        h->mag_v_last = h->hd_cat1 + nc1 * ps;
+        h->e2x = h->mag_v_last + 3 * ps; h->e2v = h->e2x + (H / 32) * ps;
     }
     h->capN = capN; h->capB = capB; h->capE = capE;
     return ADF_OK;
@@ -474,10 +485,21 @@
     return st;
 }
 
-static int32_t update_layer(adf_painn* h, int l, int N, float* x, float* vec, hipStream_t s, bool from_message = true) {
+static bool head_maxima_on(const adf_painn* h) {
+    const int H = h->hp.hidden_channels, L = h->hp.num_layers;
+    return h->tune.head_maxima && h->rmx && h->lift_on && !h->gemm_f32 && h->hd_part && h->hp.num_heads > 0 &&
+           adf_gemm16_epi2_emits(h->tune, &h->layer[L - 1].xv2_16, H, H);
+}
+
+static int32_t update_layer(adf_painn* h, int l, int N, float* x, float* vec, hipStream_t s, bool from_message = true,
+                            const float* tab_x = nullptr, const float* tab_vec = nullptr, int tab_n = 0,
+                            const int32_t* list = nullptr) {
     const int H = h->hp.hidden_channels;
     const adf_layer_weights& w = h->layer[l];
     adf_prof_begin(h, ADF_PROF_NODE, s);
+    const bool hm_cur = tab_x && h->hm_x == tab_x && h->hm_vec == tab_vec && h->hm_n == tab_n;
+    const bool hm = tab_x && head_maxima_on(h) && N > 0 && N <= h->part_stride && (!list || hm_cur);
+    if (!hm && h->hm_x && (h->hm_x == (tab_x ? tab_x : x) || h->hm_vec == (tab_x ? tab_vec : vec))) h->hm_x = h->hm_vec = nullptr;
     const bool parts = from_message && h->rmx && h->lift_on && !h->gemm_f32 && N > 0 && h->part_x == x && h->part_vec == vec &&
                        h->part_n == N && h->part_dev == h->rows_dev;
     h->part_x = h->part_vec = nullptr;
@@ -520,7 +542,16 @@
         ep.x = x; ep.vec = vec; ep.dot = h->dot; ep.vv = h->vv; ep.scale = h->scale[l]; ep.H = H;
         ep.rmag = h->lift_on ? h->mag_b : nullptr;
         ep.m_dev = h->rows_dev;
+        if (hm) { ep.xpart = h->e2x; ep.vpart = h->e2v; ep.part_stride = h->part_stride; }
         st = adf_launch_gemm16_fused(h->y, H, &w.xv2_16, N, H, H, 2, &ep, s, h->tune);
+        if (st == ADF_OK && hm) {
+            h->hm_x = h->hm_vec = nullptr;
+            st = adf_launch_rowmax_combine(h->e2x, h->part_stride, H / 32, N, h->mag_x_last, s, h->rows_dev, 1, list);
+            if (st == ADF_OK)
+                st = adf_launch_rowmax_combine(h->e2v, 3 * h->part_stride, H / 32, 3ll * N, h->mag_v_last, s, h->rows_dev, 3, list);
+            if (st == ADF_OK) { h->hm_x = tab_x; h->hm_vec = tab_vec; h->hm_n = tab_n; }
+            if (st == ADF_OK && list) { ++h->dbg_hm_list_launches; h->dbg_hm_list_rows = N; }
+        }
     }
     adf_prof_end(h, s);
     return st;
@@ -555,8 +586,28 @@
 
 extern "C" int32_t adf_painn_debug_row_maxima(adf_painn_t h, int32_t which, float* out, int64_t capacity, int32_t* rows,
                                               void* stream) {
-    if (!h || which < 0 || which > 6) { adf_set_error("debug_row_maxima: null handle or which outside 0..6"); return ADF_EINVAL; }
+    if (!h || which < 0 || which > 18) { adf_set_error("debug_row_maxima: null handle or which outside 0..18"); return ADF_EINVAL; }
     if (which == 4) { h->dbg_capture = capacity != 0; h->dbg_comb_rows = 0; return ADF_OK; }
+    if (which >= 17) {
+        if (rows) *rows = which == 17 ? h->dbg_hm_list_launches : h->dbg_hm_list_rows;
+        return ADF_OK;
+    }
+    if (which >= 7) {
+        const int H = h->hp.hidden_channels, H2 = H / 2, n = h->hm_x ? h->hm_n : 0;
+        if (!h->hd_part || n <= 0) { adf_set_error("debug_row_maxima: no forward has left the heads' row maxima (ADF_HEAD_MAXIMA=0?)"); return ADF_EINVAL; }
+        if (rows) *rows = n;
+        if (!out) return ADF_OK;
+        const int64_t widths[10] = {1, 3, H, 3 * H, 1, H, 1, H2, 1, H2};
+        const int64_t need = widths[which - 7] * n;
+        if (capacity < need) { adf_set_error("debug_row_maxima: out holds %lld floats, need %lld", (long long)capacity, (long long)need); return ADF_EINVAL; }
+        hipStream_t s = (hipStream_t)stream;
+        if (which == 11) return adf_launch_rowmax_combine(h->hd_cat, h->part_stride, H / 64, n, out, s);
+        if (which == 13) return adf_launch_rowmax_combine(h->hd_cat1, h->part_stride, (H2 + 63) / 64, n, out, s);
+        const float* src = which == 7 ? h->mag_x_last : which == 8 ? h->mag_v_last : which == 9 ? h->hm_x : which == 10 ? h->hm_vec :
+                           which == 12 ? h->cat : which == 14 ? h->dot : which == 15 ? h->mag_x1 : h->xh + (size_t)n * H;
+        ADF_HIP_CHECK(hipMemcpyAsync(out, src, sizeof(float) * (size_t)need, hipMemcpyDeviceToDevice, s));
+        return ADF_OK;
+    }
     const int H = h->hp.hidden_channels, ns = H / ADF_SLICE_CH;
     const int n = which <= 1 ? h->dbg_msg_rows : which <= 3 ? h->dbg_cat_rows : h->dbg_comb_rows;
     if (!h->rmx_part || n <= 0) { adf_set_error("debug_row_maxima: no launch has emitted row maxima (ADF_ROW_MAXIMA=0?)"); return ADF_EINVAL; }
@@ -703,14 +754,16 @@
     if (first) ADF_TRY(make_records(h, 0, N, h->incX[0], nullptr, true, h->incR[0], nullptr, s));
     for (int l = 0; l < L; ++l) {
         const int n_seen = h->inc_seen_valid ? h->inc_seen[l] : N;
-        const bool whole = first || !h->inc_seen_valid || h->inc_pend_Nseen != N || (long long)n_seen * 10 >= (long long)N * 9;
+        const bool last = l == L - 1;
+        const bool hm_stale = last && head_maxima_on(h) && !(h->hm_x == h->incX[L] && h->hm_vec == h->incV[L] && h->hm_n == N);
+        const bool whole = first || !h->inc_seen_valid || h->inc_pend_Nseen != N || (long long)n_seen * 10 >= (long long)N * 9 || hm_stale;
         h->inc_pend_whole[slot][l] = whole ? 1 : 0;
         if (h->inc_sync && !whole && n_seen == 0) continue;
         const float* vin = l == 0 ? h->vecA : h->incV[l];
         if (whole) {
             ADF_TRY(message_layer(h, l, N, h->incX[l], vin, h->incX[l + 1], h->incV[l + 1], l == 0, s, nullptr, 0,
                                   h->incR[l], true));
-            ADF_TRY(update_layer(h, l, N, h->incX[l + 1], h->incV[l + 1], s));
+            ADF_TRY(update_layer(h, l, N, h->incX[l + 1], h->incV[l + 1], s, true, last ? h->incX[L] : nullptr, h->incV[L], N));
             if (l + 1 < L)
                 ADF_TRY(make_records(h, l + 1, N, h->incX[l + 1], h->incV[l + 1], false, h->incR[l + 1], nullptr, s));
             continue;
@@ -719,7 +772,7 @@
         const int ncap = h->inc_sync ? n_seen : N;
         h->rows_dev = h->inc_cnt + l;
         int32_t st = message_layer(h, l, N, h->incX[l], vin, h->x, h->vecB, l == 0, s, list, ncap, h->incR[l], true);
-        if (st == ADF_OK) st = update_layer(h, l, ncap, h->x, h->vecB, s);
+        if (st == ADF_OK) st = update_layer(h, l, ncap, h->x, h->vecB, s, true, last ? h->incX[L] : nullptr, h->incV[L], N, list);
         if (st == ADF_OK) {
             adf_prof_begin(h, ADF_PROF_NODE, s);
             st = adf_inc_scatter_rows(h->x, list, ncap, H, h->incX[l + 1], s, h->rows_dev);
@@ -771,6 +824,7 @@
         return forward_incremental(h, N, b->atomic_numbers, out_idx, n_out, f1, f2, inc == 2, heads, s);
     }
     ADF_TRY(zero_pad_rows(h, N, s));
+    if (h->hm_x == h->x) h->hm_x = h->hm_vec = nullptr;
     ADF_TRY(adf_nodewise_embed(h, b->atomic_numbers, N, h->x, s));
     float* vin = h->vecA;
     float* vout = h->vecB;
@@ -794,7 +848,7 @@
             if (l == 0) ADF_TRY(message_layer(h, 0, N, h->x, vin, h->x, vout, true, s, nullptr, 0, rec0, rec0_ready));
             else
             ADF_TRY(message_layer(h, l, N, h->x, vin, h->x, vout, l == 0, s));
-            ADF_TRY(update_layer(h, l, N, h->x, vout, s));
+            ADF_TRY(update_layer(h, l, N, h->x, vout, s, true, l == L - 1 ? h->x : nullptr, vout, N));
             float* t = vin; vin = vout; vout = t;
         }
         adf_prof_begin(h, ADF_PROF_HEADS, s);
diff --git a/adsorbdiff_amd/csrc/common.h b/adsorbdiff_amd/csrc/common.h
--- a/adsorbdiff_amd/csrc/common.h
+++ b/adsorbdiff_amd/csrc/common.h
@@ -144,6 +144,10 @@
     int gate_ld;
     float* catpart;
     long long part_stride;
+    float* xpart;
+    float* vpart;
+    float* xact;
+    int xact_cols;
 };
 struct adf_lift {
     float* buf;
@@ -198,6 +202,11 @@
     bool dbg_capture;
     float* dbg_mag;
     int dbg_comb_rows;
+    float* hd_part;
+    float *mag_x_last, *hd_cat, *mag_x1, *hd_cat1, *mag_v_last, *e2x, *e2v;
+    const float *hm_x, *hm_vec;
+    int hm_n;
+    int dbg_hm_list_launches, dbg_hm_list_rows;
 
     int64_t capN, capB, capE;
     int32_t* nbr_cnt;
@@ -290,12 +299,14 @@
 int32_t adf_launch_rowmag(const float* A, int lda, int K1, const float* A2, int K2, long long M, float* mag, hipStream_t s,
                           const int32_t* m_dev = nullptr, int m_mul = 1);
 int32_t adf_launch_rowmax_combine(const float* part, long long stride, int nparts, long long M, float* mag, hipStream_t s,
-                                  const int32_t* m_dev = nullptr, int m_mul = 1);
+                                  const int32_t* m_dev = nullptr, int m_mul = 1, const int32_t* idx = nullptr);
+bool adf_gemm16_rows4_plain(const adf_tune& tune, const adf_w16* W, int M, int N, int K, int num_cus);
+bool adf_gemm16_epi2_emits(const adf_tune& tune, const adf_w16* W, int H, int K);
 int32_t adf_split_weight(const float* w, long long n, adf_w16* out, unsigned int* scratch_bits, hipStream_t s,
                          int perm_H = 0, int K = 0, const float* bias = nullptr, int parts = 3);
 int32_t adf_launch_gemm16_vecnorm(const float* A, int lda, const adf_w16* W, float* nrm, int M, int N, int K,
                                   hipStream_t s, const adf_tune& tune, const adf_lift* lf = nullptr,
-                                  const float* premag = nullptr);
+                                  const float* premag = nullptr, float* catpart = nullptr, long long part_stride = 0);
 int32_t adf_launch_gemm16_fused(const float* A, int lda, const adf_w16* W, int M, int H, int K, int epi,
                                 const adf_epi* ep, hipStream_t s, const adf_tune& tune, const adf_lift* lf = nullptr);
 static inline int32_t adf_linear(const adf_painn* h, const float* A, int lda, const float* W, const adf_w16* W16,
diff --git a/adsorbdiff_amd/csrc/gemm16.hip b/adsorbdiff_amd/csrc/gemm16.hip
--- a/adsorbdiff_amd/csrc/gemm16.hip
+++ b/adsorbdiff_amd/csrc/gemm16.hip
@@ -40,7 +40,7 @@
     return s * 1.6666666666666667f;
 }
 
-template <int ACT, int MI, int NJ, int EPI, bool WR = false, int NWN = 2, int NWM = 2>
+template <int ACT, int MI, int NJ, int EPI, bool WR = false, int NWN = 2, int NWM = 2, bool EMIT = false>
 __global__ __launch_bounds__(64 * NWM * NWN, (MI == 4 || NWM * NWN == 8 ? 1 : 2)) void adf_gemm_f16x3_kernel(
     const float* __restrict__ A, int lda, const _Float16* __restrict__ Whi, const _Float16* __restrict__ Wlo,
     const float* __restrict__ inv_scale, const float* __restrict__ bias, float* __restrict__ C, int ldc, int Mh, int N,
@@ -48,6 +48,8 @@
     const int M = ep.m_dev ? min(Mh, (int)*ep.m_dev) : Mh;
     static_assert(NWN == 2 || WR, "eight waves only with the register-streamed weights");
     static_assert(NWM == 2 || (NWM == 1 && WR), "one wave along M only with the register-streamed weights");
+    static_assert(!EMIT || EPI == 2, "row maxima of the stored rows: the gating epilogue only");
+    static_assert(ACT != 2 || EPI == 0, "the split activation belongs to the plain epilogue");
     constexpr int NT = 64 * NWM * NWN;
     constexpr int TM = 32 * MI * NWM;
     constexpr int TN = 32 * NJ * NWN;
@@ -316,6 +318,9 @@
             const int q = lane & 31;
             __syncthreads();
             float* T = reinterpret_cast<float*>(lds) + wave * (32 * TLD2);
+            const bool xt = ACT == 2 && n0 < ep.xact_cols;
+            float* const Cst = xt ? ep.xact : C;
+            const int ldst = xt ? ep.xact_cols : ldc;
 #pragma unroll
             for (int jj = 0; jj < NJ / 2; ++jj) {
                 const int cb = n0 + wn + 64 * jj;
@@ -328,7 +333,7 @@
                         const int lr = (r & 3) + 8 * (r >> 2) + 4 * (lane >> 5);
                         const float sc = isc * rinv[wm + 32 * i + lr];
                         float v0 = acc[i][2 * jj][r] * sc + bv0, v1 = acc[i][2 * jj + 1][r] * sc + bv1;
-                        if (ACT) { v0 = ssilu16(v0); v1 = ssilu16(v1); }
+                        if (ACT == 1 || xt) { v0 = ssilu16(v0); v1 = ssilu16(v1); }
                         T[lr * TLD2 + q] = v0;
                         T[lr * TLD2 + 32 + q] = v1;
                     }
@@ -349,9 +354,9 @@
                                 const float4 o = *reinterpret_cast<const float4*>(C + (size_t)row * ldc + col);
                                 v.x += o.x; v.y += o.y; v.z += o.z; v.w += o.w;
                             }
-                            *reinterpret_cast<float4*>(C + (size_t)row * ldc + col) = v;
+                            *reinterpret_cast<float4*>(Cst + (size_t)row * ldst + col) = v;
                         }
-                        if (ep.out_mag) {
+                        if (ep.out_mag && (ACT != 2 || xt)) {
                             float mg = col < N ? fmaxf(fmaxf(fabsf(v.x), fabsf(v.y)), fmaxf(fabsf(v.z), fabsf(v.w))) : 0.f;
                             mg = adf_row16_max(mg);
                             if (c4 == 0 && row < M) atomicMax(ep.out_mag + row, __float_as_uint(mg));
@@ -374,7 +379,7 @@
                     const int row = m0 + wm + 32 * i + (r & 3) + 8 * (r >> 2) + 4 * (lane >> 5);
                     if (row < M) {
                         float v = acc[i][j][r] * (isc * rinv[row - m0]) + bv;
-                        if (ACT) v = ssilu16(v);
+                        if (ACT == 1) v = ssilu16(v);
                         if (ep.accumulate) v += C[(size_t)row * ldc + col];
                         C[(size_t)row * ldc + col] = v;
                         if (ep.out_mag) atomicMax(ep.out_mag + row, __float_as_uint(fabsf(v)));
@@ -473,8 +478,12 @@
         for (int it = 0; it < 8; ++it) {
             const int lr = it * 4 + (lane >> 4), c4 = lane & 15;
             const int n = a0 + lr, c = cb + 4 * c4;
-            if (n < M && c < N)
-                *reinterpret_cast<float4*>(ep.cat + (size_t)n * N + c) = *reinterpret_cast<const float4*>(T + lr * TLD2 + 4 * c4);
+            const float4 nv_ = *reinterpret_cast<const float4*>(T + lr * TLD2 + 4 * c4);
+            if (n < M && c < N) *reinterpret_cast<float4*>(ep.cat + (size_t)n * N + c) = nv_;
+            if (ep.catpart) {
+                const float mg = adf_row16_max(c < N ? fmaxf(fmaxf(fmaxf(0.f, fabsf(nv_.x)), fabsf(nv_.y)), fmaxf(fabsf(nv_.z), fabsf(nv_.w))) : 0.f);
+                if (c4 == 0 && n < M && cb < N) ep.catpart[(size_t)(cb / 64) * ep.part_stride + n] = mg;
+            }
         }
     } else {
         static_assert(EPI >= 3 || (NJ == 3 && MI == 2), "fused epilogues are written for the 64 x 96 wave tile");
@@ -598,6 +607,30 @@
 #else
 #define EPI2_ST(r_, p_, base_, v_) (*reinterpret_cast<float4*>(p_) = (v_))
 #endif
+                    if constexpr (EMIT) {
+                        float4 t3[3];
+                        float mq[4];
+                        mq[3] = adf_lane8_max(fmaxf(fmaxf(fmaxf(0.f, fabsf(xo4.x)), fabsf(xo4.y)), fmaxf(fabsf(xo4.z), fabsf(xo4.w))));
+#pragma unroll
+                        for (int ax = 0; ax < 3; ++ax) {
+                            float4 t = tv[it][ax];
+                            const float4 v1 = w1[it][ax];
+                            t.x += p2.x * v1.x; t.y += p2.y * v1.y; t.z += p2.z * v1.z; t.w += p2.w * v1.w;
+                            t3[ax] = t;
+                            mq[ax] = adf_lane8_max(fmaxf(fmaxf(fmaxf(0.f, fabsf(t.x)), fabsf(t.y)), fmaxf(fabsf(t.z), fabsf(t.w))));
+                        }
+                        if (n < M) {
+                            EPI2_ST(rx, ep.x + (size_t)n * H + c, ep.x, xo4);
+                            float* vr = ep.vec + (size_t)n * 3 * H + c;
+#pragma unroll
+                            for (int ax = 0; ax < 3; ++ax) EPI2_ST(rv, vr + ax * H, ep.vec, t3[ax]);
+                            if (c4 == 0) {
+                                ep.xpart[(size_t)g * ep.part_stride + n] = mq[3];
+                                float* vp = ep.vpart + (size_t)g * 3 * ep.part_stride + (size_t)n * 3;
+                                vp[0] = mq[0]; vp[1] = mq[1]; vp[2] = mq[2];
+                            }
+                        }
+                    } else
                     if (n < M) {
                         EPI2_ST(rx, ep.x + (size_t)n * H + c, ep.x, xo4);
                         float* vr = ep.vec + (size_t)n * 3 * H + c;
@@ -644,19 +677,20 @@
 
 __global__ __launch_bounds__(256) void adf_rowmax_combine_kernel(const float* __restrict__ part, long long stride, int nparts,
                                                                  long long M, float* __restrict__ mag,
-                                                                 const int32_t* __restrict__ m_dev, int m_mul) {
+                                                                 const int32_t* __restrict__ m_dev, int m_mul,
+                                                                 const int32_t* __restrict__ idx) {
     const long long r = (long long)blockIdx.x * 256 + threadIdx.x;
     if (r >= M || (m_dev && r >= (long long)*m_dev * m_mul)) return;
     float mx = 0.f;
     for (int p = 0; p < nparts; ++p) mx = fmaxf(mx, part[(size_t)p * stride + r]);
-    mag[r] = mx;
+    mag[idx ? (long long)idx[r / m_mul] * m_mul + r % m_mul : r] = mx;
 }
 
 int32_t adf_launch_rowmax_combine(const float* part, long long stride, int nparts, long long M, float* mag, hipStream_t s,
-                                  const int32_t* m_dev, int m_mul) {
+                                  const int32_t* m_dev, int m_mul, const int32_t* idx) {
     if (M <= 0) return ADF_OK;
     hipLaunchKernelGGL(adf_rowmax_combine_kernel, dim3((unsigned)((M + 255) / 256)), dim3(256), 0, s, part, stride, nparts, M,
-                       mag, m_dev, m_mul);
+                       mag, m_dev, m_mul, idx);
     ADF_HIP_CHECK(hipGetLastError());
     return ADF_OK;
 }
@@ -755,6 +789,14 @@
     return ADF_OK;
 }
 
+bool adf_gemm16_rows4_plain(const adf_tune& tune, const adf_w16* W, int M, int N, int K, int num_cus) {
+    const int ncu = num_cus > 0 ? num_cus : 256;
+    const long long wg4 = (long long)((M + 95) / 96) * (N / 256 > 0 ? N / 256 : 1), slots4 = 2ll * ncu;
+    const bool ragged4 = wg4 < 4 * slots4 && wg4 % slots4 != 0 && wg4 % slots4 < (3 * slots4) / 10 && wg4 > slots4;
+    return (tune.gemm_rows4 & 1) && tune.gemm_w8_plain && W->frag && N % 256 == 0 && K % HK == 0 && (K / HK) % 2 == 0 &&
+           tune.gemm16_mi == 2 && !ragged4;
+}
+
 int32_t adf_launch_gemm16(const float* A, int lda, const adf_w16* W, const float* bias, float* C, int ldc, int M,
                           int N, int K, int act_ssilu, const adf_epi* ep_in, hipStream_t s, const adf_lift* lf,
                           const adf_tune& tune, int num_cus) {
@@ -782,12 +824,21 @@
     const int ncu = num_cus > 0 ? num_cus : 256;
     const long long wg8 = (long long)((M + 191) / 192) * (N / 256 > 0 ? N / 256 : 1);
     const bool ragged = wg8 < 4ll * ncu && wg8 % ncu != 0 && wg8 % ncu < (3 * ncu) / 10 && wg8 > ncu;
-    const long long wg4 = (long long)((M + 95) / 96) * (N / 256 > 0 ? N / 256 : 1), slots4 = 2ll * ncu;
-    const bool ragged4 = wg4 < 4 * slots4 && wg4 % slots4 != 0 && wg4 % slots4 < (3 * slots4) / 10 && wg4 > slots4;
-    if ((tune.gemm_rows4 & 1) && tune.gemm_w8_plain && W->frag && N % 256 == 0 && (K / HK) % 2 == 0 && mi == 2 && !ragged4) {
+    const bool rows4 = adf_gemm16_rows4_plain(tune, W, M, N, K, num_cus);
+    if (ep.xact) {
+        if (!rows4 || act_ssilu || ep.gate || ep.accumulate || ep.xact_cols <= 0 || ep.xact_cols % 256 || ep.xact_cols >= N || (ldc & 3) ||
+            (((uintptr_t)C | (uintptr_t)ep.xact) & 15)) {
+            adf_set_error("gemm16: the split-activation epilogue needs the 96 x 256 four-wave form, xact_cols a multiple of 256 below N and 16-byte aligned outputs");
+            return ADF_EINVAL;
+        }
+    }
+    if (rows4) {
         const int tn4 = N / 256, tmw4 = ((M + 95) / 96 + 7) / 8 * 8;
         dim3 g4((unsigned)(tmw4 * tn4));
-        if (act_ssilu)
+        if (ep.xact)
+            hipLaunchKernelGGL((adf_gemm_f16x3_kernel<2, 3, 2, 0, true, 4, 1>), g4, dim3(256), 0, s, A, lda, (const _Float16*)W->frag,
+                               (const _Float16*)nullptr, W->inv_scale, bias, C, ldc, M, N, K, tn4, ep);
+        else if (act_ssilu)
             hipLaunchKernelGGL((adf_gemm_f16x3_kernel<1, 3, 2, 0, true, 4, 1>), g4, dim3(256), 0, s, A, lda, (const _Float16*)W->frag,
                                (const _Float16*)nullptr, W->inv_scale, bias, C, ldc, M, N, K, tn4, ep);
         else
@@ -820,12 +871,14 @@
 }
 
 int32_t adf_launch_gemm16_vecnorm(const float* A, int lda, const adf_w16* W, float* nrm, int M, int N, int K,
-                                  hipStream_t s, const adf_tune& tune, const adf_lift* lf, const float* premag) {
+                                  hipStream_t s, const adf_tune& tune, const adf_lift* lf, const float* premag, float* catpart,
+                                  long long part_stride) {
     if (M <= 0) return ADF_OK;
     if (K % HK != 0 || (lda & 3) || (N & 3)) { adf_set_error("gemm16_vecnorm: bad shape"); return ADF_EINVAL; }
     ADF_TRY(check_a_span(3ll * M, lda));
     adf_epi ep = {};
     ep.cat = nrm;
+    ep.catpart = catpart; ep.part_stride = part_stride;
     ADF_TRY(lift_mags(A, lda, K, nullptr, 0, 3ll * M, lf, premag, &ep.rmag, s));
     const int tn = (N + 127) / 128, tm8 = ((M + 63) / 64 + 7) / 8 * 8;
     if ((tune.gemm_rows4 & 1) && tune.gemm_w8 && W->frag && N % 256 == 0 && (K / HK) % 2 == 0) {
@@ -850,6 +903,11 @@
     return ADF_OK;
 }
 
+bool adf_gemm16_epi2_emits(const adf_tune& tune, const adf_w16* W, int H, int K) {
+    return (tune.gemm_rows4 & 2) && tune.gemm_wr_fused == 2 && W->frag && W->bias_perm && K % HK == 0 && (K / HK) % 2 == 0 &&
+           H % 64 == 0 && (3 * H) % 384 == 0;
+}
+
 int32_t adf_launch_gemm16_fused(const float* A, int lda, const adf_w16* W, int M, int H, int K, int epi,
                                 const adf_epi* ep_in, hipStream_t s, const adf_tune& tune, const adf_lift* lf) {
     adf_epi epv = *ep_in;
@@ -862,6 +920,10 @@
     ADF_TRY(check_a_span(epi == 3 ? 3ll * M : (long long)M, lda));
     ADF_TRY(lift_mags(A, lda, K, nullptr, 0, epi == 3 ? 3ll * M : (long long)M, lf, ep_in->rmag, &epv.rmag, s, ep_in->m_dev,
                       epi == 3 ? 3 : 1));
+    if (ep_in->xpart && (epi != 2 || !ep_in->vpart || !adf_gemm16_epi2_emits(tune, W, H, K))) {
+        adf_set_error("gemm16_fused: row maxima asked of a form that does not emit them");
+        return ADF_EINVAL;
+    }
     const int N = 3 * H, TM = 128, TN = 192;
     const int tiles_n = N / TN;
     const int tiles_m = (M + TM - 1) / TM;
@@ -890,6 +952,9 @@
         if (epi == 1)
             hipLaunchKernelGGL((adf_gemm_f16x3_kernel<0, 2, 3, 1, true, 4, 1>), g4, dim3(256), 0, s, A, lda, (const _Float16*)W->frag,
                                (const _Float16*)nullptr, W->inv_scale, W->bias_perm, (float*)nullptr, 0, M, N, K, N / 384, *ep);
+        else if (ep->xpart)
+            hipLaunchKernelGGL((adf_gemm_f16x3_kernel<0, 2, 3, 2, true, 4, 1, true>), g4, dim3(256), 0, s, A, lda, (const _Float16*)W->frag,
+                               (const _Float16*)nullptr, W->inv_scale, W->bias_perm, (float*)nullptr, 0, M, N, K, N / 384, *ep);
         else
             hipLaunchKernelGGL((adf_gemm_f16x3_kernel<0, 2, 3, 2, true, 4, 1>), g4, dim3(256), 0, s, A, lda, (const _Float16*)W->frag,
                                (const _Float16*)nullptr, W->inv_scale, W->bias_perm, (float*)nullptr, 0, M, N, K, N / 384, *ep);
diff --git a/adsorbdiff_amd/csrc/nodewise.hip b/adsorbdiff_amd/csrc/nodewise.hip
--- a/adsorbdiff_amd/csrc/nodewise.hip
+++ b/adsorbdiff_amd/csrc/nodewise.hip
@@ -256,7 +256,12 @@
     const bool lift = h->lift_on && !h->gemm_f32;
     const adf_lift* lf = lift ? &h->lift : nullptr;
     const float* vmag = nullptr;
-    if (lift) {
+    const bool fg0 = h->tune.head_gate_fused && !h->gemm_f32 && (H2 & 3) == 0;
+    const bool hm = lift && fg0 && h->tune.head_maxima && h->hd_part && h->hm_x == x && h->hm_vec == vec && h->hm_n == N &&
+                    N <= h->part_stride;
+    const bool xa = hm && H2 % 256 == 0 && adf_gemm16_rows4_plain(h->tune, &b0.un2_16, N, H, H, h->num_cus);
+    if (hm) vmag = h->mag_v_last;
+    else if (lift) {
         if (head == 0 || !h->mag_v3_valid) ADF_TRY(adf_launch_rowmag(vec, H, H, nullptr, 0, 3ll * N, h->mag_v3, s));
         h->mag_v3_valid = head == 0;
         vmag = h->mag_v3;
@@ -265,7 +270,8 @@
         ADF_TRY(adf_linear(h, vec, H, b0.vec1_w, &b0.vec1_16, nullptr, t1, H, 3 * N, H, H, 0, s));
         hipLaunchKernelGGL(adf_head_norm_cat_kernel, dim3(ew_grid((long long)N * H / 4)), dim3(256), 0, s, x, t1, h->cat, N, H);
     } else {
-        ADF_TRY(adf_launch_gemm16_vecnorm(vec, H, &b0.vec1_16, h->cat, N, H, H, s, h->tune, lf, vmag));
+        ADF_TRY(adf_launch_gemm16_vecnorm(vec, H, &b0.vec1_16, h->cat, N, H, H, s, h->tune, lf, vmag, hm ? h->hd_cat : nullptr,
+                                          h->part_stride));
     }
     const bool fg = h->tune.head_gate_fused && !h->gemm_f32 && (H2 & 3) == 0;
     if (!fg) ADF_TRY(adf_linear(h, vec, H, b0.vec2_w, &b0.vec2_16, nullptr, t2, H2, 3 * N, H2, H, 0, s, vmag));
@@ -274,9 +280,20 @@
         adf_epi e0 = {};
         e0.A2 = h->cat; e0.K1 = H;
         e0.out_mag = h->lift_on ? reinterpret_cast<unsigned int*>(h->mag_b) : nullptr;
+        if (hm) {
+            ADF_TRY(adf_launch_rowmax_combine(h->mag_x_last, h->part_stride, 1 + H / 64, N, h->lift.buf, s));
+            e0.rmag = h->lift.buf;
+        }
         ADF_TRY(adf_launch_gemm16(x, H, &b0.un0_16, b0.un0_b, h->y, H, N, H, 2 * H, 1, &e0, s, h->lift_on ? &h->lift : nullptr,
                                   h->tune, h->num_cus));
     }
+    if (xa) {
+        adf_epi e2 = {};
+        e2.rmag = h->mag_b;
+        e2.xact = x1; e2.xact_cols = H2;
+        e2.out_mag = reinterpret_cast<unsigned int*>(h->mag_x1);
+        ADF_TRY(adf_launch_gemm16(h->y, H, &b0.un2_16, b0.un2_b, o, H, N, H, H, 0, &e2, s, lf, h->tune, h->num_cus));
+    } else
     ADF_TRY(adf_linear(h, h->y, H, b0.un2_w, &b0.un2_16, b0.un2_b, o, H, N, H, H, 0, s, (h->lift_on && !h->gemm_f32) ? h->mag_b : nullptr));
     if (fg) {
         adf_epi eg = {};
@@ -284,7 +301,7 @@
         eg.out_mag = lift ? reinterpret_cast<unsigned int*>(h->lift.buf) : nullptr;
         eg.gate = o + H2; eg.gate_ld = H;
         ADF_TRY(adf_launch_gemm16(vec, H, &b0.vec2_16, nullptr, v1, H2, 3 * N, H2, H, 0, &eg, s, lf, h->tune, h->num_cus));
-        hipLaunchKernelGGL(adf_head_xact_kernel, dim3(ew_grid((long long)N * H2 / 4)), dim3(256), 0, s, o, x1, N, H2);
+        if (!xa) hipLaunchKernelGGL(adf_head_xact_kernel, dim3(ew_grid((long long)N * H2 / 4)), dim3(256), 0, s, o, x1, N, H2);
     } else
     hipLaunchKernelGGL(adf_head_gate_kernel, dim3(ew_grid((long long)N * H2 / 4)), dim3(256), 0, s, o, t2, x1, v1, N, H2);
     if (h->gemm_f32) {
@@ -293,9 +310,13 @@
         ADF_TRY(adf_linear(h, cat1, H, b1.un0_w, &b1.un0_16, b1.un0_b, h->y, H2, N, H2, H, 1, s));
     } else {
         ADF_TRY(adf_launch_gemm16_vecnorm(v1, H2, &b1.vec1_16, cat1, N, H2, H2, s, h->tune, h->lift_on ? &h->lift : nullptr,
-                                          (fg && lift) ? h->lift.buf : nullptr));
+                                          (fg && lift) ? h->lift.buf : nullptr, xa ? h->hd_cat1 : nullptr, h->part_stride));
         adf_epi e1 = {};
         e1.A2 = cat1; e1.K1 = H2;
+        if (xa) {
+            ADF_TRY(adf_launch_rowmax_combine(h->mag_x1, h->part_stride, 1 + (H2 + 63) / 64, N, h->lift.buf, s));
+            e1.rmag = h->lift.buf;
+        }
         ADF_TRY(adf_launch_gemm16(x1, H2, &b1.un0_16, b1.un0_b, h->y, H2, N, H2, H, 1, &e1, s, h->lift_on ? &h->lift : nullptr,
                                   h->tune, h->num_cus));
     }
diff --git a/adsorbdiff_amd/lib.py b/adsorbdiff_amd/lib.py
--- a/adsorbdiff_amd/lib.py
+++ b/adsorbdiff_amd/lib.py
@@ -66,7 +66,7 @@
         "gemm16_mi", "gemm_w8_plain", "gemm_w8", "gemm_wreg", "gemm_wr_fused", "head_gate_fused", "lift_emit",
         "graph_sys_csr", "train_gemm16", "wgrad_f32",
         "eqv2_pw_mi", "eqv2_gemm_tile256", "eqv2_rotin_generic", "eqv2_rotout_generic",
-        "gemm_rows4")]
+        "gemm_rows4", "head_maxima")]
 
 
 class BatchDesc(C.Structure):
diff --git a/include/adsorbdiff_hip.h b/include/adsorbdiff_hip.h
--- a/include/adsorbdiff_hip.h
+++ b/include/adsorbdiff_hip.h
@@ -72,6 +72,7 @@
     int32_t eqv2_rotin_generic;
     int32_t eqv2_rotout_generic;
     int32_t gemm_rows4;
+    int32_t head_maxima;
 } adf_tune;
 int32_t adf_painn_get_tune(adf_painn_t h, adf_tune* out);
 
```

Result: no change. 261.6, median of 6 (+0.7%).
